# biodatageeks/datafusion-bio-functions

Hardware: AMD Instinct MI355X
Metric: overlap-pairs/sec + probe-rows/sec, IntervalJoinExec 100Mx1M (higher is better)
Workload: dtype int32; 1 GPU; join_100Mx1M_24contigs; probe_rows_per_gpu=100000000, build_rows_per_gpu=1000000, contigs=24, pairs_per_gpu=37210484, parallelism=partition-per-gpu x1, gather=False, build_overlap=True

## Files before the change

datafusion-bio-functions_amd/csrc/ivx_capi.hip:

```cpp
#include "ivx_internal.hpp"
#include <cstdlib>
#include <atomic>
#include <chrono>
#include <cstring>
#include <mutex>
#include <new>
#include <thread>
#include <condition_variable>
#include <deque>


void ivx_ctx::join_tail()
{
    if (!tail_pending) return;
    (void)hipStreamWaitEvent(stream, tail_ev, 0);
    tail_pending = false;
}

ivx_status ivx_ctx::get_scratch(int slot, size_t bytes, void **out)
{
    if (tail_pending && slot != WS_SORTHIST && slot != WS_T0 && slot != WS_T1 && slot != WS_T2) join_tail();
    ivx_buf &b = scratch[slot];
    if (sub_plan.valid && ((sub_plan.slots >> slot) & 1)) sub_plan.valid = false;
    if (join_plan.valid && ((join_plan.rows.slots >> slot) & 1)) join_plan.valid = false;
// ... 125 lines not shown
template <typename T>
ivx_status copy_out(ivx_ctx *ctx, int mem, T *dst, const T *dev, u64 n)
{
    if (mem == IVX_MEM_DEVICE || dst == nullptr || n == 0) return IVX_OK;
    IVX_HIP(ctx, hipMemcpyAsync(dst, dev, (size_t)n * sizeof(T), hipMemcpyDeviceToHost, ctx->stream));
    return IVX_OK;
}

ivx_status read_scalar(ivx_ctx *ctx, int word, u64 *out)
{
    IVX_HIP(ctx, hipMemcpyAsync(ctx->h_scalars + word, ctx->d_scalars + word, sizeof(u64), hipMemcpyDeviceToHost, ctx->stream));
    IVX_HIP(ctx, hipStreamSynchronize(ctx->stream));
    *out = ctx->h_scalars[word];
    return IVX_OK;
}

ivx_status check_probe_args(ivx_ctx *ctx, const ivx_index *ix, int kind, int mem, const void *s, const void *e, u64 n, bool defer_ready = false)
{
    if (!ctx) return IVX_ERR_INVALID;
    if (!ix) return ctx->fail(IVX_ERR_INVALID, "null index");
    if (ix->kind != kind) return ctx->fail(IVX_ERR_UNSUPPORTED, "index kind does not match this probe");
    if (ix->device != ctx->device) return ctx->fail(IVX_ERR_INVALID, "index lives on another device");
    if (mem != IVX_MEM_HOST && mem != IVX_MEM_DEVICE) return ctx->fail(IVX_ERR_INVALID, "bad mem");
    if (n && (!s || !e)) return ctx->fail(IVX_ERR_INVALID, "null coordinate column");
    if (n > 0xFFFFFFFFull) return ctx->fail(IVX_ERR_INVALID, "probe batch exceeds UInt32 index capacity");
    IVX_HIP(ctx, hipSetDevice(ctx->device));
    if (ix->ready != nullptr && !defer_ready) IVX_HIP(ctx, hipStreamWaitEvent(ctx->stream, ix->ready, 0));
    return IVX_OK;
}

struct CallMetrics {
    ivx_ctx *c; bool build; std::chrono::steady_clock::time_point t0;
    CallMetrics(ivx_ctx *ctx, bool is_build, u64 rows) : c(ctx), build(is_build), t0(std::chrono::steady_clock::now())
    {
        if (build) { c->metrics.build_input_batches++; c->metrics.build_input_rows += rows; }
        else { c->metrics.input_batches++; c->metrics.input_rows += rows; }
    }
    void out(u64 rows) { if (rows) { c->metrics.output_batches++; c->metrics.output_rows += rows; } }
    ~CallMetrics()
    {
        const double ms = std::chrono::duration<double, std::milli>(std::chrono::steady_clock::now() - t0).count();
        (build ? c->metrics.build_time : c->metrics.join_time) += ms;
    }
};

struct KernelTimer {
    ivx_ctx *c;
    explicit KernelTimer(ivx_ctx *ctx) : c(ctx) { (void)hipEventRecord(c->ev0, c->stream); c->last_ms = -1.0; }
    ~KernelTimer() { (void)hipEventRecord(c->ev1, c->stream); }
};

}


extern "C" const char *ivx_version(void) { return "ivx-hip 0.1 (gfx950)"; }

static bool create_aux_stream(hipStream_t *out)
{
    int lo = 0, hi = 0;
    if (hipDeviceGetStreamPriorityRange(&lo, &hi) == hipSuccess && hipStreamCreateWithPriority(out, hipStreamNonBlocking, hi) == hipSuccess) return true;
    return hipStreamCreateWithFlags(out, hipStreamNonBlocking) == hipSuccess;
}

extern "C" ivx_status ivx_ctx_create(int device_ordinal, ivx_ctx **out)
{
    if (!out) return IVX_ERR_INVALID;
    *out = nullptr;
    int ndev = 0;
    if (hipGetDeviceCount(&ndev) != hipSuccess || ndev <= 0) return IVX_ERR_NO_DEVICE;
    if (device_ordinal < 0 || device_ordinal >= ndev) return IVX_ERR_NO_DEVICE;
    hipDeviceProp_t prop;
    if (hipGetDeviceProperties(&prop, device_ordinal) != hipSuccess) return IVX_ERR_NO_DEVICE;
    if (std::strncmp(prop.gcnArchName, "gfx950", 6) != 0) return IVX_ERR_NO_DEVICE;
    ivx_ctx *c = new (std::nothrow) ivx_ctx();
    if (!c) return IVX_ERR_OOM;
    c->device = device_ordinal;
    bool ok = hipSetDevice(device_ordinal) == hipSuccess &&
              hipStreamCreateWithFlags(&c->own_stream, hipStreamNonBlocking) == hipSuccess &&
              create_aux_stream(&c->aux) &&
              hipEventCreateWithFlags(&c->ev_fork, hipEventDisableTiming) == hipSuccess &&
              hipEventCreateWithFlags(&c->tail_ev, hipEventDisableTiming) == hipSuccess &&
              hipEventCreate(&c->ev0) == hipSuccess && hipEventCreate(&c->ev1) == hipSuccess &&
              hipMalloc((void **)&c->d_scalars, 64 * sizeof(u64)) == hipSuccess &&
              hipHostMalloc((void **)&c->h_scalars, 64 * sizeof(u64), hipHostMallocDefault) == hipSuccess;
    if (!ok) { ivx_ctx_free(c); return IVX_ERR_HIP; }
    c->stream = c->own_stream;
    if (const char *e = getenv("IVX_BUILD_OVERLAP")) c->overlap = e[0] == '1';
    *out = c;
    return IVX_OK;
}

extern "C" void ivx_ctx_free(ivx_ctx *c)
{
    if (!c) return;
    (void)hipSetDevice(c->device);
    (void)hipStreamSynchronize(c->stream);
    if (c->aux) (void)hipStreamSynchronize(c->aux);
    for (auto &b : c->scratch) if (b.p) (void)hipFree(b.p);
    for (auto &b : c->pinned) if (b.p) (void)hipHostFree(b.p);
    if (c->d_scalars) (void)hipFree(c->d_scalars);
    if (c->h_scalars) (void)hipHostFree(c->h_scalars);
    if (c->ev0) (void)hipEventDestroy(c->ev0);
    if (c->ev1) (void)hipEventDestroy(c->ev1);
    if (c->own_stream) (void)hipStreamDestroy(c->own_stream);
    if (c->aux) (void)hipStreamDestroy(c->aux);
    if (c->ev_fork) (void)hipEventDestroy(c->ev_fork);
    if (c->tail_ev) (void)hipEventDestroy(c->tail_ev);
    delete c;
}

extern "C" const char *ivx_last_error(const ivx_ctx *c) { return c ? c->err.c_str() : "null ctx"; }

extern "C" ivx_status ivx_ctx_set_stream(ivx_ctx *c, void *hip_stream)
{
    if (!c) return IVX_ERR_INVALID;
    if (c->tail_pending) { (void)hipStreamSynchronize(c->aux); c->tail_pending = false; }
    c->stream = (hipStream_t)hip_stream;
    return IVX_OK;
}

extern "C" ivx_status ivx_ctx_use_own_stream(ivx_ctx *c)
{
    if (!c) return IVX_ERR_INVALID;
    if (c->tail_pending) { (void)hipStreamSynchronize(c->aux); c->tail_pending = false; }
    c->stream = c->own_stream;
    return IVX_OK;
}

extern "C" ivx_status ivx_ctx_set_build_overlap(ivx_ctx *c, int on)
{
    if (!c) return IVX_ERR_INVALID;
    c->overlap = on != 0;
    return IVX_OK;
}

extern "C" ivx_status ivx_ctx_synchronize(ivx_ctx *c)
{
    if (!c) return IVX_ERR_INVALID;
    if (c->tail_pending) { IVX_HIP(c, hipStreamSynchronize(c->aux)); c->tail_pending = false; }
    IVX_HIP(c, hipStreamSynchronize(c->stream));
    return IVX_OK;
}

extern "C" ivx_status ivx_ctx_metrics(const ivx_ctx *c, ivx_metrics *out)
{
    if (!c || !out) return IVX_ERR_INVALID;
    *out = c->metrics;
    return IVX_OK;
}

extern "C" void ivx_ctx_reset_metrics(ivx_ctx *c) { if (c) c->metrics = ivx_metrics{}; }

extern "C" ivx_status ivx_ctx_set_memory_limit(ivx_ctx *c, uint64_t bytes)
{
    if (!c) return IVX_ERR_INVALID;
    c->mem_limit = bytes;
    return IVX_OK;
}

extern "C" uint64_t ivx_ctx_reserved_bytes(const ivx_ctx *c) { return c ? c->reserved() : 0; }

extern "C" ivx_status ivx_ctx_trim(ivx_ctx *c, uint64_t keep_bytes)
{
    if (!c) return IVX_ERR_INVALID;
    IVX_HIP(c, hipSetDevice(c->device));
    IVX_HIP(c, hipStreamSynchronize(c->stream));
    if (c->aux) { IVX_HIP(c, hipStreamSynchronize(c->aux)); c->tail_pending = false; }
    c->sub_plan.valid = false; c->join_plan.valid = false;
// ... 76 lines not shown
    if (ix->ready) { (void)hipEventSynchronize(ix->ready); (void)hipEventDestroy(ix->ready); }
    for (size_t i = 0; i < ix->allocs.size(); i++) pool_give(ix->device, ix->allocs[i], ix->alloc_caps[i]);
    if (ix->owner_bytes) ix->owner_bytes->fetch_sub(ix->bytes, std::memory_order_relaxed);
    delete ix;
}

extern "C" uint64_t ivx_index_rows(const ivx_index *ix) { return ix ? ix->n : 0; }
extern "C" uint64_t ivx_index_device_bytes(const ivx_index *ix) { return ix ? ix->bytes : 0; }

extern "C" ivx_status ivx_index_layout(ivx_ctx *ctx, const ivx_index *ix, uint32_t *out, uint32_t n_out)
{
    if (!ctx) return IVX_ERR_INVALID;
    if (!ix) return ctx->fail(IVX_ERR_INVALID, "null index");
    if (n_out && !out) return ctx->fail(IVX_ERR_INVALID, "null out");
    if (ix->device != ctx->device) return ctx->fail(IVX_ERR_INVALID, "index lives on another device");
    u32 w[IVX_LAYOUT_WORDS] = {};
    w[IVX_LAYOUT_KIND] = (u32)ix->kind;
    if (ix->kind != IVX_KIND_NEAREST && ix->jv.hdr != nullptr) {
        IVX_HIP(ctx, hipSetDevice(ctx->device));
        if (ix->ready != nullptr) IVX_HIP(ctx, hipStreamWaitEvent(ctx->stream, ix->ready, 0));
        u32 h[HDR_WORDS];
        IVX_HIP(ctx, hipMemcpyAsync(h, ix->jv.hdr, sizeof(h), hipMemcpyDeviceToHost, ctx->stream));
        IVX_HIP(ctx, hipStreamSynchronize(ctx->stream));
        const u32 nlev = h[HDR_NLEV] < IVX_MAXL ? h[HDR_NLEV] : IVX_MAXL;
        u32 levrows = 0;
        for (u32 l = 0; l < nlev; l++) if (h[HDR_LEVCNT + l]) levrows |= 1u << l;
        w[IVX_LAYOUT_SH0] = h[HDR_SH0];
        w[IVX_LAYOUT_NLEV] = h[HDR_NLEV];
        w[IVX_LAYOUT_LEVROWS] = levrows;
        w[IVX_LAYOUT_RCELLS] = h[HDR_NREG] ? h[HDR_RCELLS] : 0u;
        w[IVX_LAYOUT_RCS] = h[HDR_NREG] ? h[HDR_CS] : 0xFFFFFFFFu;
        w[IVX_LAYOUT_NREG] = h[HDR_NREG];
        w[IVX_LAYOUT_PK24] = h[HDR_PK24];
        w[IVX_LAYOUT_SLOW] = h[HDR_SLOW];
        w[IVX_LAYOUT_FG] = h[HDR_FG];
        w[IVX_LAYOUT_FBITS] = h[HDR_FG] != 0xFFFFFFFFu ? h[HDR_FBITS] : 0u;
        w[IVX_LAYOUT_NROUTE_NREG] = ix->nroute_nreg;
        w[IVX_LAYOUT_LBUILD] = h[HDR_LBUILD];
    }
    for (u32 i = 0; i < n_out && i < (u32)IVX_LAYOUT_WORDS; i++) out[i] = w[i];
    return IVX_OK;
}


static bool rowval_routed_ok(u64 n)
{
    if (const char *f = getenv("IVX_JOIN_PATH")) return !strcmp(f, "routed");
    return n >= (1u << 21);
}

static ivx_status overlap_common(ivx_ctx *ctx, const ivx_index *ix, int mem, int mode,
                                 const u32 *key, const i32 *start, const i32 *end, u64 n,
                                 u32 *per_row, u8 *exists, u32 *bidx, u32 *pidx, u64 cap, u64 *total)
{
    IVX_TRY(check_probe_args(ctx, ix, IVX_KIND_OVERLAP, mem, start, end, n, true));
    CallMetrics cm(ctx, false, n);
    const u32 *dk = nullptr; const i32 *ds = nullptr, *de = nullptr;
    bool regions = ix->jv_nreg > 0 && (mode == JP_COUNT || mode == JP_FILL) && n >= (1u << 21);
    bool rowval = ix->jv_nreg > 0 && ix->jv_nreg <= IVX_MAXREG_WIDE && (mode == JP_PER_ROW || mode == JP_EXISTS) && n >= (1u << 21);
    if (const char *f = getenv("IVX_JOIN_PATH")) {
        if (!strcmp(f, "direct")) regions = rowval = false;
        else if (!strcmp(f, "regions")) {
            regions = ix->jv_nreg > 0 && (mode == JP_COUNT || mode == JP_FILL);
            rowval = ix->jv_nreg > 0 && ix->jv_nreg <= IVX_MAXREG_WIDE && (mode == JP_PER_ROW || mode == JP_EXISTS);
        }
    }
    const void *in[3] = {key, start, end};
    ivx_join_plan &pl = ctx->join_plan;
    const bool planned = regions && mode == JP_FILL && pl.valid && !getenv("IVX_NO_PLAN") && pl.mem == mem && memcmp(pl.in, in, sizeof(in)) == 0 && pl.n == n &&
                         pl.ix == (const void *)ix && pl.ix_serial == ix->serial && pl.stream == ctx->stream;
    if (ix->ready != nullptr && !(regions && !planned)) IVX_HIP(ctx, hipStreamWaitEvent(ctx->stream, ix->ready, 0));
    if (!planned) {
        IVX_TRY(stage_in(ctx, mem, WS_IN_KEY, key, n, &dk));
        IVX_TRY(stage_in(ctx, mem, WS_IN_START, start, n, &ds));
        IVX_TRY(stage_in(ctx, mem, WS_IN_END, end, n, &de));
    }
    u32 *d_row = nullptr, *d_b = nullptr, *d_p = nullptr; u8 *d_ex = nullptr;
    IVX_TRY(stage_out(ctx, mem, WS_OUT_A, per_row, n, &d_row));
    IVX_TRY(stage_out(ctx, mem, WS_OUT_B, exists, n, &d_ex));
    IVX_TRY(stage_out(ctx, mem, WS_OUT_C, bidx, cap, &d_b));
    IVX_TRY(stage_out(ctx, mem, WS_OUT_D, pidx, cap, &d_p));
    const bool defer_clear = regions && !planned;
    if (!defer_clear) IVX_HIP(ctx, hipMemsetAsync(ctx->d_scalars, 0, 2 * sizeof(u64), ctx->stream));
    {
        KernelTimer t(ctx);
        if (regions) {
            if (!planned) pl.valid = false;
            const ivx_status st = ivx_join_probe_regions(ctx, ix->jv, ix->jv_nreg, mode, dk, ds, de, n, d_b, d_p, cap, ctx->d_scalars, planned, ix->jv_filter, ix->jv_pk24,
                                                         ix->jv_fast_unknown ? 2 : (ix->jv_fast ? 1 : 0), planned ? nullptr : ix->ready, defer_clear);
            if (st != IVX_OK) { pl.valid = false; return st; }
            if (mode == JP_COUNT && pl.valid) { memcpy(pl.in, in, sizeof(in)); pl.mem = mem; pl.n = n; pl.ix = ix; pl.ix_serial = ix->serial; pl.stream = ctx->stream; }
        }
        else if (rowval) IVX_TRY(ivx_rowval_probe_regions(ctx, ix->jv, ix->jv_nreg, mode == JP_PER_ROW ? IVX_RV_PER_ROW : IVX_RV_EXISTS, dk, ds, de, n, 0,
                                                          mode == JP_PER_ROW ? (void *)d_row : (void *)d_ex, ctx->d_scalars, ix->jv_filter, ix->jv_pk24, ix->jv_fast && !ix->jv_fast_unknown));
        else if (n && (mode == JP_PER_ROW || mode == JP_EXISTS) && ix->nroute_nreg > 0 && rowval_routed_ok(n))
            IVX_TRY(ivx_join_rowval_routed(ctx, ix, mode, dk, ds, de, n, d_row, d_ex, ctx->d_scalars));
        else IVX_TRY(ivx_join_probe(ctx, ix->jv, mode, dk, ds, de, n, d_row, d_ex, d_b, d_p, cap, ctx->d_scalars));
    }
    u64 tot = 0;
    if (mode != JP_EXISTS) {
        IVX_HIP(ctx, hipMemcpyAsync(ctx->h_scalars, ctx->d_scalars, 2 * sizeof(u64), hipMemcpyDeviceToHost, ctx->stream));
        IVX_HIP(ctx, hipStreamSynchronize(ctx->stream));
        tot = ctx->h_scalars[0];
        if (ctx->h_scalars[1]) { ctx->join_plan.valid = false; return ctx->fail(IVX_ERR_HIP, "internal error: the probe met an unpublished page of routed rows"); }
    }
    if (mode == JP_COUNT && regions && pl.valid) pl.total = tot;
    if (total) *total = tot;
    if (mode == JP_FILL && tot > cap) return ctx->fail(IVX_ERR_CAPACITY, "pair buffers too small");
    cm.out(mode == JP_FILL ? tot : (mode == JP_COUNT ? 0 : n));
    if (planned) pl.valid = false;
    IVX_TRY(copy_out(ctx, mem, per_row, d_row, n));
    IVX_TRY(copy_out(ctx, mem, exists, d_ex, n));
    if (mode == JP_FILL) { IVX_TRY(copy_out(ctx, mem, bidx, d_b, tot)); IVX_TRY(copy_out(ctx, mem, pidx, d_p, tot)); }
    if (mem == IVX_MEM_HOST) IVX_HIP(ctx, hipStreamSynchronize(ctx->stream));
    return IVX_OK;
}

extern "C" ivx_status ivx_probe_overlap_count(ivx_ctx *ctx, const ivx_index *ix, int mem, const uint32_t *key,
                                              const int32_t *start, const int32_t *end, uint64_t n,
                                              uint32_t *per_row, uint64_t *total)
{
    return overlap_common(ctx, ix, mem, per_row ? JP_PER_ROW : JP_COUNT, key, start, end, n, per_row, nullptr, nullptr, nullptr, 0, total);
}

__global__ void k_add_base(u32 *__restrict__ p, u64 n, u32 base)
{
    for (u64 i = (u64)blockIdx.x * blockDim.x + threadIdx.x; i < n; i += (u64)gridDim.x * blockDim.x) p[i] += base;
}

struct HostCopier {
    struct Job { void *dst; const void *src; size_t bytes; hipEvent_t ev; };
    std::mutex mu; std::condition_variable cv, cv_done; std::deque<Job> jobs; bool closed = false; hipError_t herr = hipSuccess;
    u64 done = 0;
    hipStream_t cs = nullptr; std::thread th; std::vector<hipEvent_t> evs; bool started = false;
    hipError_t start(int device)
    {
        const hipError_t e = hipStreamCreateWithFlags(&cs, hipStreamNonBlocking);
        if (e != hipSuccess) return e;
        try {
        th = std::thread([this, device]() {
            (void)hipSetDevice(device);
            for (;;) {
                Job j;
                { std::unique_lock<std::mutex> lk(mu); cv.wait(lk, [&] { return closed || !jobs.empty(); }); if (jobs.empty()) return; j = jobs.front(); jobs.pop_front(); }
                hipError_t e2 = j.ev ? hipStreamWaitEvent(cs, j.ev, 0) : hipSuccess;
                if (e2 == hipSuccess && j.bytes) e2 = hipMemcpyAsync(j.dst, j.src, j.bytes, hipMemcpyDeviceToHost, cs);
                if (e2 == hipSuccess) e2 = hipStreamSynchronize(cs);
                { std::lock_guard<std::mutex> lk(mu); if (e2 != hipSuccess) herr = e2; done++; }
                cv_done.notify_all();
            }
        });
        } catch (...) { (void)hipStreamDestroy(cs); cs = nullptr; return hipErrorOutOfMemory; }
        started = true;
        return hipSuccess;
    }
    hipError_t mark(hipStream_t st, hipEvent_t *ev)
    {
        hipError_t e = hipEventCreateWithFlags(ev, hipEventDisableTiming);
        if (e != hipSuccess) return e;
        evs.push_back(*ev);
        return hipEventRecord(*ev, st);
    }
    void push(void *dst, const void *src, size_t bytes, hipEvent_t ev)
    {
        { std::lock_guard<std::mutex> lk(mu); jobs.push_back(Job{dst, src, bytes, ev}); }
        cv.notify_all();
    }
    void wait_until(u64 k) { std::unique_lock<std::mutex> lk(mu); cv_done.wait(lk, [&] { return done >= k; }); }
    hipError_t finish()
    {
        if (!started) return hipSuccess;
        { std::lock_guard<std::mutex> lk(mu); closed = true; }
        cv.notify_all();
        th.join();
        for (hipEvent_t e : evs) (void)hipEventDestroy(e);
        (void)hipStreamDestroy(cs);
        started = false;
        return herr;
    }
    ~HostCopier() { (void)finish(); }
};

static ivx_status overlap_fill_host_chunked(ivx_ctx *ctx, const ivx_index *ix, const u32 *key, const i32 *start, const i32 *end, u64 n,
                                            u32 *bidx, u32 *pidx, u64 cap, u64 *written, u32 nchunk)
// ... 46 lines not shown
        }
    }
    const hipError_t es = hipStreamSynchronize(st);
    const hipError_t herr = hc.finish();
    ctx->join_plan.valid = false;
    ctx->metrics.input_batches = m0.input_batches + 1;
    ctx->metrics.output_batches = m0.output_batches + ((rc == IVX_OK && !over && cum) ? 1 : 0);
    if (over) ctx->metrics.output_rows = m0.output_rows;
    if (rc != IVX_OK) return rc;
    if (es != hipSuccess) return ctx->fail_hip("hipStreamSynchronize", es);
    if (herr != hipSuccess) return ctx->fail_hip("hipMemcpyAsync(pairs)", herr);
    if (written) *written = over ? need : cum;
    if (over) return ctx->fail(IVX_ERR_CAPACITY, "pair buffers too small");
    return IVX_OK;
}

extern "C" ivx_status ivx_probe_overlap_fill(ivx_ctx *ctx, const ivx_index *ix, int mem, const uint32_t *key,
                                             const int32_t *start, const int32_t *end, uint64_t n,
                                             uint32_t *build_idx, uint32_t *probe_idx, uint64_t cap, uint64_t *written)
{
    if (ctx && cap && (!build_idx || !probe_idx)) return ctx->fail(IVX_ERR_INVALID, "null pair buffers");
    if (ctx && ix && mem == IVX_MEM_HOST && cap && start && end) {
        const char *ce = getenv("IVX_HOST_CHUNKS");
        const u32 nchunk = ce ? (u32)atoi(ce) : (n >= (16ull << 20) ? 4u : 1u);
        const void *in[3] = {key, start, end};
        const ivx_join_plan &pl = ctx->join_plan;
        const bool planned = pl.valid && pl.mem == mem && memcmp(pl.in, in, sizeof(in)) == 0 && pl.n == n && pl.ix == (const void *)ix && pl.ix_serial == ix->serial;
        if (nchunk > 1 && n >= (u64)nchunk * 65536 && !planned && ix->kind == IVX_KIND_OVERLAP)
            return overlap_fill_host_chunked(ctx, ix, key, start, end, n, build_idx, probe_idx, cap, written, nchunk);
    }
    return overlap_common(ctx, ix, mem, JP_FILL, key, start, end, n, nullptr, nullptr, build_idx, probe_idx, cap, written);
}

extern "C" ivx_status ivx_probe_exists(ivx_ctx *ctx, const ivx_index *ix, int mem, const uint32_t *key,
                                       const int32_t *start, const int32_t *end, uint64_t n, uint8_t *exists)
{
    if (ctx && n && !exists) return ctx->fail(IVX_ERR_INVALID, "null exists buffer");
    return overlap_common(ctx, ix, mem, JP_EXISTS, key, start, end, n, nullptr, exists, nullptr, nullptr, 0, nullptr);
}


namespace {

ivx_status marks_stage(ivx_ctx *ctx, int mem, u32 *caller, u64 nw, u32 **dev)
{
    if (mem == IVX_MEM_DEVICE) { *dev = caller; return IVX_OK; }
    IVX_TRY(ctx->get_scratch(WS_OUT_A, (size_t)nw * sizeof(u32), (void **)dev));
    if (nw) IVX_HIP(ctx, hipMemsetAsync(*dev, 0, (size_t)nw * sizeof(u32), ctx->stream));
    return IVX_OK;
}

ivx_status marks_or_back(ivx_ctx *ctx, int mem, u32 *caller, const u32 *dev, u64 nw)
{
    if (mem == IVX_MEM_DEVICE || nw == 0) return IVX_OK;
    std::vector<u32> got;
    try { got.resize((size_t)nw); } catch (const std::bad_alloc &) { return ctx->fail(IVX_ERR_OOM, "host allocation failed"); }
    IVX_HIP(ctx, hipMemcpyAsync(got.data(), dev, (size_t)nw * sizeof(u32), hipMemcpyDeviceToHost, ctx->stream));
    IVX_HIP(ctx, hipStreamSynchronize(ctx->stream));
    for (u64 w = 0; w < nw; w++) caller[w] |= got[w];
    return IVX_OK;
}

ivx_status mark_common(ivx_ctx *ctx, const ivx_index *ix, int mem, const u32 *key, const i32 *start, const i32 *end, u64 n, u32 *marks)
{
    IVX_TRY(check_probe_args(ctx, ix, IVX_KIND_OVERLAP, mem, start, end, n));
    if (n && ix->n && !marks) return ctx->fail(IVX_ERR_INVALID, "null mark bitmap");
    CallMetrics cm(ctx, false, n);
    ctx->join_plan.valid = false;
    const u64 nw = (ix->n + 31) / 32;
    if (n == 0 || nw == 0) return IVX_OK;
    bool regions = ix->jv_nreg > 0 && ix->jv_nreg <= IVX_MAXREG_WIDE && n >= (1u << 21);
    if (const char *f = getenv("IVX_JOIN_PATH")) {
        if (!strcmp(f, "direct")) regions = false;
        else if (!strcmp(f, "regions")) regions = ix->jv_nreg > 0 && ix->jv_nreg <= IVX_MAXREG_WIDE;
    }
    const u32 *dk = nullptr; const i32 *ds = nullptr, *de = nullptr; u32 *dm = nullptr;
    IVX_TRY(stage_in(ctx, mem, WS_IN_KEY, key, n, &dk));
    IVX_TRY(stage_in(ctx, mem, WS_IN_START, start, n, &ds));
    IVX_TRY(stage_in(ctx, mem, WS_IN_END, end, n, &de));
    IVX_TRY(marks_stage(ctx, mem, marks, nw, &dm));
    {
        KernelTimer t(ctx);
        bool took = false;
        if (regions) IVX_TRY(ivx_mark_probe_regions(ctx, ix->jv, ix->jv_nreg, dk, ds, de, n, dm, ix->jv_filter, ix->jv_pk24, ix->jv_fast && !ix->jv_fast_unknown, &took));
        if (!took) IVX_TRY(ivx_mark_probe(ctx, ix->jv, dk, ds, de, n, dm));
    }
    return marks_or_back(ctx, mem, marks, dm, nw);
}

}

extern "C" ivx_status ivx_probe_mark_build(ivx_ctx *ctx, const ivx_index *ix, int mem, const uint32_t *key,
                                           const int32_t *start, const int32_t *end, uint64_t n, uint32_t *marks)
{
    return mark_common(ctx, ix, mem, key, start, end, n, marks);
}

extern "C" ivx_status ivx_bits_mark(ivx_ctx *ctx, int mem, const uint32_t *idx, uint64_t n, uint32_t *bits, uint64_t n_bits)
{
    if (!ctx) return IVX_ERR_INVALID;
    if (mem != IVX_MEM_HOST && mem != IVX_MEM_DEVICE) return ctx->fail(IVX_ERR_INVALID, "bad mem");
    if (n && !idx) return ctx->fail(IVX_ERR_INVALID, "bits_mark: null idx");
    if (n_bits && !bits) return ctx->fail(IVX_ERR_INVALID, "bits_mark: null bitmap");
    if (n_bits > 0xFFFFFFFFull) return ctx->fail(IVX_ERR_INVALID, "bits_mark: bitmap exceeds UInt32 index capacity");
    if (n == 0) return IVX_OK;
    IVX_HIP(ctx, hipSetDevice(ctx->device));
    const u64 nw = (n_bits + 31) / 32;
    const u32 *didx; u32 *dbits;
    IVX_TRY(stage_in(ctx, mem, WS_IN_KEY, idx, n, &didx));
    IVX_TRY(marks_stage(ctx, mem, bits, nw, &dbits));
    {
        KernelTimer t(ctx);
        IVX_TRY(ivx_bits_mark_device(ctx, didx, n, dbits, n_bits));
    }
    return marks_or_back(ctx, mem, bits, dbits, nw);
}

extern "C" ivx_status ivx_bits_select(ivx_ctx *ctx, int mem, const uint32_t *bits, uint64_t n_bits, int want_set,
                                      uint32_t *out, uint64_t cap, uint64_t *n_out)
{
    if (!ctx) return IVX_ERR_INVALID;
    if (!n_out) return ctx->fail(IVX_ERR_INVALID, "null n_out");
    *n_out = 0;
    if (mem != IVX_MEM_HOST && mem != IVX_MEM_DEVICE) return ctx->fail(IVX_ERR_INVALID, "bad mem");
    if (n_bits && !bits) return ctx->fail(IVX_ERR_INVALID, "bits_select: null bitmap");
    if (cap && !out) return ctx->fail(IVX_ERR_INVALID, "bits_select: null out");
    if (n_bits > 0xFFFFFFFFull) return ctx->fail(IVX_ERR_INVALID, "bits_select: bitmap exceeds UInt32 index capacity");
    IVX_HIP(ctx, hipSetDevice(ctx->device));
    const u32 *dbits; u32 *dout;
    IVX_TRY(stage_in(ctx, mem, WS_IN_KEY, bits, (n_bits + 31) / 32, &dbits));
    IVX_TRY(stage_out(ctx, mem, WS_OUT_A, out, cap, &dout));
    u64 m = 0;
    {
        KernelTimer t(ctx);
        const ivx_status st = ivx_bits_select_device(ctx, dbits, n_bits, want_set, dout, cap, &m);
        *n_out = m;
        if (st != IVX_OK) return st;
    }
    if (cap) IVX_TRY(copy_out(ctx, mem, out, dout, m));
    if (mem == IVX_MEM_HOST) IVX_HIP(ctx, hipStreamSynchronize(ctx->stream));
    return IVX_OK;
}


ivx_status ivx_count_probe(ivx_ctx *ctx, const ivx_index *ix, const u32 *key, const i32 *s, const i32 *e, u64 n, int strict, i64 *out);
ivx_status ivx_coverage_probe(ivx_ctx *ctx, const ivx_index *ix, const u32 *key, const i32 *s, const i32 *e, u64 n, int strict, i64 *out);
ivx_status ivx_nearest_probe(ivx_ctx *ctx, const ivx_index *ix, const u32 *key, const i32 *s, const i32 *e, u64 n,
                             int strict, u32 k, int include_overlaps, u32 *ob, u32 *op, i64 *od, u64 cap, u64 *rows);
ivx_status ivx_merge_device(ivx_ctx *ctx, const u32 *key, const i64 *s, const i64 *e, u64 n, u32 nkeys,
                            i64 min_dist, int strict, u32 *ok, i64 *os, i64 *oe, i64 *on, u64 *m);
ivx_status ivx_subtract_device(ivx_ctx *ctx, const u32 *lkey, const i64 *ls, const i64 *le, u64 nl,
                               const u32 *rkey, const i64 *rs, const i64 *re, u64 nr, u32 nkeys, int strict,
                               u32 *ok, i64 *os, i64 *oe, u32 *orow, u64 cap, u64 *n_out);
ivx_status ivx_subtract_fill_planned(ivx_ctx *ctx, u32 *ok, i64 *os, i64 *oe, u32 *orow, u64 cap, u64 *n_out);
ivx_status ivx_cluster_device(ivx_ctx *ctx, const u32 *key, const i64 *s, const i64 *e, u64 n, u32 nkeys,
                              i64 min_dist, int strict, const i64 *key_base,
                              u32 *ok, i64 *os, i64 *oe, u32 *orow, i64 *oc, i64 *ocs, i64 *oce, u64 *key_clusters, u64 *m);
ivx_status ivx_complement_device(ivx_ctx *ctx, const u32 *key, const i64 *s, const i64 *e, u64 n,
                                 const u32 *vkey, const i64 *vs, const i64 *ve, u64 nv, u32 nkeys, int strict,
                                 u32 *ok, i64 *os, i64 *oe, u64 cap, u64 *n_out);
ivx_status ivx_take_fixed_device(ivx_ctx *ctx, const void *src, u32 width, u64 n_src, const u8 *src_valid,
                                 const u32 *idx, u64 n, void *out, u8 *out_valid);
ivx_status ivx_take_view_device(ivx_ctx *ctx, const void *views, const u8 *const *bufs, u64 n_src, const u8 *src_valid,
                                const u32 *idx, u64 n, void *out_views, u8 *out_data, u64 data_cap, u64 *data_bytes, u8 *out_valid);
ivx_status ivx_take_bits_device(ivx_ctx *ctx, const u8 *src_bits, u64 n_src, const u8 *src_valid, const u32 *idx, u64 n, u8 *out_bits, u8 *out_valid);
ivx_status ivx_take_utf8_device(ivx_ctx *ctx, int large, const void *offsets, const u8 *data, u64 n_src, const u8 *src_valid,
                                const u32 *idx, u64 n, void *out_offsets, u8 *out_data, u64 data_cap, u64 *data_bytes, u8 *out_valid);
// ... 936 lines not shown
```

datafusion-bio-functions_amd/csrc/ivx_device.hpp:

```cpp
#pragma once
#include "ivx_internal.hpp"

__device__ __forceinline__ u32 lane_id() { return __builtin_amdgcn_mbcnt_hi(~0u, __builtin_amdgcn_mbcnt_lo(~0u, 0u)); }

__device__ __forceinline__ u32 mask_rank_from(u64 mask, u32 base)
{
    return __builtin_amdgcn_mbcnt_hi((u32)(mask >> 32), __builtin_amdgcn_mbcnt_lo((u32)mask, base));
}

__device__ __forceinline__ u32 mask_rank(u64 mask)
{
    return __builtin_amdgcn_mbcnt_hi((u32)(mask >> 32), __builtin_amdgcn_mbcnt_lo((u32)mask, 0u));
}

template <int CTRL, int ROWS>
__device__ __forceinline__ u32 dpp0(u32 v) { return (u32)__builtin_amdgcn_update_dpp(0, (int)v, CTRL, ROWS, 0xf, false); }
__device__ __forceinline__ u32 wave_incl_max32(u32 v)
{
    u32 o;
    o = dpp0<0x111, 0xf>(v); v = o > v ? o : v;
    o = dpp0<0x112, 0xf>(v); v = o > v ? o : v;
    o = dpp0<0x114, 0xf>(v); v = o > v ? o : v;
    o = dpp0<0x118, 0xf>(v); v = o > v ? o : v;
    o = dpp0<0x142, 0xa>(v); v = o > v ? o : v;
    o = dpp0<0x143, 0xc>(v); v = o > v ? o : v;
    return v;
}
__device__ __forceinline__ u32 wave_incl_sum32(u32 v)
{
    v += dpp0<0x111, 0xf>(v); v += dpp0<0x112, 0xf>(v); v += dpp0<0x114, 0xf>(v); v += dpp0<0x118, 0xf>(v);
    v += dpp0<0x142, 0xa>(v); v += dpp0<0x143, 0xc>(v);
    return v;
}
__device__ __forceinline__ u32 wave_prev32(u32 v) { return dpp0<0x138, 0xf>(v); }
__device__ __forceinline__ u32 wave_next32(u32 v) { return dpp0<0x130, 0xf>(v); }

template <typename T>
__device__ __forceinline__ T wave_incl_scan(T v)
{
    const u32 l = lane_id();
#pragma unroll
    for (int d = 1; d < IVX_WAVE; d <<= 1) {
        T o = __shfl_up(v, d, IVX_WAVE);
        if (l >= (u32)d) v += o;
    }
    return v;
}

template <typename T>
__device__ __forceinline__ T wave_sum(T v)
{
#pragma unroll
    for (int d = IVX_WAVE / 2; d > 0; d >>= 1) v += __shfl_xor(v, d, IVX_WAVE);
    return v;
}

template <typename T, int NT>
__device__ __forceinline__ T block_excl_scan(T v, T *lds, T *total)
{
    constexpr int NW = NT / IVX_WAVE;
    const u32 l = lane_id();
    const u32 w = threadIdx.x / IVX_WAVE;
    T inc = wave_incl_scan(v);
    if (l == IVX_WAVE - 1) lds[w] = inc;
    __syncthreads();
    if (threadIdx.x == 0) {
        T run = 0;
#pragma unroll
        for (int i = 0; i < NW; i++) { T t = lds[i]; lds[i] = run; run += t; }
        lds[NW] = run;
    }
    __syncthreads();
    T res = inc - v + lds[w];
    *total = lds[NW];
    __syncthreads();
    return res;
}

template <typename T, int NT>
__device__ __forceinline__ T block_sum(T v, T *lds)
{
    constexpr int NW = NT / IVX_WAVE;
    T s = wave_sum(v);
    if (lane_id() == 0) lds[threadIdx.x / IVX_WAVE] = s;
    __syncthreads();
    T r = 0;
#pragma unroll
    for (int i = 0; i < NW; i++) r += lds[i];
    __syncthreads();
    return r;
}

static inline u32 ivx_stream_grid(u64 n, u32 per_block, u32 max_blocks = 2048)
{
    u64 b = (n + per_block - 1) / per_block;
    if (b < 1) b = 1;
// ... 4 lines not shown
```

datafusion-bio-functions_amd/csrc/ivx_internal.hpp:

```cpp
#pragma once
#include <hip/hip_runtime.h>
#include <stdint.h>
#include <atomic>
#include <memory>
#include <string>
#include <vector>
#include "../../include/ivx.h"

typedef uint8_t u8;
typedef uint32_t u32;
typedef int32_t i32;
typedef uint64_t u64;
typedef int64_t i64;

#define IVX_WAVE 64

struct ivx_buf { void *p = nullptr; size_t cap = 0; };

enum { IVX_NSCRATCH = 56, IVX_NPIN = 4 };

struct ivx_sub_plan {
    bool valid = false;
    u64 slots = 0;
    int mem = 0;
    const void *in[6] = {};
    u64 nl = 0, nr = 0, nh = 0, total = 0;
    u32 nkeys = 0;
    int strict = 0;
    int wf = 0;
    hipStream_t stream = nullptr;
    const u32 *lk, *lrow, *rk, *hk, *hj;
    const i64 *lsv, *lev, *rsv, *hrs, *hpm;
    const void *sm;
    const u64 *offs;
    const u32 *plan_hlo; const i64 *plan_tail;
};

struct PageTab { u32 *ptab; u32 pstride, lgpg; };
struct ivx_route_ctl {
    u32 rcur[1024];
    u32 pool_next, pad0[3];
    u32 rest_n[2], pad1[2];
    u32 rfirst[1032];
    u32 cfirst[1032];
};
struct FpRest;
enum {
    IVX_ROWS_FLAT = 0,
    IVX_ROWS_PAGED,
    IVX_ROWS_TABLE
};
struct ivx_routed {
    int form = IVX_ROWS_FLAT;
    const u64 *se = nullptr;
    const u32 *ids = nullptr;
    const unsigned short *cidx = nullptr;
    const u32 *rfirst = nullptr;
    u32 nblk = 1, chunk = 0, ndig = 0;
    const u32 *unsorted = nullptr;
    PageTab pt{nullptr, 0u, 0u};
    bool packed = false;
    u32 rowbits = 32;
    bool all_routed = false;
    ivx_route_ctl *ctl = nullptr;
    FpRest *rest = nullptr; u64 *rest_rows = nullptr;
    const uint2 *vtab = nullptr;
    const i32 *ds = nullptr, *de = nullptr;
    u32 adj = 0;
    u64 slots = 0;
};

struct ivx_join_plan {
    bool valid = false;
    int mem = 0;
    const void *in[3] = {};
    u64 n = 0;
    u64 total = 0;
    const void *ix = nullptr; u64 ix_serial = 0;
    hipStream_t stream = nullptr;
    ivx_routed rows;
};

struct ivx_ctx {
    int device = 0;
    hipStream_t own_stream = nullptr;
    hipStream_t stream = nullptr;
    hipEvent_t ev0 = nullptr, ev1 = nullptr;
    double last_ms = 0.0;
    std::string err;
    ivx_buf scratch[IVX_NSCRATCH];
    ivx_buf pinned[IVX_NPIN];
    u64 *d_scalars = nullptr;
    u64 *h_scalars = nullptr;
    ivx_sub_plan sub_plan;
    ivx_join_plan join_plan;
    ivx_metrics metrics{};
    u64 mem_limit = 0;
    u64 fill_hint = 0;
    u64 scratch_bytes = 0, building_bytes = 0;
    hipStream_t aux = nullptr;
    hipEvent_t ev_fork = nullptr, tail_ev = nullptr;
    bool overlap = false, tail_pending = false;
    void join_tail();
    std::shared_ptr<std::atomic<u64>> live_index_bytes = std::make_shared<std::atomic<u64>>(0);
    u64 reserved() const { return scratch_bytes + building_bytes + live_index_bytes->load(std::memory_order_relaxed); }

    ivx_status fail(ivx_status st, const std::string &msg) { err = msg; return st; }
    ivx_status fail_hip(const char *what, hipError_t e)
    {
        err = std::string(what) + ": " + hipGetErrorString(e);
        return e == hipErrorOutOfMemory ? IVX_ERR_OOM : IVX_ERR_HIP;
    }
    ivx_status get_scratch(int slot, size_t bytes, void **out);
    ivx_status get_pinned(int slot, size_t bytes, void **out);
};

#define IVX_HIP(ctx, call)                                              \
    do {                                                                \
        hipError_t e__ = (call);                                        \
        if (e__ != hipSuccess) return (ctx)->fail_hip(#call, e__);      \
    } while (0)

#define IVX_TRY(call)                                                   \
    do {                                                                \
        ivx_status s__ = (call);                                        \
        if (s__ != IVX_OK) return s__;                                  \
    } while (0)

enum {
    WS_IN_KEY = 0, WS_IN_START, WS_IN_END, WS_IN2_KEY, WS_IN2_START, WS_IN2_END,
    WS_OUT_A, WS_OUT_B, WS_OUT_C, WS_OUT_D, WS_OUT_E, WS_OUT_F, WS_OUT_G, WS_OUT_H,
    WS_SCAN0, WS_SCAN1, WS_SCAN2,
    WS_GRID0, WS_GRID1, WS_GRID2,
    WS_SORTHIST,
    WS_SA0, WS_SA1, WS_SA2, WS_SB0, WS_SB1, WS_SB2,
    WS_RA0, WS_RA1, WS_RA2, WS_RB0, WS_RB1, WS_RB2,
    WS_T0, WS_T1, WS_T2, WS_T3, WS_T4, WS_T5, WS_T6, WS_T7, WS_T8, WS_T9,
    WS_IN3_KEY, WS_IN3_START, WS_IN3_END, WS_IN3_WEIGHT, WS_IN_KEYLEN,
    WS_IN_TEXTOFF, WS_IN_TEXT
};
static_assert(WS_IN_TEXT < IVX_NSCRATCH, "scratch slot ids must fit the context's slot array");

#ifndef IVX_LSTEP
#define IVX_LSTEP 2
#endif
#define IVX_MAXL (32 / IVX_LSTEP)
#define IVX_SH_MIN 4

struct ivx_ent { i32 s, e; u32 row; };

enum { HDR_SH0 = 0, HDR_NLEV = 1, HDR_NBINS = 2, HDR_CS = 3 , HDR_NREG = 4,
       HDR_RCELLS = 5 , HDR_RMUL_LO = 6, HDR_RMUL_HI = 7 , HDR_LEVCNT = 8 ,
       HDR_FG = 8 + IVX_MAXL , HDR_FBITS = 9 + IVX_MAXL ,
       HDR_PK24 = 10 + IVX_MAXL ,
       HDR_SLOW = 11 + IVX_MAXL ,
       HDR_LBUILD = 12 + IVX_MAXL ,
       HDR_BADKEY = 13 + IVX_MAXL ,
       HDR_WORDS = 14 + IVX_MAXL };
#define IVX_FBITS_MAX (1u << 24)
#define IVX_MAXREG 255
#define IVX_MAXREG_WIDE 1023
#define IVX_MAXREG2 65025u
#define IVX_REG_CS_MAX 13

#ifndef IVX_RP_ECAP
#define IVX_RP_ECAP 6144
#endif
#define IVX_RP_HALO 8u
struct ivx_regdesc { u32 k; i32 origin; u32 span, lb, slo, shi, e0, ne; i32 rbase;  };

struct JoinIndexView {
    const i32 *origin;
    const u32 *span;
    const u32 *kcnt;
    const u32 *lbase;
    const u32 *binstart;
    const ivx_ent *ent;
    const u32 *hdr;
    const u32 *kreg;
    const u32 *rkey;
    const ivx_regdesc *rdesc;
    const u32 *fbits;
    const u32 *fbase;
    u32 nkeys;
};

struct RankGridView {
    const i32 *origin;
    const u32 *span;
    const u32 *kcnt;
    const u32 *koff;
    const u32 *kbase;
    const u32 *binstart;
    const i32 *val;
    const u32 *hdr;
    u32 nkeys;
};

struct CoverageView {
    RankGridView first, last;
    const i64 *pw;
    const i32 *nfirst, *nlast;
};

struct ivx_nrec { i32 a, b; u32 row; i32 pmax; };

struct NearestView {
    RankGridView by_start, by_end, pmax;
    const ivx_nrec *rs;
    const ivx_nrec *re;
    JoinIndexView ov;
};

struct DepthProfileView {
    const u32 *key, *pos;
    const i32 *cov;
    const u32 *koff;
    const u8 *seen;
    u64 steps;
};

struct ivx_index {
    u64 serial = 0;
    int kind = 0;
    int device = 0;
    u64 n = 0;
    u32 nkeys = 0;
    size_t bytes = 0;
    std::shared_ptr<std::atomic<u64>> owner_bytes;
    std::vector<void *> allocs;
    std::vector<size_t> alloc_caps;
    JoinIndexView jv{};
    u32 jv_nreg = 0;
    bool jv_filter = false;
    bool jv_pk24 = false;
    bool jv_fast = false;
    bool jv_fast_unknown = false;
    hipEvent_t ready = nullptr;
    RankGridView gs{}, ge{};
    CoverageView cv{};
    NearestView nv{};
    JoinIndexView nroute{};
    u32 nroute_nreg = 0;
    DepthProfileView dp{};
    int flags = 0;
};
enum { IVX_IXF_REGION_ROWVAL = 1 };

ivx_status ivx_scan_exclusive_u32(ivx_ctx *ctx, u32 *data, u64 n, const u32 *skip = nullptr);
ivx_status ivx_scan_exclusive_u64(ivx_ctx *ctx, u64 *data, u64 n);

ivx_status ivx_join_build(ivx_ctx *ctx, ivx_index *ix, const u32 *key, const i32 *s, const i32 *e, u64 n, bool overlap = false);
ivx_status ivx_join_probe(ivx_ctx *ctx, const JoinIndexView &jv, int mode,
                          const u32 *key, const i32 *s, const i32 *e, u64 n,
                          u32 *per_row, u8 *exists, u32 *ob, u32 *op, u64 cap, u64 *d_cursor);
enum { JP_COUNT = 0, JP_PER_ROW = 1, JP_EXISTS = 2, JP_FILL = 3 };
ivx_status ivx_join_probe_regions(ivx_ctx *ctx, const JoinIndexView &jv, u32 nreg, int mode,
                                  const u32 *key, const i32 *s, const i32 *e, u64 n,
                                  u32 *ob, u32 *op, u64 cap, u64 *d_cursor, bool planned = false, bool has_filter = false, bool pk24 = false,
                                  int fast = 0 , hipEvent_t ready = nullptr,
                                  bool clear_cursor = false );

enum { IVX_RV_COUNT = 0, IVX_RV_COVERAGE = 1, IVX_RV_PER_ROW = 2, IVX_RV_EXISTS = 3 };
ivx_status ivx_route_view_build(ivx_ctx *ctx, ivx_index *ix, const i32 *origin, const u32 *span, const u32 *kcnt);
void ivx_route_view_ready(ivx_ctx *ctx, ivx_index *ix);
ivx_status ivx_join_rowval_routed(ivx_ctx *ctx, const ivx_index *ix, int mode, const u32 *key, const i32 *s, const i32 *e, u64 n,
                                  u32 *per_row, u8 *exists, u64 *d_total);
ivx_status ivx_unroute_u32(ivx_ctx *ctx, const ivx_routed &r, u64 n, const u32 *vb, u32 *out32, u8 *out8);
ivx_status ivx_route_rows(ivx_ctx *ctx, const JoinIndexView &rv, const u32 *key, const i32 *s, const i32 *e, u64 n, u32 adj, ivx_routed *out);
ivx_status ivx_unroute_pair(ivx_ctx *ctx, const ivx_routed &r, u64 n, const u32 *vb, const i64 *vd, u32 *ob, u32 *op, i64 *od, i64 dflt);
ivx_status ivx_rowval_probe_regions(ivx_ctx *ctx, const JoinIndexView &jv, u32 nreg, int kind,
                                    const u32 *key, const i32 *s, const i32 *e, u64 n, int strict, void *out, u64 *d_total,
                                    bool has_filter = false, bool pk24 = false, bool fast = false);

ivx_status ivx_mark_probe(ivx_ctx *ctx, const JoinIndexView &jv, const u32 *key, const i32 *s, const i32 *e, u64 n, u32 *marks);
ivx_status ivx_mark_probe_regions(ivx_ctx *ctx, const JoinIndexView &jv, u32 nreg, const u32 *key, const i32 *s, const i32 *e, u64 n,
                                  u32 *marks, bool has_filter, bool pk24, bool fast, bool *took);
ivx_status ivx_bits_mark_device(ivx_ctx *ctx, const u32 *idx, u64 n, u32 *bits, u64 n_bits);
ivx_status ivx_bits_select_device(ivx_ctx *ctx, const u32 *bits, u64 n_bits, int want_set, u32 *out, u64 cap, u64 *n_out);

ivx_status ivx_depth_device(ivx_ctx *ctx, const u32 *rkey, const u32 *rpos, const u32 *rflags, const u32 *rmapq,
                            const i32 *cigar_offsets, const u32 *cigar_ops, u64 n_reads,
                            const u32 *skey, const u32 *sstart, const u32 *send, const i32 *sweight, u64 n_seg,
                            u32 nkeys, const u32 *key_len, u32 filter_flag, u32 min_mapq,
                            u32 *ok, u32 *os, u32 *oe, i32 *oc, u64 cap, u64 *n_out);

struct ivx_depth_evs { u64 n; const u64 *ev; const uint2 *cg; };
ivx_status ivx_depth_events(ivx_ctx *ctx, const u32 *rkey, const u32 *rpos, const u32 *rflags, const u32 *rmapq,
                            const i32 *cigar_offsets, const u32 *cigar_ops, u64 n_reads,
                            const u32 *skey, const u32 *sstart, const u32 *send, const i32 *sweight, u64 n_seg,
                            u32 nkeys, const u32 *key_len, u32 filter_flag, u32 min_mapq, u8 *seen, ivx_depth_evs *out);
struct ivx_cigar_plan {
    int large; const void *off; const u8 *txt; u64 n_reads, n_bytes, n_ops, nblk; i64 off0; u32 mis; void *tsum;
};
ivx_status ivx_cigar_count(ivx_ctx *ctx, int large, const void *text_offsets, const u8 *text, bool text_at_off0, u64 n_reads,
                           ivx_cigar_plan *plan);
ivx_status ivx_cigar_write(ivx_ctx *ctx, const ivx_cigar_plan &plan, i32 *out_off, u32 *out_ops);
ivx_status ivx_depth_profile_begin(ivx_ctx *ctx, ivx_index *ix, u8 **seen);
ivx_status ivx_depth_profile_finish(ivx_ctx *ctx, ivx_index *ix, const ivx_depth_evs &evs);
ivx_status ivx_depth_profile_koff(ivx_ctx *ctx, const u32 *skey, u32 steps, u32 nkeys, u32 *koff);
ivx_status ivx_depth_expand_device(ivx_ctx *ctx, const DepthProfileView &dp, u32 key, u32 first_pos, u64 n, int skip_pos0,
                                   i32 *out_pos, int16_t *out_cov);
ivx_status ivx_depth_profile_merge_device(ivx_ctx *ctx, const DepthProfileView &a, u32 nka, const DepthProfileView &b, u32 nkb, ivx_index *ix);
ivx_status ivx_depth_profile_blocks_device(ivx_ctx *ctx, const DepthProfileView &dp, u32 *ok, u32 *os, u32 *oe, i32 *oc, u64 cap, u64 *n_out);
ivx_status ivx_depth_regions_device(ivx_ctx *ctx, const DepthProfileView &dp, u32 nkeys, const u32 *qkey, const u32 *qs, const u32 *qe, u64 n,
                                    u32 pos_lo, const u32 *key_hi, int skip_pos0, const i32 *thresholds, u32 n_thr,
                                    i64 *out_len, i64 *out_sum, i64 *out_ge);
ivx_status ivx_depth_windows_device(ivx_ctx *ctx, const DepthProfileView &dp, u32 key, u32 first_pos, u32 last_pos, u32 width, u64 n,
                                    int skip_pos0, const i32 *thresholds, u32 n_thr, i64 *out_len, i64 *out_sum, i64 *out_ge);

ivx_status ivx_index_alloc(ivx_ctx *ctx, ivx_index *ix, size_t bytes, void **out);
```

datafusion-bio-functions_amd/csrc/ivx_join.hip:

```cpp
#include <cstdlib>
#include <cstring>
#include "ivx_device.hpp"
#include "ivx_grid.hpp"
#include "ivx_join.hpp"

namespace {

constexpr int BT = 256;

constexpr int LB_T = 1024;
constexpr int LB_ROWS = 4;
constexpr u32 LB_TILE = LB_T * LB_ROWS;
constexpr u32 LB_STRIDE = IVX_MAXREG_WIDE + 1;
constexpr u32 LB_CCAP = 8192;
constexpr u32 LB_MAXTILES = 1024;
constexpr int LB_KEEP = (IVX_RP_ECAP + LB_T - 1) / LB_T;
constexpr u64 LB_MIN_ROWS = 1u << 14, LB_MAX_ROWS = (u64)LB_MAXTILES * LB_TILE;
static_assert(LB_STRIDE == LB_T && LB_TILE <= 4096 && LB_CCAP == (1u << IVX_REG_CS_MAX), "k_lbuild_tiles: one table word per thread, 12-bit ranks");
static inline u32 lb_tstride(u32 ntiles) { return ntiles | 1u; }


__device__ __forceinline__ u32 cells_of(u32 cnt, u32 span, u32 sh) { return cnt ? (sh >= 32 ? 1u : (span >> sh) + 1u) : 0u; }

__global__ __launch_bounds__(1024) void k_join_layout(const i32 *kmin, const i32 *kmax, const u32 *kcnt, u32 nkeys, u64 n,
                                                      i32 *origin, u32 *span, u32 *lbase, u32 *hdr, u64 maxcells,
                                                      u32 *kreg, u32 *rkey, const u32 *lenhist, u32 regmax, u32 *fbase, int filter_mode, int lbuild_ok, const u32 *badkey)
{
    __shared__ u64 red[1024 / IVX_WAVE + 1];
    __shared__ u32 s_sh0;
    const u32 t = threadIdx.x;
    for (u32 k = t; k < nkeys; k += 1024) {
        u32 c = kcnt[k];
        origin[k] = c ? kmin[k] : 0;
        span[k] = c ? (u32)((i64)kmax[k] - (i64)kmin[k]) : 0u;
    }
    __syncthreads();
    __shared__ u64 s_tot[40];
    __shared__ u64 s_loff[IVX_MAXL + 1];
    const u32 wv = t / IVX_WAVE, ln = lane_id();
    constexpr u32 NWV = 1024 / IVX_WAVE;
    const u64 budget0 = 2 * n + nkeys;
    for (u32 sh = IVX_SH_MIN + wv; sh <= 31; sh += NWV) {
        u64 a = 0;
        for (u32 k = ln; k < nkeys; k += IVX_WAVE) a += cells_of(kcnt[k], span[k], sh);
        a = wave_sum(a);
        if (ln == 0) s_tot[sh] = a;
    }
    __syncthreads();
    __shared__ float s_occ0;
    __shared__ u64 s_cum[34];
    __shared__ float s_cost[32], s_cocc[32];
    __shared__ u32 s_shb;
    if (t <= 32) s_cum[t + 1] = lenhist[t];
    __syncthreads();
    __shared__ u32 s_fg;
    if (t == 0) {
        u32 shb = IVX_SH_MIN;
        while (shb < 31 && s_tot[shb] > budget0) shb++;
        s_shb = shb;
        u32 fg = 0xFFFFFFFFu;
        if (filter_mode != 0 && (u64)nkeys * 34 < IVX_FBITS_MAX / 2) {
            u32 g = IVX_SH_MIN;
            while (g < 31 && s_tot[g] + (u64)nkeys * 34 > IVX_FBITS_MAX) g++;
            const double bits = (double)(s_tot[g] + nkeys);
            double touched = 0.0;
            for (u32 b = 0; b <= 32; b++) touched += (double)s_cum[b + 1] * ((b > g ? (double)(3ull << (b - g)) * 0.25 : 0.0) + 1.5);
            if (n && s_tot[g] + (u64)nkeys * 34 <= IVX_FBITS_MAX && (filter_mode == 2 || touched < 0.15 * bits) && touched < 64.0 * (double)n + 1.0e6) fg = g;
        }
        s_fg = fg;
        u64 run = 0;
        s_cum[0] = 0;
        for (u32 b = 0; b <= 32; b++) { run += s_cum[b + 1]; s_cum[b + 1] = run; }
    }
    __syncthreads();
    if (t < 32) {
        const u32 sh = s_shb + t;
        float cost = 3.0e38f, occ0 = 0.f;
        if (sh <= 31) {
            cost = 0.f;
            u32 lo_bits = 0;
            for (u32 l = 0; l < IVX_MAXL; l++) {
                const u32 lsh = sh + IVX_LSTEP * l;
                const bool last = lsh >= 32 || l + 1 == IVX_MAXL;
                const u32 hi_bits = last ? 32u : lsh;
                const u64 rows = hi_bits >= lo_bits ? s_cum[hi_bits + 1] - s_cum[lo_bits] : 0;
                const float cells = lsh >= 32 ? (float)(nkeys ? nkeys : 1u) : (float)(s_tot[lsh] ? s_tot[lsh] : 1);
                const float occ = (float)rows / cells;
                if (l == 0) { occ0 = occ; cost += 1.f + 2.2f * occ; }
                else if (rows) cost += 8.f + 2.2f * occ * 4.f;
                if (last) break;
                lo_bits = lsh + 1;
            }
        }
        s_cost[t] = cost; s_cocc[t] = occ0;
    }
    __syncthreads();
    if (t == 0) {
        u32 bi = 0;
        for (u32 c = 1; c < 32; c++) if (s_cost[c] < s_cost[bi]) bi = c;
#ifdef IVX_SH_BIAS
        { const int b2 = (int)bi + (IVX_SH_BIAS); bi = b2 < 0 ? 0u : (s_shb + (u32)b2 > 31 ? 31 - s_shb : (u32)b2); }
#endif
        s_sh0 = s_shb + bi; s_occ0 = s_cocc[bi];
    }
    __syncthreads();
    const u32 sh0 = s_sh0;
    u32 nlev = 0;
    for (u32 l = 0; l < IVX_MAXL; l++) { nlev = l + 1; if (sh0 + IVX_LSTEP * l >= 32) break; }
    for (u32 l = wv; l < nlev; l += NWV) {
// ... 23 lines not shown
    }
    for (u32 mid = wv; mid <= 32; mid += NWV) {
        u64 a = 0;
        for (u32 k = ln; k < nkeys; k += IVX_WAVE) {
            const u64 c = cells_of(kcnt[k], span[k], sh0);
            a += mid >= 32 ? (c ? 1u : 0u) : ((c + (1ull << mid) - 1) >> mid);
        }
        a = wave_sum(a);
        if (ln == 0) s_tot[mid] = a;
    }
    __syncthreads();
    u32 clo = 0;
    while (clo < 32 && s_tot[clo] > IVX_MAXREG) clo++;
    if (clo > IVX_REG_CS_MAX && clo <= 32 && s_tot[IVX_REG_CS_MAX] <= IVX_MAXREG2) clo = IVX_REG_CS_MAX;
    u64 R = clo < 32 ? (1ull << clo) : 0;
    bool pow2 = true;
    if (clo < 32 && s_occ0 * (float)R > 0.9f * (float)IVX_RP_ECAP) {
        const float want = 0.85f * (float)IVX_RP_ECAP / s_occ0;
        R = want < 1.f ? 1ull : (u64)want;
        pow2 = false;
    }
    auto regions_for = [&](u64 r) -> u64 {
        u64 a = 0;
        for (u32 k = t; k < nkeys; k += 1024) { const u64 c = cells_of(kcnt[k], span[k], sh0); a += (c + r - 1) / r; }
        return block_sum<u64, 1024>(a, red);
    };
    if (R && nkeys > regmax && regions_for(1ull << 40) > regmax) R = 0;
    if (R) {
        if (!(pow2 && clo < 32 && s_tot[clo] <= regmax)) while (regions_for(R) > regmax) { R *= 2; }
        if (!pow2) {
            u64 mc = 0;
            for (u32 k = t; k < nkeys; k += 1024) { const u64 c = cells_of(kcnt[k], span[k], sh0); mc = c > mc ? c : mc; }
            __shared__ u64 s_mc;
            if (t == 0) s_mc = 0;
            __syncthreads();
            atomicMax((unsigned long long *)&s_mc, (unsigned long long)mc);
            __syncthreads();
            const u64 M = ((1ull << 40) + R - 1) / R;
            if (s_mc * R >= (1ull << 40) || s_mc > (1ull << 63) / M || (R & (R - 1)) == 0) {
                u64 p = 1; while (p * 2 <= R) p *= 2;
                R = p; pow2 = true;
                while (regions_for(R) > regmax) R *= 2;
            }
        }
    }
    u32 cs = 32;
    if (R && pow2) { cs = 0; while ((1ull << cs) < R) cs++; }
    u64 rrun = 0;
    for (u32 k0 = 0; k0 < nkeys; k0 += 1024) {
        const u32 k = k0 + t;
        u64 c = k < nkeys ? cells_of(kcnt[k], span[k], sh0) : 0u;
        c = R ? (c + R - 1) / R : 0;
        u64 tot;
        const u64 ex = block_excl_scan<u64, 1024>(c, red, &tot);
        if (k < nkeys && R) {
            kreg[k] = (u32)(rrun + ex);
            for (u64 r = 0; r < c; r++) rkey[rrun + ex + r] = k;
        }
        rrun += tot;
    }
    {
        const u32 fg = s_fg;
        u64 frun = 0;
        for (u32 k0 = 0; k0 < nkeys; k0 += 1024) {
            const u32 k = k0 + t;
            u64 c = (fg != 0xFFFFFFFFu && k < nkeys && kcnt[k]) ? (u64)(((span[k] >> fg) + 2u + 31u) & ~31u) : 0u;
            u64 tot;
            const u64 ex = block_excl_scan<u64, 1024>(c, red, &tot);
            if (k < nkeys) fbase[k] = (u32)(frun + ex);
            frun += tot;
        }
        if (t == 0) { hdr[HDR_FG] = frun <= IVX_FBITS_MAX ? fg : 0xFFFFFFFFu; hdr[HDR_FBITS] = (u32)frun; }
    }
    if (t == 0) {
        kreg[nkeys] = (u32)rrun;
        hdr[HDR_CS] = pow2 ? cs : 0xFFFFFFFFu;
        hdr[HDR_NREG] = R ? (u32)rrun : 0u;
        hdr[HDR_RCELLS] = (u32)(R > 0xFFFFFFFFull ? 0xFFFFFFFFull : R);
        const u64 M = R ? ((1ull << 40) + R - 1) / R : 0;
        hdr[HDR_RMUL_LO] = (u32)M; hdr[HDR_RMUL_HI] = (u32)(M >> 32);
        hdr[HDR_PK24] = (R && sh0 < 24 && R <= (1ull << (24 - sh0))) ? 1u : 0u;
        hdr[HDR_BADKEY] = *badkey;
        hdr[HDR_LBUILD] = (lbuild_ok && R && R <= LB_CCAP && rrun && rrun <= IVX_MAXREG_WIDE && s_cum[33] == s_cum[sh0 + 1]) ? 1u : 0u;
    }
}

__global__ __launch_bounds__(LB_T) void k_lbuild_tiles(const u32 *__restrict__ key, const i32 *__restrict__ s, const i32 *__restrict__ e, u64 n, u32 nkeys,
                                                     const i32 *origin, const u32 *kreg, u32 *hdr, ivx_ent *__restrict__ rows,
                                                     u32 *__restrict__ tab, u32 tstride, u32 *__restrict__ binstart, u64 nbinwords)
{
    if (hdr[HDR_LBUILD] == 0) {
        for (u64 i = (u64)blockIdx.x * LB_T + threadIdx.x; i < nbinwords; i += (u64)gridDim.x * LB_T) binstart[i] = 0;
        return;
    }
    __shared__ u32 s_cnt[LB_STRIDE];
    __shared__ u32 red[LB_T / IVX_WAVE + 1];
    const u32 t = threadIdx.x;
    s_cnt[t] = 0;
    const u32 sh0 = hdr[HDR_SH0], cs = hdr[HDR_CS];
    const u64 rmul = (u64)hdr[HDR_RMUL_LO] | ((u64)hdr[HDR_RMUL_HI] << 32);
    __syncthreads();
    const u64 base = (u64)blockIdx.x * LB_TILE;
    const u32 have = n - base < LB_TILE ? (u32)(n - base) : LB_TILE;
    const u32 *tk = key ? key + base : nullptr;
    const i32 *ts = s + base, *te = e + base;
    i32 rs[LB_ROWS], re[LB_ROWS];
    u32 rr[LB_ROWS];
#pragma unroll
    for (int it = 0; it < LB_ROWS; it++) {
        const u32 i = (u32)it * LB_T + t;
        rr[it] = 0xFFFFFFFFu; rs[it] = 0; re[it] = 0;
        if (i < have) {
            const u32 k = tk ? tk[i] : 0u;
            if (k < nkeys) {
                rs[it] = ts[i]; re[it] = te[i];
                const u32 c = (u32)((i64)rs[it] - (i64)origin[k]) >> sh0;
                u32 reg = kreg[k] + (cs != 0xFFFFFFFFu ? c >> cs : (u32)(((u64)c * rmul) >> 40));
                reg = reg < LB_STRIDE - 1 ? reg : LB_STRIDE - 2;
                rr[it] = reg | (atomicAdd(&s_cnt[reg], 1u) << 10);
            }
        }
    }
    __syncthreads();
    u32 tot;
    const u32 p = block_excl_scan<u32, LB_T>(s_cnt[t], red, &tot);
    s_cnt[t] = p; tab[(u64)t * tstride + blockIdx.x] = p;
    if (t == 0 && tot) hdr[HDR_LEVCNT] = 1u;
    __syncthreads();
    ivx_ent *trows = rows + base;
#pragma unroll
    for (int it = 0; it < LB_ROWS; it++) {
        if (rr[it] == 0xFFFFFFFFu) continue;
        ivx_ent x; x.s = rs[it]; x.e = re[it]; x.row = (u32)base + (u32)it * LB_T + t;
        trows[s_cnt[rr[it] & (LB_STRIDE - 1)] + (rr[it] >> 10)] = x;
    }
}

__global__ __launch_bounds__(LB_T) void k_lbuild_regions(const i32 *origin, const u32 *span, const u32 *lbase, const u32 *kreg, const u32 *rkey,
                                                       const u32 *hdr, u32 nkeys, const ivx_ent *__restrict__ rows, const u32 *__restrict__ tab,
                                                       u32 ntiles, u32 tstride, u32 *__restrict__ binstart, ivx_ent *__restrict__ ent)
{
    if (hdr[HDR_LBUILD] == 0) return;
    const u32 r = blockIdx.x, nreg = hdr[HDR_NREG], t = threadIdx.x;
    if (r >= nreg) return;
    __shared__ u32 s_cell[LB_CCAP];
    __shared__ u32 s_tpre[LB_MAXTILES + 1];
    __shared__ unsigned short s_src[LB_MAXTILES];
    __shared__ u32 red[LB_T / IVX_WAVE + 1];
    const u32 sh0 = hdr[HDR_SH0], R = hdr[HDR_RCELLS], k = rkey[r];
    const i64 o = origin[k];
    const u32 cells0 = (span[k] >> sh0) + 1u;
    const u32 rc0 = (u32)((u64)(r - kreg[k]) * R);
    const u32 nc = cells0 - rc0 < R ? cells0 - rc0 : R;
    u32 run = 0, e0 = 0, total = 0;
    for (u32 t0 = 0; t0 < ntiles; t0 += LB_T) {
        const u32 ti = t0 + t;
        u32 a = 0, b = 0;
        if (ti < ntiles) {
            a = tab[(u64)r * tstride + ti]; b = tab[(u64)(r + 1) * tstride + ti];
            total += tab[(u64)(LB_STRIDE - 1) * tstride + ti];
        }
        u32 tot;
        const u32 ex = block_excl_scan<u32, LB_T>(b - a, red, &tot);
        if (ti < ntiles) { s_tpre[ti] = run + ex; s_src[ti] = (unsigned short)a; }
        run += tot; e0 += a;
    }
    e0 = block_sum<u32, LB_T>(e0, red);
    total = block_sum<u32, LB_T>(total, red);
    const u32 N = run;
    if (t == 0) s_tpre[ntiles] = N;
    for (u32 j = t; j < nc; j += LB_T) s_cell[j] = 0;
    __syncthreads();
    auto fetch = [&](u32 i) -> ivx_ent {
        u32 lo = 0, hi = ntiles - 1;
        while (lo < hi) { const u32 m = (lo + hi + 1) >> 1; if (s_tpre[m] <= i) lo = m; else hi = m - 1; }
        return rows[(u64)lo * LB_TILE + s_src[lo] + (i - s_tpre[lo])];
    };
    auto cell_in = [&](i32 st) -> u32 { const u32 c = ((u32)((i64)st - o) >> sh0) - rc0; return c < nc ? c : nc - 1; };
    ivx_ent mine[LB_KEEP];
#pragma unroll
    for (int j = 0; j < LB_KEEP; j++) {
        const u32 i = t + (u32)j * LB_T;
        if (i < N) { mine[j] = fetch(i); atomicAdd(&s_cell[cell_in(mine[j].s)], 1u); }
    }
    for (u32 i = t + LB_KEEP * LB_T; i < N; i += LB_T) atomicAdd(&s_cell[cell_in(fetch(i).s)], 1u);
    __syncthreads();
    const u64 gb = (u64)lbase[k] + rc0;
    u32 crun = 0;
    for (u32 c0 = 0; c0 < nc; c0 += 4 * LB_T) {
        const u32 j = c0 + 4 * t;
        u32 c4[4], sum = 0, tot;
#pragma unroll
        for (int q = 0; q < 4; q++) { c4[q] = j + q < nc ? s_cell[j + q] : 0u; sum += c4[q]; }
        u32 p = crun + block_excl_scan<u32, LB_T>(sum, red, &tot);
#pragma unroll
        for (int q = 0; q < 4; q++) { if (j + q < nc) { s_cell[j + q] = p; binstart[gb + j + q] = e0 + p; } p += c4[q]; }
        crun += tot;
    }
    {
        const u32 nlev = hdr[HDR_NLEV], nbins = hdr[HDR_NBINS];
        const u32 l0 = nlev > 1 ? lbase[nkeys] : nbins;
        const u32 len = nbins + 1 - l0, per = (len + nreg - 1) / nreg;
        const u64 a = (u64)l0 + (u64)r * per, b = a + per < (u64)nbins + 1 ? a + per : (u64)nbins + 1;
        for (u64 x = a + t; x < b; x += LB_T) binstart[x] = total;
    }
    __syncthreads();
#pragma unroll
    for (int j = 0; j < LB_KEEP; j++) {
        const u32 i = t + (u32)j * LB_T;
        if (i < N) ent[e0 + atomicAdd(&s_cell[cell_in(mine[j].s)], 1u)] = mine[j];
    }
    for (u32 i = t + LB_KEEP * LB_T; i < N; i += LB_T) { const ivx_ent x = fetch(i); ent[e0 + atomicAdd(&s_cell[cell_in(x.s)], 1u)] = x; }
}

__global__ __launch_bounds__(256) void k_join_regdesc(const i32 *origin, const u32 *span, const u32 *lbase, u32 *hdr,
                                                      const u32 *kreg, const u32 *rkey, const u32 *binstart, ivx_regdesc *rdesc)
{
    const u32 r = threadIdx.x + blockIdx.x * 256;
    if (r == 0) {
        bool upper = hdr[HDR_LEVCNT] == 0;
        for (u32 l = 1; l < hdr[HDR_NLEV]; l++) upper |= hdr[HDR_LEVCNT + l] != 0;
        if (upper) hdr[HDR_SLOW] = 1u;
    }
    if (r >= hdr[HDR_NREG]) return;
    const u32 sh0 = hdr[HDR_SH0];
    const u64 R = hdr[HDR_RCELLS];
    ivx_regdesc d;
    d.k = rkey[r]; d.origin = origin[d.k]; d.span = span[d.k]; d.lb = lbase[d.k];
    const u32 cells0 = (d.span >> sh0) + 1u;
    const u64 rc0w = (u64)(r - kreg[d.k]) * R;
    const u32 rc0 = (u32)rc0w;
    const u64 rc1w = rc0w + R;
    const u32 rc1 = rc1w < cells0 ? (u32)rc1w : cells0;
    d.slo = rc0 ? rc0 - 1u : 0u;
    d.shi = rc1 + IVX_RP_HALO < cells0 ? rc1 + IVX_RP_HALO : cells0;
    d.e0 = binstart[d.lb + d.slo];
    d.ne = binstart[d.lb + d.shi] - d.e0;
    d.rbase = (i32)((i64)d.origin + (i64)(rc0w << sh0));
    if (d.ne > IVX_RP_ECAP || d.shi - d.slo + 1u > 8192u + IVX_RP_HALO + 2u) hdr[HDR_SLOW] = 1u;
    rdesc[r] = d;
}

__global__ __launch_bounds__(BT) void k_join_count(const u32 *__restrict__ key, const i32 *__restrict__ s,
                                                   const i32 *__restrict__ e, u64 n, u32 nkeys,
                                                   const i32 *origin, const u32 *lbase, u32 *hdr, u32 *bincnt,
                                                   u32 *__restrict__ cellid, u32 *__restrict__ rank)
{
    if (hdr[HDR_LBUILD]) return;
    const u32 sh0 = hdr[HDR_SH0], nlev = hdr[HDR_NLEV];
    u32 levels = 0;
    for (u64 i = (u64)blockIdx.x * BT + threadIdx.x; i < n; i += (u64)gridDim.x * BT) {
        u32 k = key ? key[i] : 0u;
        if (k >= nkeys) { cellid[i] = 0xFFFFFFFFu; continue; }
        i32 si = s[i], ei = e[i];
        u32 l = level_of(si, ei, sh0, nlev);
        const u32 c = cell_of(origin, lbase, nkeys, k, si, l, sh0);
        cellid[i] = c;
        rank[i] = atomicAdd(&bincnt[c], 1u);
        levels |= 1u << l;
    }
#pragma unroll
    for (int d = IVX_WAVE / 2; d > 0; d >>= 1) levels |= __shfl_xor(levels, d, IVX_WAVE);
    if (lane_id() == 0)
        for (u32 l = 0; l < nlev; l++)
            if ((levels >> l) & 1u) hdr[HDR_LEVCNT + l] = 1u;
}

__global__ __launch_bounds__(BT) void k_join_scatter(const i32 *__restrict__ s, const i32 *__restrict__ e, u64 n,
                                                     const u32 *__restrict__ binstart, const u32 *__restrict__ cellid,
                                                     const u32 *__restrict__ rank, ivx_ent *ent, const u32 *hdr)
{
    if (hdr[HDR_LBUILD]) return;
    for (u64 i = (u64)blockIdx.x * BT + threadIdx.x; i < n; i += (u64)gridDim.x * BT) {
        const u32 c = cellid[i];
        if (c == 0xFFFFFFFFu) continue;
        ivx_ent x; x.s = s[i]; x.e = e[i]; x.row = (u32)i;
        ent[binstart[c] + rank[i]] = x;
    }
}

__global__ __launch_bounds__(BT) void k_join_filter(const u32 *__restrict__ key, const i32 *__restrict__ s, const i32 *__restrict__ e, u64 n, u32 nkeys,
                                                    const i32 *origin, const u32 *span, const u32 *fbase, const u32 *hdr, u32 *fbits)
{
    const u32 g = hdr[HDR_FG];
    if (g == 0xFFFFFFFFu) return;
    for (u64 i = (u64)blockIdx.x * BT + threadIdx.x; i < n; i += (u64)gridDim.x * BT) {
        const u32 k = key ? key[i] : 0u;
        if (k >= nkeys) continue;
        const i32 si = s[i], ei = e[i];
        const u32 last = (span[k] >> g) + 1u;
        const i64 o = origin[k];
        const u32 b0 = (u32)(((i64)si - o) >> g);
        const i64 hi = ((i64)(ei > si ? ei : si) - o) >> g;
        const u32 b1 = hi > (i64)last ? last : (u32)hi;
        const u32 p0 = fbase[k] + b0, p1 = fbase[k] + b1;
        for (u32 w = p0 >> 5; w <= (p1 >> 5); w++) {
            u32 m = 0xFFFFFFFFu;
            if (w == (p0 >> 5)) m &= 0xFFFFFFFFu << (p0 & 31);
            if (w == (p1 >> 5)) m &= 0xFFFFFFFFu >> (31 - (p1 & 31));
            if ((fbits[w] & m) != m) atomicOr(&fbits[w], m);
        }
    }
}


constexpr int PT = 256;
constexpr int PI = 4;
constexpr int PTILE = PT * PI;

__global__ __launch_bounds__(1024) void k_nroute_layout(const i32 *origin, const u32 *span, const u32 *kcnt, u32 nkeys, u32 *kreg, u32 *rkey, u32 *hdr)
{
    __shared__ u64 red[1024 / IVX_WAVE + 1];
    const u32 t = threadIdx.x;
    const u32 sh0 = 10;
    auto regions_for = [&](u32 cs) -> u64 {
        u64 a = 0;
        for (u32 k = t; k < nkeys; k += 1024) if (kcnt[k]) a += (((u64)(span[k] >> sh0) + 1) + ((1ull << cs) - 1)) >> cs;
        return block_sum<u64, 1024>(a, red);
    };
    u32 cs = 0;
    while (cs < 32 && regions_for(cs) > IVX_MAXREG_WIDE) cs++;
    const bool ok = regions_for(cs) <= IVX_MAXREG_WIDE;
// ... 112 lines not shown


ivx_status ivx_route_view_build(ivx_ctx *ctx, ivx_index *ix, const i32 *origin, const u32 *span, const u32 *kcnt)
{
    hipStream_t st = ctx->stream;
    const u32 nkeys = ix->nkeys;
    u32 *kreg, *rkey, *rhdr;
    IVX_TRY(ivx_index_alloc(ctx, ix, ((size_t)nkeys + 1) * sizeof(u32), (void **)&kreg));
    IVX_TRY(ivx_index_alloc(ctx, ix, ((size_t)IVX_MAXREG_WIDE + 1) * sizeof(u32), (void **)&rkey));
    IVX_TRY(ivx_index_alloc(ctx, ix, HDR_WORDS * sizeof(u32), (void **)&rhdr));
    IVX_HIP(ctx, hipMemsetAsync(rhdr, 0, HDR_WORDS * sizeof(u32), st));
    hipLaunchKernelGGL(k_nroute_layout, dim3(1), dim3(1024), 0, st, origin, span, kcnt, nkeys, kreg, rkey, rhdr);
    IVX_HIP(ctx, hipMemcpyAsync(ctx->h_scalars + 48, rhdr, HDR_WORDS * sizeof(u32), hipMemcpyDeviceToHost, st));
    ix->nroute = JoinIndexView{};
    ix->nroute.origin = origin; ix->nroute.span = span; ix->nroute.kcnt = kcnt; ix->nroute.kreg = kreg; ix->nroute.rkey = rkey;
    ix->nroute.hdr = rhdr; ix->nroute.nkeys = nkeys;
    IVX_HIP(ctx, hipGetLastError());
    return IVX_OK;
}
void ivx_route_view_ready(ivx_ctx *ctx, ivx_index *ix) { ix->nroute_nreg = ((const u32 *)(ctx->h_scalars + 48))[HDR_NREG]; }

ivx_status ivx_join_rowval_routed(ivx_ctx *ctx, const ivx_index *ix, int mode, const u32 *key, const i32 *s, const i32 *e, u64 n,
                                  u32 *per_row, u8 *exists, u64 *d_total)
{
    hipStream_t st = ctx->stream;
    ivx_routed R;
    IVX_TRY(ivx_route_rows(ctx, ix->nroute, key, s, e, n, 0u, &R));
    u32 *vb;
    IVX_TRY(ctx->get_scratch(WS_T2, n * sizeof(u32), (void **)&vb));
    const u32 grid = (ivx_stream_grid(n, PT * 4, 1280u) + 7u) & ~7u;
    hipLaunchKernelGGL(k_overlap_rowval_routed, dim3(grid), dim3(PT), 0, st, ix->jv, ix->nroute.rkey, ix->nroute_nreg, R.se, R.rfirst, R.nblk,
                       mode == JP_EXISTS ? 1 : 0, vb, (unsigned long long *)d_total, R.unsorted);
    IVX_TRY(ivx_unroute_u32(ctx, R, n, vb, per_row, exists));
    const u32 g2 = ivx_stream_grid(n, PTILE, 256 * 8);
    if (mode == JP_PER_ROW) hipLaunchKernelGGL((k_probe_overlap<JP_PER_ROW, PI>), dim3(g2), dim3(PT), 0, st, ix->jv, key, s, e, n, per_row, exists, (u32 *)nullptr, (u32 *)nullptr, (u64)0, (unsigned long long *)d_total, R.unsorted);
    else hipLaunchKernelGGL((k_probe_overlap<JP_EXISTS, PI>), dim3(g2), dim3(PT), 0, st, ix->jv, key, s, e, n, per_row, exists, (u32 *)nullptr, (u32 *)nullptr, (u64)0, (unsigned long long *)d_total, R.unsorted);
    IVX_HIP(ctx, hipGetLastError());
    return IVX_OK;
}

ivx_status ivx_join_build(ivx_ctx *ctx, ivx_index *ix, const u32 *key, const i32 *s, const i32 *e, u64 n, bool overlap)
{
    const u32 nkeys = ix->nkeys;
    hipStream_t st = ctx->stream;
    const u64 maxcells = 2 * n + (IVX_LSTEP >= 4 ? n / 4 : n) + (u64)IVX_MAXL * nkeys + 64;
    if (maxcells + 1 >= 0xFFFFFFFFull) return ctx->fail(IVX_ERR_INVALID, "build side too large for 32-bit cell ids");

    i32 *origin; u32 *span, *kcnt, *lbase, *binstart, *hdr, *kreg, *rkey, *fbase, *fbits; ivx_ent *ent; ivx_regdesc *rdesc;
    IVX_TRY(ivx_index_alloc(ctx, ix, nkeys * sizeof(i32), (void **)&origin));
    IVX_TRY(ivx_index_alloc(ctx, ix, nkeys * sizeof(u32), (void **)&span));
    IVX_TRY(ivx_index_alloc(ctx, ix, nkeys * sizeof(u32), (void **)&kcnt));
    IVX_TRY(ivx_index_alloc(ctx, ix, (size_t)IVX_MAXL * nkeys * sizeof(u32), (void **)&lbase));
    IVX_TRY(ivx_index_alloc(ctx, ix, (maxcells + 1) * sizeof(u32), (void **)&binstart));
    IVX_TRY(ivx_index_alloc(ctx, ix, HDR_WORDS * sizeof(u32), (void **)&hdr));
    IVX_TRY(ivx_index_alloc(ctx, ix, ((size_t)nkeys + 1) * sizeof(u32), (void **)&kreg));
    size_t regcap = (size_t)(n / (IVX_RP_ECAP / 2)) + (size_t)(maxcells >> IVX_REG_CS_MAX) + 2 * (size_t)nkeys + 64;
    regcap = regcap <= IVX_MAXREG + 1 ? (size_t)IVX_MAXREG + 1 : (regcap > (size_t)IVX_MAXREG2 + 1 ? (size_t)IVX_MAXREG2 + 1 : regcap);
    IVX_TRY(ivx_index_alloc(ctx, ix, regcap * sizeof(u32), (void **)&rkey));
    IVX_TRY(ivx_index_alloc(ctx, ix, regcap * sizeof(ivx_regdesc), (void **)&rdesc));
    IVX_TRY(ivx_index_alloc(ctx, ix, (n ? n : 1) * sizeof(ivx_ent), (void **)&ent));
    const size_t fwords = IVX_FBITS_MAX / 32 + 4;
    IVX_TRY(ivx_index_alloc(ctx, ix, nkeys * sizeof(u32), (void **)&fbase));
    IVX_TRY(ivx_index_alloc(ctx, ix, fwords * sizeof(u32), (void **)&fbits));

    i32 *kmin, *kmax; u32 *cellid, *rank, *errflag;
    IVX_TRY(ctx->get_scratch(WS_GRID0, nkeys * sizeof(i32), (void **)&kmin));
    IVX_TRY(ctx->get_scratch(WS_GRID1, nkeys * sizeof(i32), (void **)&kmax));
    const char *benv = getenv("IVX_BUILD");
    const bool lb_try = n >= LB_MIN_ROWS && n <= LB_MAX_ROWS && !(benv && !strcmp(benv, "global"));
    const u32 lb_tiles = lb_try ? (u32)((n + LB_TILE - 1) / LB_TILE) : 0u;
    IVX_TRY(ctx->get_scratch(WS_GRID2, (n ? n : 1) * (lb_try ? sizeof(ivx_ent) : sizeof(u32)), (void **)&cellid));
    const size_t tabbytes = (size_t)lb_tstride(lb_tiles) * LB_STRIDE * sizeof(u32);
    IVX_TRY(ctx->get_scratch(WS_T9, (n ? n : 1) * sizeof(u32) > tabbytes ? (n ? n : 1) * sizeof(u32) : tabbytes, (void **)&rank));
    errflag = (u32 *)(ctx->d_scalars + 8);
    u32 *lenhist = (u32 *)(ctx->d_scalars + 32);

    ivx_zero_ranges zr{{errflag, lenhist, hdr}, {1u, 34u, (u32)HDR_WORDS}};
    const char *fenv = getenv("IVX_FILTER");
    const int filter_mode = !fenv ? 1 : !strcmp(fenv, "0") ? 0 : !strcmp(fenv, "force") ? 2 : 1;
    static_assert((IVX_FBITS_MAX / 32 + 4) % 4 == 0, "the bitmap is cleared in 16-byte words");
    if (filter_mode) { zr.big = (uint4 *)fbits; zr.nbig = (u32)(fwords / 4); }
    IVX_TRY(ivx_keystats_len(ctx, key, s, n, nkeys, kmin, kmax, kcnt, errflag, 1u, e, lenhist, &zr));
    const u32 grid = ivx_stream_grid(n, BT * 2, 16384);
    hipLaunchKernelGGL(k_join_layout, dim3(1), dim3(1024), 0, st, kmin, kmax, kcnt, nkeys, n, origin, span, lbase, hdr, maxcells, kreg, rkey, (const u32 *)lenhist, (u32)(regcap - 1), fbase, filter_mode, lb_try ? 1 : 0, (const u32 *)errflag);
    if (filter_mode) hipLaunchKernelGGL(k_join_filter, dim3(grid), dim3(BT), 0, st, key, s, e, n, nkeys, (const i32 *)origin, (const u32 *)span, (const u32 *)fbase, (const u32 *)hdr, fbits);
    const bool want_route = ix->kind == IVX_KIND_OVERLAP && n >= (4u << 20);
    overlap = overlap && ctx->overlap && ctx->aux != nullptr && !want_route && n >= (1u << 16);
    hipStream_t tail_st = st;
    struct TailGuard {
        ivx_ctx *c; bool armed = false;
        ~TailGuard() { if (armed) (void)hipStreamSynchronize(c->aux); }
    } guard{ctx};
    bool q_lds = lb_try, q_global = true;
    if (overlap) {
        ctx->join_tail();
        IVX_HIP(ctx, hipEventRecord(ctx->ev_fork, st));
        IVX_HIP(ctx, hipStreamWaitEvent(ctx->aux, ctx->ev_fork, 0));
        tail_st = ctx->aux;
        IVX_HIP(ctx, hipMemcpyAsync(ctx->h_scalars + 32, hdr, HDR_WORDS * sizeof(u32), hipMemcpyDeviceToHost, st));
        IVX_HIP(ctx, hipStreamSynchronize(st));
        if (((const u32 *)(ctx->h_scalars + 32))[HDR_BADKEY]) return ctx->fail(IVX_ERR_INVALID, "build key id >= n_keys");
        q_lds = lb_try && ((const u32 *)(ctx->h_scalars + 32))[HDR_LBUILD] != 0;
        q_global = !q_lds;
        guard.armed = true;
    }
    if (q_lds)
        hipLaunchKernelGGL(k_lbuild_tiles, dim3(lb_tiles), dim3(LB_T), 0, tail_st, key, s, e, n, nkeys, (const i32 *)origin, (const u32 *)kreg, hdr,
                           (ivx_ent *)cellid, rank, lb_tstride(lb_tiles), binstart, maxcells + 1);
    else
        IVX_HIP(ctx, hipMemsetAsync(binstart, 0, (maxcells + 1) * sizeof(u32), tail_st));
    if (q_global) {
        hipLaunchKernelGGL(k_join_count, dim3(grid), dim3(BT), 0, tail_st, key, s, e, n, nkeys, origin, lbase, hdr, binstart, cellid, rank);
        const hipStream_t keep = ctx->stream;
        ctx->stream = tail_st;
        const ivx_status sst = ivx_scan_exclusive_u32(ctx, binstart, maxcells + 1, hdr + HDR_LBUILD);
        ctx->stream = keep;
        IVX_TRY(sst);
        hipLaunchKernelGGL(k_join_scatter, dim3(grid), dim3(BT), 0, tail_st, s, e, n, (const u32 *)binstart, (const u32 *)cellid, (const u32 *)rank, ent, (const u32 *)hdr);
    }
    if (q_lds) {
        const u32 rgrid = regcap - 1 < IVX_MAXREG_WIDE ? (u32)(regcap - 1) : (u32)IVX_MAXREG_WIDE;
        hipLaunchKernelGGL(k_lbuild_regions, dim3(rgrid), dim3(LB_T), 0, tail_st, (const i32 *)origin, (const u32 *)span, (const u32 *)lbase, (const u32 *)kreg,
                           (const u32 *)rkey, (const u32 *)hdr, nkeys, (const ivx_ent *)cellid, (const u32 *)rank, lb_tiles, lb_tstride(lb_tiles), binstart, ent);
    }
    hipLaunchKernelGGL(k_join_regdesc, dim3((u32)((regcap + 255) / 256)), dim3(256), 0, tail_st, origin, span, lbase, hdr, kreg, rkey, binstart, rdesc);
    IVX_HIP(ctx, hipGetLastError());
    if (overlap) {
        if (ix->ready == nullptr) IVX_HIP(ctx, hipEventCreateWithFlags(&ix->ready, hipEventDisableTiming));
        IVX_HIP(ctx, hipEventRecord(ix->ready, ctx->aux));
        IVX_HIP(ctx, hipEventRecord(ctx->tail_ev, ctx->aux));
        ctx->tail_pending = true;
        ix->jv_fast_unknown = true;
    }
    if (want_route) IVX_TRY(ivx_route_view_build(ctx, ix, origin, span, kcnt));

    if (!overlap) {
        IVX_HIP(ctx, hipMemcpyAsync(ctx->h_scalars + 32, hdr, HDR_WORDS * sizeof(u32), hipMemcpyDeviceToHost, st));
        IVX_HIP(ctx, hipStreamSynchronize(st));
    }
    if (((const u32 *)(ctx->h_scalars + 32))[HDR_BADKEY]) return ctx->fail(IVX_ERR_INVALID, "build key id >= n_keys");
    ix->jv_nreg = ((const u32 *)(ctx->h_scalars + 32))[HDR_NREG];
    ix->jv_filter = ((const u32 *)(ctx->h_scalars + 32))[HDR_FG] != 0xFFFFFFFFu;
    ix->jv_pk24 = ((const u32 *)(ctx->h_scalars + 32))[HDR_PK24] != 0;
    ix->jv_fast = ((const u32 *)(ctx->h_scalars + 32))[HDR_SLOW] == 0 && ix->jv_nreg > 0;
    if (want_route) ivx_route_view_ready(ctx, ix);
    guard.armed = false;

    ix->jv.origin = origin; ix->jv.span = span; ix->jv.kcnt = kcnt; ix->jv.lbase = lbase;
    ix->jv.binstart = binstart; ix->jv.ent = ent; ix->jv.hdr = hdr; ix->jv.nkeys = nkeys;
    ix->jv.kreg = kreg; ix->jv.rkey = rkey; ix->jv.rdesc = rdesc;
    ix->jv.fbits = fbits; ix->jv.fbase = fbase;
    return IVX_OK;
}

ivx_status ivx_join_probe(ivx_ctx *ctx, const JoinIndexView &jv, int mode,
                          const u32 *key, const i32 *s, const i32 *e, u64 n,
                          u32 *per_row, u8 *exists, u32 *ob, u32 *op, u64 cap, u64 *d_cursor)
{
    if (n == 0) return IVX_OK;
    unsigned long long *cur = (unsigned long long *)d_cursor;
    const bool small = n <= (1u << 18);
    const u32 grid = small ? (u32)((n + PT - 1) / PT) : ivx_stream_grid(n, PTILE, 256 * 8);
#define IVX_PROBE_LAUNCH(M_) do { \
        if (small) hipLaunchKernelGGL((k_probe_overlap<M_, 1>), dim3(grid), dim3(PT), 0, ctx->stream, jv, key, s, e, n, per_row, exists, ob, op, cap, cur, (const u32 *)nullptr); \
        else hipLaunchKernelGGL((k_probe_overlap<M_, PI>), dim3(grid), dim3(PT), 0, ctx->stream, jv, key, s, e, n, per_row, exists, ob, op, cap, cur, (const u32 *)nullptr); \
    } while (0)
    switch (mode) {
    case JP_COUNT: IVX_PROBE_LAUNCH(JP_COUNT); break;
    case JP_PER_ROW: IVX_PROBE_LAUNCH(JP_PER_ROW); break;
    case JP_EXISTS: IVX_PROBE_LAUNCH(JP_EXISTS); break;
    default: IVX_PROBE_LAUNCH(JP_FILL); break;
    }
#undef IVX_PROBE_LAUNCH
    IVX_HIP(ctx, hipGetLastError());
    return IVX_OK;
}
```

datafusion-bio-functions_amd/csrc/ivx_ops32.hip:

```cpp
#include <cstdlib>
#include <cstring>
#include "ivx_grid.hpp"
#include "ivx_runs.hpp"
#include "ivx_scan.hpp"
#include "ivx_sort.hpp"

namespace {

constexpr int OT = 256;
constexpr u32 SIGN = 0x80000000u;

__device__ __forceinline__ i32 wadd(i32 a, i32 b) { return (i32)((u32)a + (u32)b); }
__device__ __forceinline__ i32 wsub(i32 a, i32 b) { return (i32)((u32)a - (u32)b); }

ivx_status check_keyflag(ivx_ctx *ctx)
{
    u32 *errflag = (u32 *)(ctx->d_scalars + 8);
    IVX_HIP(ctx, hipMemcpyAsync(ctx->h_scalars + 8, errflag, sizeof(u64), hipMemcpyDeviceToHost, ctx->stream));
    IVX_HIP(ctx, hipStreamSynchronize(ctx->stream));
    if (*(u32 *)(ctx->h_scalars + 8)) return ctx->fail(IVX_ERR_INVALID, "build key id >= n_keys");
    return IVX_OK;
}


// ... 699 lines not shown
        IVX_TRY(ctx->get_scratch(WS_T4, n * sizeof(i64), (void **)&rs));
        IVX_TRY(ctx->get_scratch(WS_T8, n * sizeof(i64), (void **)&re));
        ivx_runs_out ro{rk, rs, re, nullptr};
        IVX_TRY(ivx_merge_runs(ctx, ks, ss, es, n, 0, 0, ro, &m));
    }
    IVX_HIP(ctx, hipMemcpyAsync(ctx->h_scalars + 8, flags, sizeof(u64), hipMemcpyDeviceToHost, st));
    IVX_HIP(ctx, hipStreamSynchronize(st));
    const u32 *hf = (const u32 *)(ctx->h_scalars + 8);
    if (hf[0]) return ctx->fail(IVX_ERR_INVALID, "build key id >= n_keys");
    if (hf[1]) return ctx->fail(IVX_ERR_UNSUPPORTED, "coverage: a build interval has end < start (the reference's result for it is unspecified)");
    i32 *nfirst, *nlast; u64 *pw;
    IVX_TRY(ivx_index_alloc(ctx, ix, (m ? m : 1) * sizeof(i32), (void **)&nfirst));
    IVX_TRY(ivx_index_alloc(ctx, ix, (m ? m : 1) * sizeof(i32), (void **)&nlast));
    IVX_TRY(ivx_index_alloc(ctx, ix, (m + 1) * sizeof(u64), (void **)&pw));
    hipLaunchKernelGGL(k_nodes, dim3(grid1(m + 1)), dim3(OT), 0, st, (const i64 *)rs, (const i64 *)re, m, nfirst, nlast, pw);
    IVX_TRY(ivx_scan_exclusive_u64(ctx, pw, m + 1));
    IVX_TRY(ivx_grid_build(ctx, ix, rk, nfirst, m, nkeys, &ix->cv.first, true));
    IVX_TRY(ivx_grid_build(ctx, ix, rk, nlast, m, nkeys, &ix->cv.last, true));
    ix->cv.nfirst = nfirst; ix->cv.nlast = nlast; ix->cv.pw = (const i64 *)pw;
    IVX_HIP(ctx, hipGetLastError());
    IVX_TRY(build_route_view(ctx, ix, ix->cv.first));
    IVX_TRY(ivx_join_build(ctx, ix, rk, nfirst, nlast, m));
    route_view_ready(ctx, ix);
    ix->flags |= IVX_IXF_REGION_ROWVAL;
    return IVX_OK;
}

ivx_status ivx_nearest_build(ivx_ctx *ctx, ivx_index *ix, const u32 *key, const i32 *s, const i32 *e, u64 n)
{
    hipStream_t st = ctx->stream;
    const u32 nkeys = ix->nkeys;
    IVX_HIP(ctx, hipMemsetAsync(ctx->d_scalars + 8, 0, sizeof(u64), st));
    const u64 na = n ? n : 1;
    ivx_nrec *rs, *re; u32 *ks;
    IVX_TRY(ivx_index_alloc(ctx, ix, na * sizeof(ivx_nrec), (void **)&rs));
    IVX_TRY(ivx_index_alloc(ctx, ix, na * sizeof(ivx_nrec), (void **)&re));
    IVX_TRY(ctx->get_scratch(WS_T0, na * 4, (void **)&ks));
    IVX_TRY(nearest_sorted_records(ctx, key, s, e, n, nkeys, ks, rs, re));
    if (n) {
        SegMaxIn in{ks, rs}; SegMaxOut out{rs};
        IVX_TRY((ivxscan::inclusive_f<SegMaxOp>(ctx, in, out, n)));
    }
    IVX_TRY(ivx_grid_build(ctx, ix, ks, &rs->a, n, nkeys, &ix->nv.by_start, true, 4));
    IVX_TRY(ivx_grid_build(ctx, ix, ks, &re->a, n, nkeys, &ix->nv.by_end, true, 4));
    IVX_TRY(ivx_grid_build(ctx, ix, ks, &rs->pmax, n, nkeys, &ix->nv.pmax, true, 4));
    ix->nv.rs = rs; ix->nv.re = re;
    IVX_TRY(build_route_view(ctx, ix, ix->nv.by_start));
    IVX_HIP(ctx, hipGetLastError());
    IVX_TRY(check_keyflag(ctx));
    route_view_ready(ctx, ix);
    return IVX_OK;
}


static bool rowval_routed_wanted(const ivx_index *ix, u64 n)
{
    if (ix->nroute_nreg == 0) return false;
    const char *f = getenv("IVX_ROWVAL_PATH");
    if (f && !strcmp(f, "routed")) return true;
    if (f) return false;
    return n >= (1u << 21);
}

static ivx_status rowval_routed(ivx_ctx *ctx, const ivx_index *ix, bool coverage, const u32 *key, const i32 *s, const i32 *e, u64 n, int strict, i64 *out)
{
    hipStream_t st = ctx->stream;
    ivx_routed R;
    IVX_TRY(ivx_route_rows(ctx, ix->nroute, key, s, e, n, strict ? 1u : 0u, &R));
    i64 *vd;
    IVX_TRY(ctx->get_scratch(WS_T3, n * sizeof(i64), (void **)&vd));
    const u32 grid = (ivx_stream_grid(n, OT * 4) + 7u) & ~7u;
    if (coverage) hipLaunchKernelGGL((k_rowval_routed<true>), dim3(grid), dim3(OT), 0, st, ix->gs, ix->ge, ix->cv, ix->nroute.rkey, ix->nroute_nreg, R.se, R.rfirst, R.nblk, vd, R.unsorted);
    else hipLaunchKernelGGL((k_rowval_routed<false>), dim3(grid), dim3(OT), 0, st, ix->gs, ix->ge, ix->cv, ix->nroute.rkey, ix->nroute_nreg, R.se, R.rfirst, R.nblk, vd, R.unsorted);
    IVX_TRY(ivx_unroute_pair(ctx, R, n, nullptr, vd, nullptr, nullptr, out, 0));
    if (coverage) hipLaunchKernelGGL(k_probe_coverage, dim3(ivx_stream_grid(n, OT * 4)), dim3(OT), 0, st, ix->cv, key, s, e, n, strict, out, R.unsorted);
    else hipLaunchKernelGGL(k_probe_count, dim3(ivx_stream_grid(n, OT * 4)), dim3(OT), 0, st, ix->gs, ix->ge, key, s, e, n, strict, out, R.unsorted);
    IVX_HIP(ctx, hipGetLastError());
    return IVX_OK;
}

ivx_status ivx_count_probe(ivx_ctx *ctx, const ivx_index *ix, const u32 *key, const i32 *s, const i32 *e, u64 n, int strict, i64 *out)
{
    if (n == 0) return IVX_OK;
    if (rowval_regions_wanted(ix, n)) return ivx_rowval_probe_regions(ctx, ix->jv, ix->jv_nreg, IVX_RV_COUNT, key, s, e, n, strict, out, nullptr, ix->jv_filter, ix->jv_pk24, ix->jv_fast);
    if (rowval_routed_wanted(ix, n)) return rowval_routed(ctx, ix, false, key, s, e, n, strict, out);
    hipLaunchKernelGGL(k_probe_count, dim3(ivx_stream_grid(n, OT)), dim3(OT), 0, ctx->stream, ix->gs, ix->ge, key, s, e, n, strict, out, (const u32 *)nullptr);
    IVX_HIP(ctx, hipGetLastError());
    return IVX_OK;
}

ivx_status ivx_coverage_probe(ivx_ctx *ctx, const ivx_index *ix, const u32 *key, const i32 *s, const i32 *e, u64 n, int strict, i64 *out)
{
    if (n == 0) return IVX_OK;
    if (rowval_regions_wanted(ix, n)) return ivx_rowval_probe_regions(ctx, ix->jv, ix->jv_nreg, IVX_RV_COVERAGE, key, s, e, n, strict, out, nullptr, ix->jv_filter, ix->jv_pk24, ix->jv_fast);
    if (rowval_routed_wanted(ix, n)) return rowval_routed(ctx, ix, true, key, s, e, n, strict, out);
    hipLaunchKernelGGL(k_probe_coverage, dim3(ivx_stream_grid(n, OT)), dim3(OT), 0, ctx->stream, ix->cv, key, s, e, n, strict, out, (const u32 *)nullptr);
    IVX_HIP(ctx, hipGetLastError());
    return IVX_OK;
}

ivx_status ivx_nearest_probe(ivx_ctx *ctx, const ivx_index *ix, const u32 *key, const i32 *s, const i32 *e, u64 n,
                             int strict, u32 k, int include_overlaps, u32 *ob, u32 *op, i64 *od, u64 cap, u64 *rows)
{
    *rows = 0;
    if (n == 0) return IVX_OK;
    hipStream_t st = ctx->stream;
    if (k <= 1) {
        if (cap < n) { *rows = n; return ctx->fail(IVX_ERR_CAPACITY, "nearest: output buffers too small"); }
        bool routed = ix->nroute_nreg > 0 && n >= (1u << 21);
        if (const char *f = getenv("IVX_NEAREST_PATH")) routed = !strcmp(f, "routed") ? ix->nroute_nreg > 0 : (!strcmp(f, "direct") ? false : routed);
        if (k == 1 && routed) {
            ivx_routed R;
            IVX_TRY(ivx_route_rows(ctx, ix->nroute, key, s, e, n, strict ? 1u : 0u, &R));
            u32 *vb; i64 *vd = nullptr;
            IVX_TRY(ctx->get_scratch(WS_T2, n * sizeof(u32), (void **)&vb));
            if (od) IVX_TRY(ctx->get_scratch(WS_T3, n * sizeof(i64), (void **)&vd));
            const int pmax_first = getenv("IVX_NEAREST_PMAX_FIRST") ? atoi(getenv("IVX_NEAREST_PMAX_FIRST")) : 1;
            hipLaunchKernelGGL(k_nearest_routed, dim3((ivx_stream_grid(n, NR_T * 4, 1280u) + 7u) & ~7u), dim3(NR_T), 0, st, ix->nv, ix->nroute.rkey, ix->nroute_nreg, R.se,
                               R.rfirst, R.nblk, strict ? 1u : 0u, include_overlaps, vb, vd, R.unsorted, pmax_first);
            IVX_TRY(ivx_unroute_pair(ctx, R, n, vb, vd, ob, op, od, -1));
            hipLaunchKernelGGL(k_probe_nearest1, dim3(ivx_stream_grid(n, OT * 4)), dim3(OT), 0, st, ix->nv, key, s, e, n, strict, include_overlaps, ob, op, od, R.unsorted);
        } else if (k == 1) {
            hipLaunchKernelGGL(k_probe_nearest1, dim3(ivx_stream_grid(n, OT)), dim3(OT), 0, st, ix->nv, key, s, e, n, strict, include_overlaps, ob, op, od, (const u32 *)nullptr);
        } else {
            u32 *cnt; u64 *offs;
            IVX_TRY(ctx->get_scratch(WS_T3, n * sizeof(u32), (void **)&cnt));
            IVX_TRY(ctx->get_scratch(WS_T4, (n + 1) * sizeof(u64), (void **)&offs));
            IVX_HIP(ctx, hipMemsetAsync(cnt, 0, n * sizeof(u32), st));
            hipLaunchKernelGGL(k_rows_of, dim3(grid1(n + 1)), dim3(OT), 0, st, (const u32 *)cnt, n, offs);
            IVX_TRY(ivx_scan_exclusive_u64(ctx, offs, n + 1));
            hipLaunchKernelGGL(k_nearest_emit, dim3(ivx_stream_grid(n, OT)), dim3(OT), 0, st, n, 1u, (const u32 *)cnt, (const i64 *)nullptr, (const u32 *)cnt, (const u64 *)offs, cap, ob, op, od);
        }
        IVX_HIP(ctx, hipGetLastError());
        *rows = n;
        return IVX_OK;
    }
    u32 *tmp, *cnt; u64 *offs; i64 *tmpd = nullptr;
    IVX_TRY(ctx->get_scratch(WS_T2, n * (u64)k * sizeof(u32), (void **)&tmp));
    if (od) IVX_TRY(ctx->get_scratch(WS_T5, n * (u64)k * sizeof(i64), (void **)&tmpd));
    IVX_TRY(ctx->get_scratch(WS_T3, n * sizeof(u32), (void **)&cnt));
    IVX_TRY(ctx->get_scratch(WS_T4, (n + 1) * sizeof(u64), (void **)&offs));
    hipLaunchKernelGGL(k_probe_nearestk, dim3(ivx_stream_grid(n, OT * 2)), dim3(OT), 0, st, ix->nv, key, s, e, n, strict, include_overlaps, k, tmp, tmpd, cnt);
    hipLaunchKernelGGL(k_rows_of, dim3(grid1(n + 1)), dim3(OT), 0, st, (const u32 *)cnt, n, offs);
    IVX_TRY(ivx_scan_exclusive_u64(ctx, offs, n + 1));
    IVX_HIP(ctx, hipMemcpyAsync(ctx->h_scalars + 3, offs + n, sizeof(u64), hipMemcpyDeviceToHost, st));
    IVX_HIP(ctx, hipStreamSynchronize(st));
    const u64 total = ctx->h_scalars[3];
    *rows = total;
    if (total > cap) return ctx->fail(IVX_ERR_CAPACITY, "nearest: output buffers too small");
    hipLaunchKernelGGL(k_nearest_emit, dim3(ivx_stream_grid(n, OT * 2)), dim3(OT), 0, st, n, k, (const u32 *)tmp, (const i64 *)tmpd, (const u32 *)cnt, (const u64 *)offs, cap, ob, op, od);
    IVX_HIP(ctx, hipGetLastError());
    return IVX_OK;
}
```

datafusion-bio-functions_amd/csrc/ivx_regions.hpp:

```cpp
#pragma once
#include <type_traits>
#include <cstdlib>
#include <cstring>
#include "ivx_join.hpp"

__host__ __device__ __forceinline__ u32 pk_maxlen(u32 rowbits) { const u32 spare = rowbits >= 32 ? 0u : 32u - rowbits; return (1u << (8u + (spare > 8u ? 8u : spare))) - 1u; }
struct PkRow { u32 rel, len, hi; };
__device__ __forceinline__ PkRow pk_unpack(u64 w, u32 rowbits)
{
    const u32 lo32 = (u32)w, hi32 = (u32)(w >> 32);
    return PkRow{lo32 & 0xFFFFFFu, (lo32 >> 24) | ((rowbits < 32 ? (hi32 >> rowbits) & 0xFFu : 0u) << 8), hi32};
}

template <class W, class Miss>
__device__ __forceinline__ W *routed_word(const PageTab &pt, W *pool, u32 r, u32 v, Miss &&miss)
{
    u32 pg = pt.ptab[(u64)r * pt.pstride + (v >> pt.lgpg)];
    if (pg == 0u) { pg = 1u; miss(); }
    return pool + (((u64)(pg - 1u) << pt.lgpg) + (v & ((1u << pt.lgpg) - 1u)));
}

constexpr int RP_T = 1024;
constexpr int RP_W = RP_T / IVX_WAVE;
constexpr u32 FP_CHUNK = (u32)RP_W * IVX_WAVE * 8u;

struct FpRest { u32 r, first, cnt, pad; };
__host__ __device__ __forceinline__ u64 fp_max_batches(u64 n, u32 nreg) { return ((n >> 13) + nreg + 1) * (u64)(RP_W * 8); }

template <class F> inline void with_bools(F &&f) { f(); }
template <class F, class... B> inline void with_bools(F &&f, bool b, B... rest)
{
    if (b) with_bools([&](auto... t) { f(std::true_type{}, t...); }, rest...);
    else with_bools([&](auto... t) { f(std::false_type{}, t...); }, rest...);
}
#define IVX_B(tag) (decltype(tag)::value)

ivx_status ivx_route_flat(ivx_ctx *ctx, const JoinIndexView &jv, const u32 *key, const i32 *s, const i32 *e, u64 n, u32 adj,
                          u32 ndig, bool ids16, u32 max_tiles, ivx_routed *R);
struct ivx_paged_opts { bool filter, packed, rowval, lean; u32 adj; u64 *zero2 = nullptr; };
ivx_status ivx_route_paged(ivx_ctx *ctx, const JoinIndexView &jv, u32 nreg, const u32 *key, const i32 *s, const i32 *e, u64 n,
                           const ivx_paged_opts &o, ivx_routed *R);
ivx_status ivx_route_two_level(ivx_ctx *ctx, const JoinIndexView &jv, u32 nreg, const u32 *key, const i32 *s, const i32 *e, u64 n, ivx_routed *R);
ivx_status ivx_unroute_values(ivx_ctx *ctx, const ivx_routed &R, u32 nreg, int kind, const u32 *val, u64 n, void *out, u64 *d_total, int sorted_done = 0);
```

datafusion-bio-functions_amd/csrc/ivx_regions_probe.hip:

```cpp
#include "ivx_regions.hpp"

namespace {


#ifndef IVX_RP_B
#define IVX_RP_B 8
#endif
#ifndef IVX_RP_RING
#define IVX_RP_RING 512
#endif
#ifndef IVX_RP_ECAP
#define IVX_RP_ECAP 6144
#endif
constexpr int RP_B = IVX_RP_B;
constexpr u32 RP_HALO = IVX_RP_HALO;
constexpr u32 RP_CCAP = 8192 + RP_HALO + 2;
constexpr u32 RP_ECAP = IVX_RP_ECAP;
constexpr u32 RP_RING = IVX_RP_RING;
constexpr u32 RP_NSLOT = 4;
constexpr u32 RP_NPG = 64;
constexpr u32 RP_STASH = 48;
constexpr u32 FD_SLOT_SHIFT = 13;
#ifndef IVX_FD_HEAD
#define IVX_FD_HEAD 3
// ... 414 lines not shown
                            prel[PK ? q : 0] = w.rel; plen[PK ? q : 0] = w.len;
                            qs[q] = (i32)((u32)S.rbase + w.rel); qe[q] = (i32)((u32)qs[q] + w.len); rowv[q] = w.hi & rowmask;
                            nxr[q] = w.len;
                        } else { qs[q] = (i32)(u32)nx[q]; qe[q] = (i32)(u32)(nx[q] >> 32); rowv[q] = nxr[q]; }
                        if (!nfull && b0 + (u64)q * (RP_W * IVX_WAVE) + ln < c_hi) okmask |= 1u << q;
                    }
                    if (nfull) okmask = (1u << B) - 1u;
                    const bool cfull = nfull;
                    cat0 = nat0;
                    if (PK) {
                        u32 esc = 0;
#pragma unroll
                        for (int q = 0; q < B; q++) if (((okmask >> q) & 1u) && nxr[q] == maxlen) esc |= 1u << q;
                        relmask = okmask & ~esc;
                        if (__any(esc != 0)) {
                            i32 ts[B], te[B];
#pragma unroll
                            for (int q = 0; q < B; q++) { const u32 rr = ((esc >> q) & 1u) ? rowv[q] : 0u; ts[q] = ps_in[rr]; te[q] = pe_in[rr]; }
#pragma unroll
                            for (int q = 0; q < B; q++) if ((esc >> q) & 1u) { qs[q] = (i32)((u32)ts[q] + adj); qe[q] = (i32)((u32)te[q] - adj); }
                        }
                    }
                    nfull = prefetch(r0 + (u64)RP_W * WB, b0 + (u64)RP_W * WB);
                    if (MODE >= RV_COUNT) {
                        u32 val[B];
                        if constexpr (PK) batch_rowval<MODE, B, true>(S, qs, qe, okmask, val, (const u32 (&)[B])prel, (const u32 (&)[B])plen, relmask);
                        else batch_rowval<MODE, B, false>(S, qs, qe, okmask, val, (const u32 (&)[B])qs, (const u32 (&)[B])qs, 0u);
#pragma unroll
                        for (int q = 0; q < B; q++) {
                            if (!((okmask >> q) & 1u)) continue;
                            const u64 i = b0 + (u64)q * (RP_W * IVX_WAVE) + ln;
                            if (PAGED) {
                                const u64 at = cfull ? cat0 + (u64)q * (RP_W * IVX_WAVE) : row_at(i, r, rf);
                                ((u64 *)ob)[at] = (u64)val[q] | ((u64)rowv[q] << 32);
                            } else ob[i] = val[q];
                        }
                        continue;
                    }
                    u32 start = 0;
                    bool direct = false;
                    u32 got;
                    if constexpr (PK) got = batch_walk<FILL, B, true>(S, L, qs, qe, rowv, okmask, wv, pend_start, start, direct, (const u32 (&)[B])prel, (const u32 (&)[B])plen, relmask);
                    else got = batch_walk<FILL, B, false>(S, L, qs, qe, rowv, okmask, wv, pend_start, start, direct, (const u32 (&)[B])qs, (const u32 (&)[B])qs, 0u);
                    if (MODE == 0) { wcur += got; continue; }
                    round_publish(L, got, round, wv, cursor);
                    if (direct) {
                        bool fits;
                        const u64 g = round_wait(L, round, wv, cap, fits);
                        batch_write_direct<B>(S, L, qs, qe, rowv, okmask, wv, g, fits, ob, op);
                        start += got; got = 0;
                    }
                    if (round) round_copy_out(L, pend_mine, pend_start, round - 1, wv, ob, op, cap);
                    pend_mine = got; pend_start = start; round++;
                }
                lo = c_hi;
                if (PAGED && lo < hi && lo < rend) r--;
            }
        }
        if (MODE == 0) {
            const u64 tot = wave_sum(wcur);
            if (ln == 0 && tot) atomicAdd(cursor, (unsigned long long)tot);
        }
    }
    if (FILL && round) round_copy_out(L, pend_mine, pend_start, round - 1, wv, ob, op, cap);
}


template <int B, class W>
struct LeanRows {
    static constexpr u32 WB = IVX_WAVE * B;
    static constexpr u32 SUB = 8u / B;
    const u32 *s_cfirst, *rcur; PageTab pt; W *pool;
    u32 rowbits, maxlen, wv, ln, nreg, c_lo, nbatch;
    u32 r, first, cnt; W *src; u64 nx[B];
    struct Batch { u32 first, cnt; W *src; };

    __device__ __forceinline__ bool init(const JoinIndexView &ix, u32 *s_cf, const u32 *cfirst, const u32 *rcur_, const PageTab &pt_, W *pool_, u32 rowbits_)
    {
        s_cfirst = s_cf; rcur = rcur_; pt = pt_; pool = pool_; rowbits = rowbits_; maxlen = pk_maxlen(rowbits_);
        wv = __builtin_amdgcn_readfirstlane(threadIdx.x / IVX_WAVE); ln = lane_id();
        nreg = ix.hdr[HDR_NREG];
        for (u32 t = threadIdx.x; t <= nreg; t += RP_T) s_cf[t] = cfirst[t];
        __syncthreads();
        const u32 nchunk = s_cf[nreg];
        c_lo = (u32)((u64)nchunk * blockIdx.x / gridDim.x);
        const u32 c_hi = (u32)((u64)nchunk * (blockIdx.x + 1) / gridDim.x);
        nbatch = (c_hi - c_lo) * SUB;
        return c_lo < c_hi;
    }
    template <class Miss>
    __device__ __forceinline__ void start(Miss &&miss)
    {
        {
            u32 a = 0, b = nreg;
            while (a < b) { const u32 m = (a + b + 1) >> 1; if (s_cfirst[m] <= c_lo) a = m; else b = m - 1; }
            r = a;
        }
        src = pool;
        prefetch(0, miss);
    }
    template <class Miss>
    __device__ __forceinline__ void prefetch(u32 i, Miss &&miss)
    {
        const u32 c = c_lo + i / SUB, sb = i % SUB;
        while (c >= s_cfirst[r + 1]) r++;
        first = (c - s_cfirst[r]) * FP_CHUNK + wv * (8u * IVX_WAVE) + sb * WB;
        const u32 rows = rcur[r];
        cnt = rows > first ? (rows - first < WB ? rows - first : WB) : 0u;
        if (cnt) {
            src = routed_word(pt, pool, r, first, miss);
#pragma unroll
            for (int q = 0; q < B; q++) nx[q] = src[q * IVX_WAVE + ln];
        }
    }
    template <class Miss>
    __device__ __forceinline__ Batch take(u32 i, u32 (&rel)[B], u32 (&len)[B], u32 (&hi)[B], Miss &&miss)
    {
        const Batch b{first, cnt, src};
#pragma unroll
        for (int q = 0; q < B; q++) { const PkRow w = pk_unpack(nx[q], rowbits); rel[q] = w.rel; len[q] = w.len; hi[q] = w.hi; }
        if (i + 1 < nbatch) prefetch(i + 1, miss);
        return b;
    }
};

template <int B, bool FULL>
__device__ __forceinline__ void lean_cells_of(const Slice &S, const u32 (&rel)[B], const u32 (&len)[B], u32 maxlen, u32 cnt, u32 ln,
                                              u32 (&ca)[B], u32 (&cb)[B], u32 &slow, u32 &okm)
{
    const u32 sh0 = S.sh0, off = S.off, cmax = S.cmax, ncm1 = S.ncm1;
#pragma unroll
    for (int q = 0; q < B; q++) {
        const u32 t = ((rel[q] + 1u) >> sh0) + off;
        const u32 bl0 = (t > 1u ? t : 1u) - 1u;
        const u32 bh0 = ((rel[q] + len[q]) >> sh0) + off;
        const u32 bh = bh0 < cmax ? bh0 : cmax;
        bool bad = len[q] == maxlen || bh >= ncm1;
        const bool ok = FULL || (u32)q * IVX_WAVE + ln < cnt;
        if (ok && bad) slow |= 1u << q;
        if (ok && !bad) okm |= 1u << q;
        bad |= !ok;
        const u32 e1 = bad ? 0u : bh + 1u;
        const u32 bl = bl0 < e1 ? bl0 : e1;
        ca[q] = S.s_off[bl];
        cb[q] = S.s_off[e1];
    }
}
template <int B>
__device__ __forceinline__ void lean_cells(const Slice &S, const u32 (&rel)[B], const u32 (&len)[B], u32 maxlen, u32 cnt, u32 ln,
                                           u32 (&ca)[B], u32 (&cb)[B], u32 &slow, u32 &okm)
{
    slow = 0; okm = 0;
    if (cnt == IVX_WAVE * B) lean_cells_of<B, true>(S, rel, len, maxlen, cnt, ln, ca, cb, slow, okm);
    else lean_cells_of<B, false>(S, rel, len, maxlen, cnt, ln, ca, cb, slow, okm);
}

template <int B>
__device__ __forceinline__ void lean_list_slow(u32 slow, u32 r, u32 first, u32 ln, u64 *__restrict__ rest_rows, u32 *rest_n)
{
#pragma unroll
    for (int q = 0; q < B; q++)
        if ((slow >> q) & 1u) rest_rows[atomicAdd(rest_n + 1, 1u)] = (u64)(first + (u32)q * IVX_WAVE + ln) | ((u64)r << 32);
}

template <class W> struct RestRow { W *slot; u32 row, hi; i32 qs, qe; };
template <class W, class Miss>
__device__ __forceinline__ RestRow<W> rest_row(const JoinIndexView &ix, const PageTab &pt, W *pool, u32 r, u32 v, u32 rowbits,
                                               const i32 *ps_in, const i32 *pe_in, u32 adj, Miss &&miss)
{
    W *slot = routed_word(pt, pool, r, v, miss);
    const PkRow w = pk_unpack(*slot, rowbits);
    const u32 row = w.hi & (rowbits >= 32 ? 0xFFFFFFFFu : (1u << rowbits) - 1u);
    i32 qs, qe;
    if (w.len == pk_maxlen(rowbits)) { qs = (i32)((u32)ps_in[row] + adj); qe = (i32)((u32)pe_in[row] - adj); }
    else { qs = (i32)((u32)ix.rdesc[r].rbase + w.rel); qe = (i32)((u32)qs + w.len); }
    return RestRow<W>{slot, row, w.hi, qs, qe};
}

template <int B, bool DRAIN>
__global__ __launch_bounds__(RP_T) void k_fill_fast(JoinIndexView ix, const u64 *__restrict__ pool, const u32 *__restrict__ rcur,
                                                    const u32 *__restrict__ cfirst, PageTab pt, u32 *__restrict__ ob, u32 *__restrict__ op, u64 cap,
                                                    unsigned long long *cursor, const u32 *bsel, u32 rowbits, FpRest *__restrict__ rest, u64 *__restrict__ rest_rows, u32 *rest_n,
                                                    u32 drain)
{
    if (bsel != nullptr && *bsel != (u32)B) return;
    if (ix.hdr[HDR_SLOW] != 0u) return;
    IVX_PROBE_LDS(true)
    __shared__ u32 s_cfirst[IVX_MAXREG_WIDE + 2];
    __shared__ u32 s_wat[RP_NSLOT][RP_W];
    __shared__ u32 s_stash[DRAIN ? RP_W : 1][RP_STASH];
    const u32 wv = __builtin_amdgcn_readfirstlane(threadIdx.x / IVX_WAVE), ln = lane_id();
    auto miss = [&]() { if (ln == 0) atomicOr((unsigned int *)(cursor + 1), 1u); };
    LeanRows<B, const u64> rows;
    if (!rows.init(ix, s_cfirst, cfirst, rcur, pt, pool, rowbits)) return;
    Slice S;
    slice_init(ix, S, L);
    rows.start(miss);
    const u32 rowmask = rowbits >= 32 ? 0xFFFFFFFFu : (1u << rowbits) - 1u;
    u32 loaded_r = 0xFFFFFFFFu;
    u32 round = 0;
    u32 pend_mine = 0;
    constexpr u32 HALF = RP_RING / 2;
    auto copy_out = [&](u32 pr) {
        const u32 sl = pr % RP_NSLOT;
        while (__hip_atomic_load(&L.s_ready[sl], __ATOMIC_ACQUIRE, __HIP_MEMORY_SCOPE_WORKGROUP) != pr + 1u) __builtin_amdgcn_s_sleep(1);
        if (!pend_mine) return;
        const u64 base = L.s_base[sl];
        const u32 tot = s_wat[sl][RP_W - 1] + L.s_wcnt[sl][RP_W - 1];
        if (base + tot > cap) return;
        const u64 g = base + s_wat[sl][wv];
        u32 *ob_w = ob + g, *op_w = op + g;
        const uint2 *half = (const uint2 *)L.s_q[wv] + (pr & 1u) * HALF;
        for (u32 t = ln; t < pend_mine; t += IVX_WAVE) {
            const uint2 x = half[t];
            ob_w[t] = L.s_row[x.x]; op_w[t] = x.y & rowmask;
        }
    };
    for (u32 i = 0; i < rows.nbatch; i++) {
        const u32 r = rows.r;
        if (r != loaded_r) {
            if (round) { copy_out(round - 1u); pend_mine = 0; }
            slice_load(ix, S, L, r, true);
            loaded_r = r;
        }
        u32 rel[B], len[B], roww[B];
        const auto bt = rows.take(i, rel, len, roww, miss);
        const u32 first = bt.first, cnt = bt.cnt;
        const i32 rbase = S.rbase;
        u32 ca[B], cb[B], slow, okm;
        lean_cells<B>(S, rel, len, rows.maxlen, cnt, ln, ca, cb, slow, okm);
        u32 wpos = 0;
        uint2 *half = (uint2 *)L.s_q[wv] + (round & 1u) * HALF;
        auto step = [&](u32 &j, u32 jend, i32 qs, i32 qe, u32 rw, u64 &actm) {
            const u64 x = L.s_ent[j];
            const u64 mm = actm & __builtin_amdgcn_sicmp((i32)(u32)x, qe, 41 ) & __builtin_amdgcn_sicmp((i32)(u32)(x >> 32), qs, 39 );
            if (__builtin_amdgcn_inverse_ballot_w64(mm)) half[mask_rank_from(mm, wpos) & (HALF - 1)] = make_uint2(j, rw);
            wpos += (u32)__popcll(mm);
            j++;
            actm = __builtin_amdgcn_uicmp(j, jend, 36 );
        };
        u32 sfill = 0;
#pragma unroll
        for (int q = 0; q < B; q++) {
            const i32 qs = (i32)((u32)rbase + rel[q]), qe = (i32)((u32)qs + len[q]);
            u32 j = ca[q];
            const u32 jend = cb[q];
            u64 actm = __builtin_amdgcn_uicmp(j, jend, 36);
            if constexpr (!DRAIN) {
                if (actm != 0) {
                    do step(j, jend, qs, qe, roww[q], actm); while (actm != 0);
                }
            } else {
                const u32 lim = drain < RP_STASH - sfill ? drain : RP_STASH - sfill;
                if ((u32)__popcll(actm) > lim) {
#pragma unroll
                    for (int h = 0; h < FD_HEAD; h++) step(j, jend, qs, qe, roww[q], actm);
                    while ((u32)__popcll(actm) > lim) step(j, jend, qs, qe, roww[q], actm);
                }
                if (actm != 0) {
                    if (__builtin_amdgcn_inverse_ballot_w64(actm)) s_stash[wv][mask_rank_from(actm, sfill)] = j | (((u32)q * IVX_WAVE + ln) << FD_SLOT_SHIFT);
                    sfill += (u32)__popcll(actm);
                }
            }
        }
        if (DRAIN && sfill != 0) {
            __builtin_amdgcn_fence(__ATOMIC_RELEASE, "wavefront");
            __builtin_amdgcn_wave_barrier();
            __builtin_amdgcn_fence(__ATOMIC_ACQUIRE, "wavefront");
            const bool has = ln < sfill;
            const u32 e = has ? s_stash[wv][ln] : 0u;
            const PkRow w = pk_unpack(bt.src[e >> FD_SLOT_SHIFT], rowbits);
            const i32 qs = (i32)((u32)rbase + w.rel), qe = (i32)((u32)qs + w.len);
            const u32 bh0 = ((w.rel + w.len) >> S.sh0) + S.off;
            u32 j = e & ((1u << FD_SLOT_SHIFT) - 1u);
            const u32 jend = has ? (u32)S.s_off[(bh0 < S.cmax ? bh0 : S.cmax) + 1u] : 0u;
            u64 actm = __builtin_amdgcn_uicmp(j, jend, 36);
            while (actm != 0) step(j, jend, qs, qe, w.hi, actm);
        }
        u32 got = wpos;
        const bool skip = got > HALF;
        if (__builtin_expect(skip, 0)) {
            if (ln < B && ln * IVX_WAVE < cnt) rest[atomicAdd(rest_n, 1u)] = FpRest{r, first + ln * IVX_WAVE, cnt - ln * IVX_WAVE < IVX_WAVE ? cnt - ln * IVX_WAVE : (u32)IVX_WAVE, 0u};
            got = 0;
        } else if (__builtin_expect(slow != 0, 0)) lean_list_slow<B>(slow, r, first, ln, rest_rows, rest_n);
        if (ln == 0) {
            const u32 sl = round % RP_NSLOT;
            L.s_wcnt[sl][wv] = got;
            const u32 before = __hip_atomic_fetch_add(&L.s_arrive[sl], 1u, __ATOMIC_ACQ_REL, __HIP_MEMORY_SCOPE_WORKGROUP);
            if (before == RP_W - 1) {
                u32 tot = 0;
#pragma unroll
                for (int w = 0; w < RP_W; w++) { s_wat[sl][w] = tot; tot += L.s_wcnt[sl][w]; }
                L.s_base[sl] = tot ? atomicAdd(cursor, (unsigned long long)tot) : 0ull;
                __hip_atomic_store(&L.s_arrive[sl], 0u, __ATOMIC_RELAXED, __HIP_MEMORY_SCOPE_WORKGROUP);
                __hip_atomic_store(&L.s_ready[sl], round + 1u, __ATOMIC_RELEASE, __HIP_MEMORY_SCOPE_WORKGROUP);
            }
        }
        if (round) copy_out(round - 1u);
        pend_mine = got; round++;
    }
    if (round) copy_out(round - 1u);
}

__global__ __launch_bounds__(256) void k_fill_rest(JoinIndexView ix, const u64 *__restrict__ pool, PageTab pt, const FpRest *__restrict__ rest,
                                                   const u64 *__restrict__ rest_rows, const u32 *__restrict__ rest_n, u32 *__restrict__ ob,
                                                   u32 *__restrict__ op, u64 cap, unsigned long long *cursor, const i32 *__restrict__ ps_in,
                                                   const i32 *__restrict__ pe_in, u32 rowbits)
{
    const u32 nbat = rest_n[0], nrow = rest_n[1];
    if (nbat == 0 && nrow == 0) return;
    const u32 wpb = blockDim.x / IVX_WAVE, ln = lane_id();
    const u32 sh0 = ix.hdr[HDR_SH0], nlev = ix.hdr[HDR_NLEV];
    auto rows64 = [&](bool ok, u32 r, u32 v) {
        i32 qs = 0, qe = -1; u32 row = 0, k = 0;
        if (ok) {
            const auto e = rest_row(ix, pt, pool, r, v, rowbits, ps_in, pe_in, 0u, [&]() { atomicOr((unsigned int *)(cursor + 1), 1u); });
            qs = e.qs; qe = e.qe; row = e.row;
            k = ix.rkey[r];
        }
        u32 m = 0;
        if (ok) walk(ix, sh0, 0, nlev, k, qs, qe, [&](u32) { m++; });
        const u32 inc = wave_incl_scan(m);
        const u32 tot = __shfl(inc, IVX_WAVE - 1, IVX_WAVE);
        if (tot == 0) return;
        unsigned long long g = 0;
        if (ln == 0) g = atomicAdd(cursor, (unsigned long long)tot);
        g = __shfl(g, 0, IVX_WAVE);
        if (g + tot > cap) return;
        u64 at = g + inc - m;
        if (m) walk(ix, sh0, 0, nlev, k, qs, qe, [&](u32 brow) { ob[at] = brow; op[at] = row; at++; });
    };
    const u32 wave = blockIdx.x * wpb + threadIdx.x / IVX_WAVE, nwave = gridDim.x * wpb;
    for (u32 i0 = wave * IVX_WAVE; i0 < nrow; i0 += nwave * IVX_WAVE) {
        const bool ok = i0 + ln < nrow;
        const u64 e = ok ? rest_rows[i0 + ln] : 0ull;
        rows64(ok, (u32)(e >> 32), (u32)e);
    }
    for (u32 b = wave; b < nbat; b += nwave) {
        const FpRest w = rest[b];
        for (u32 t0 = 0; t0 < w.cnt; t0 += IVX_WAVE) rows64(t0 + ln < w.cnt, w.r, w.first + t0 + ln);
    }
}

#ifndef IVX_RV_WPS
#define IVX_RV_WPS 4
#endif
#ifndef IVX_RV_B
#define IVX_RV_B 8
#endif
template <int KIND, int B>
__global__ __launch_bounds__(RP_T, IVX_RV_WPS) void k_rv_fast(JoinIndexView ix, u64 *__restrict__ pool, const u32 *__restrict__ rcur, const u32 *__restrict__ cfirst,
                                                  PageTab pt, u32 rowbits, u64 *__restrict__ rest_rows, u32 *rest_n)
{
    __shared__ unsigned short s_off[RP_CCAP];
    __shared__ u64 s_ent[RP_ECAP];
    __shared__ u32 s_cfirst[IVX_MAXREG_WIDE + 2];
    ProbeLds L{s_off, s_ent, nullptr, nullptr, nullptr, nullptr, nullptr, nullptr, nullptr};
    const u32 ln = lane_id();
    auto miss = []() {};
    LeanRows<B, u64> rows;
    if (!rows.init(ix, s_cfirst, cfirst, rcur, pt, pool, rowbits)) return;
    Slice S;
    slice_init(ix, S, L);
    rows.start(miss);
    u32 loaded_r = 0xFFFFFFFFu;
    for (u32 i = 0; i < rows.nbatch; i++) {
        const u32 r = rows.r;
        if (r != loaded_r) { slice_load(ix, S, L, r, true); loaded_r = r; }
        u32 rel[B], len[B], roww[B];
        const auto bt = rows.take(i, rel, len, roww, miss);
        u64 *dst = bt.src;
        const i32 rbase = S.rbase;
        u32 ca[B], cb[B], slow, okm;
        lean_cells<B>(S, rel, len, rows.maxlen, bt.cnt, ln, ca, cb, slow, okm);
#pragma unroll
        for (int q = 0; q < B; q++) {
            const i32 qs = (i32)((u32)rbase + rel[q]), qe = (i32)((u32)qs + len[q]);
            const i32 ca1 = rv_wadd(qe, 1), cb1 = rv_wsub(qs, 1);
            u32 v = 0;
            for (u32 j = ca[q]; j < cb[q]; j++) {
                const u64 x = s_ent[j];
                const i32 xs = (i32)(u32)x, xe = (i32)(u32)(x >> 32);
                if (xs <= qe && xe >= qs) {
                    if (KIND == RV_COVERAGE) { const i32 d = rv_wsub(ca1 < xe ? ca1 : xe, cb1 > xs ? cb1 : xs); v = (u32)rv_wadd((i32)v, d > 1 ? d : 1); }
                    else v++;
                }
            }
            if ((okm >> q) & 1u) dst[q * IVX_WAVE + ln] = (u64)v | ((u64)roww[q] << 32);
        }
        if (__builtin_expect(slow != 0, 0)) lean_list_slow<B>(slow, r, bt.first, ln, rest_rows, rest_n);
    }
}

template <int KIND>
__global__ __launch_bounds__(256) void k_rv_rest(JoinIndexView ix, u64 *__restrict__ pool, PageTab pt, const u64 *__restrict__ rest_rows,
                                                 const u32 *__restrict__ rest_n, const i32 *__restrict__ ps_in, const i32 *__restrict__ pe_in,
                                                 u32 rowbits, u32 adj)
{
    const u32 nrow = rest_n[1];
    const u32 sh0 = ix.hdr[HDR_SH0], nlev = ix.hdr[HDR_NLEV];
    for (u32 i = blockIdx.x * blockDim.x + threadIdx.x; i < nrow; i += gridDim.x * blockDim.x) {
        const u64 ent = rest_rows[i];
        const u32 r = (u32)(ent >> 32);
        const auto e = rest_row(ix, pt, pool, r, (u32)ent, rowbits, ps_in, pe_in, adj, []() {});
        const i32 qs = e.qs, qe = e.qe;
        u32 v = 0;
        if (KIND == RV_COVERAGE) {
            const i32 a = rv_wadd(qe, 1), b = rv_wsub(qs, 1);
            walk_ent(ix, sh0, 0, nlev, ix.rkey[r], qs, qe, [&](const ivx_ent &n) {
                const i32 d = rv_wsub(a < n.e ? a : n.e, b > n.s ? b : n.s);
                v = (u32)rv_wadd((i32)v, d > 1 ? d : 1);
            });
        } else if (KIND != RV_COUNT || !(qe < qs)) {
            walk_ent(ix, sh0, 0, nlev, ix.rkey[r], qs, qe, [&](const ivx_ent &) { v++; });
        }
        *e.slot = (u64)v | ((u64)e.hi << 32);
    }
}

template <int B>
__global__ __launch_bounds__(RP_T, IVX_RV_WPS) void k_mark_fast(JoinIndexView ix, const u64 *__restrict__ pool, const u32 *__restrict__ rcur, const u32 *__restrict__ cfirst,
                                                    PageTab pt, u32 rowbits, u64 *__restrict__ rest_rows, u32 *rest_n, u32 *marks)
{
// ... 192 lines not shown
                    const u32 ncell = S.ncell0;
                    const i64 lo64 = (i64)qs - ((i64)1 << S.sh0) + 1 - (i64)S.origin;
                    const i64 bl = lo64 <= 0 ? 0 : (lo64 >> S.sh0);
                    if (bl < (i64)ncell) {
                        const u32 blo = (u32)bl;
                        const i64 bh = hi64 >> S.sh0;
                        const u32 bhi = bh >= (i64)ncell ? ncell - 1u : (u32)bh;
                        if (blo <= bhi) {
                            lds = S.inlds && blo >= S.slo && bhi < S.shi;
                            if (lds) { ja = S.s_off[blo - S.slo]; jb = S.s_off[bhi + 1 - S.slo]; }
                            else { ja = ix.binstart[S.lb + blo]; jb = ix.binstart[S.lb + bhi + 1]; }
                        }
                    }
                }
                const u32 la = lds ? ja : 0u, lb = lds ? jb : 0u, ga = lds ? 0u : ja, gb = lds ? 0u : jb;
                walk(la, lb, true);
                if (__any(ga < gb)) walk(ga, gb, false);
            }
            if (S.upper) {
                for (u32 l = 1; l < S.nlev; l++) {
                    if (ix.hdr[HDR_LEVCNT + l] == 0) continue;
                    const u32 sh = S.sh0 + IVX_LSTEP * l;
                    u32 ja = 0, jb = 0;
                    if (live) {
                        u32 blo = 0, bhi = 0; bool any = true;
                        if (sh < 32) {
                            const u32 ncell = (S.span >> sh) + 1u;
                            const i64 lo64 = (i64)qs - ((i64)1 << sh) + 1 - (i64)S.origin;
                            const i64 bl = lo64 <= 0 ? 0 : (lo64 >> sh);
                            const i64 bh = hi64 >> sh;
                            if (bl >= (i64)ncell) any = false;
                            else { blo = (u32)bl; bhi = bh >= (i64)ncell ? ncell - 1u : (u32)bh; if (blo > bhi) any = false; }
                        }
                        if (any) { const u32 lbase = ix.lbase[(u64)l * ix.nkeys + S.k]; ja = ix.binstart[lbase + blo]; jb = ix.binstart[lbase + bhi + 1]; }
                    }
                    if (__any(ja < jb)) walk(ja, jb, false);
                }
            }
        }
        lo = c_hi;
        if (PAGED && lo < hi && lo < rend) r--;
    }
}

struct RegionKnobs {
    bool two_pass;
    bool pack_off;
    bool lean_off;
    bool filter_off;
    const char *dense;
    const char *rp_rows;
    const char *fill_drain;
};
RegionKnobs region_knobs()
{
    auto is = [](const char *name, const char *v) { const char *x = getenv(name); return x && !strcmp(x, v); };
    return RegionKnobs{is("IVX_PART", "two"), is("IVX_PACK", "0"), is("IVX_FILL", "old"), is("IVX_FILTER", "0"), getenv("IVX_DENSE"), getenv("IVX_RP_ROWS"), getenv("IVX_FILL_DRAIN")};
}

int fill_rows_per_lane(const RegionKnobs &K, u64 cap, u64 n)
{
    if (K.rp_rows) return atoi(K.rp_rows);
    const double per_row = (double)cap / (double)n;
    return per_row <= 0.40 ? 8 : per_row <= 0.8 ? 4 : per_row <= 1.6 ? 2 : 1;
}

u32 fill_drain_of(const RegionKnobs &K, int b)
{
    if (K.fill_drain) { const int t = atoi(K.fill_drain); return t <= 0 ? 0u : (u32)t < RP_STASH ? (u32)t : RP_STASH; }
    return b == 8 ? 12u : b == 4 ? 16u : 0u;
}

bool dense_fill_wanted(const RegionKnobs &K, u64 cap, u64 n)
{
    if (K.dense) return atoi(K.dense) != 0;
    return (double)cap / (double)n > 3.5;
}

bool lean_rows_ok(const ivx_routed &R)
{
    return R.form == IVX_ROWS_PAGED && R.packed && R.pt.lgpg >= 13 && R.rest_rows != nullptr;
}

template <int V> using int_tag = std::integral_constant<int, V>;
template <class F> void with_rows_per_lane(int b, F &&f)
{
    switch (b) { case 1: f(int_tag<1>{}); break; case 2: f(int_tag<2>{}); break; case 4: f(int_tag<4>{}); break; default: f(int_tag<8>{}); }
}

template <int MODE, int B>
void launch_probe_regions(hipStream_t st, const JoinIndexView &jv, const ivx_routed &R, u32 grid, u32 *ob, u32 *op, u64 cap,
                          unsigned long long *cur, const u32 *bsel = nullptr, const u32 *only_if_set = nullptr)
{
    const u32 vpb = RP_VGRID / grid;
    if (R.form == IVX_ROWS_PAGED) {
        auto go = [&](auto pk) {
            hipLaunchKernelGGL((k_probe_regions<MODE, B, false, true, IVX_B(pk)>), dim3(grid), dim3(RP_T), 0, st, jv, (const void *)R.se, (const void *)R.ids, R.rfirst, 1u, vpb,
                               ob, op, cap, cur, 1u, R.adj, (const u32 *)nullptr, R.pt, bsel, R.ds, R.de, R.rowbits, only_if_set);
        };
        if constexpr (MODE >= RV_COUNT) go(std::true_type{}); else with_bools(go, R.packed);
        return;
    }
    hipLaunchKernelGGL((k_probe_regions<MODE, B, false>), dim3(grid), dim3(RP_T), 0, st, jv, (const void *)R.se, (const void *)R.ids, R.rfirst, R.nblk, vpb, ob, op, cap, cur, 1u, R.adj, R.unsorted);
    hipLaunchKernelGGL((k_probe_regions<MODE, B, true>), dim3(grid), dim3(RP_T), 0, st, jv, (const void *)R.ds, (const void *)R.de, R.rfirst, R.nblk, vpb, ob, op, cap, cur, 1u, R.adj, R.unsorted);
}

ivx_status dense_fill(ivx_ctx *ctx, const JoinIndexView &jv, u32 nreg, const ivx_routed &R, u64 n, u32 *ob, u32 *op, u64 cap, u64 *d_cursor)
{
    hipStream_t st = ctx->stream;
    const u64 slots = (n >> 6) + nreg + 3;
    u64 *pcount;
    IVX_TRY(ctx->get_scratch(WS_T3, slots * sizeof(u64), (void **)&pcount));
    IVX_HIP(ctx, hipMemsetAsync(pcount, 0, slots * sizeof(u64), st));
    auto pass = [&](auto pass_tag) {
        constexpr int P = decltype(pass_tag)::value;
        if (R.form == IVX_ROWS_PAGED) {
            with_bools([&](auto pk) {
                hipLaunchKernelGGL((k_probe_dense<P, false, true, IVX_B(pk)>), dim3(RP_VGRID), dim3(RP_T), 0, st, jv, (const void *)R.se, (const void *)R.ids, R.rfirst, 1u, 1u,
                                   (const u32 *)nullptr, pcount, ob, op, cap, R.pt, R.ds, R.de, R.rowbits);
            }, R.packed);
            return;
        }
        hipLaunchKernelGGL((k_probe_dense<P, false>), dim3(RP_VGRID), dim3(RP_T), 0, st, jv, (const void *)R.se, (const void *)R.ids, R.rfirst, R.nblk, 1u, R.unsorted, pcount, ob, op, cap);
        hipLaunchKernelGGL((k_probe_dense<P, true>), dim3(RP_VGRID), dim3(RP_T), 0, st, jv, (const void *)R.ds, (const void *)R.de, R.rfirst, R.nblk, 1u, R.unsorted, pcount, ob, op, cap);
    };
    pass(int_tag<0>{});
    IVX_TRY(ivx_scan_exclusive_u64(ctx, pcount, slots));
    IVX_HIP(ctx, hipMemcpyAsync(d_cursor, pcount + (slots - 1), sizeof(u64), hipMemcpyDeviceToDevice, st));
    pass(int_tag<1>{});
    IVX_HIP(ctx, hipGetLastError());
    return IVX_OK;
}

ivx_status probe_pairs(ivx_ctx *ctx, const JoinIndexView &jv, u32 nreg, int mode, const ivx_routed &R, u64 n, u32 *ob, u32 *op, u64 cap,
                       u64 *d_cursor, u64 hint, int fast, bool reused, const RegionKnobs &K)
{
    hipStream_t st = ctx->stream;
    unsigned long long *cur = (unsigned long long *)d_cursor;
    if (mode != JP_FILL) {
        launch_probe_regions<0, RP_B>(st, jv, R, RP_VGRID, ob, op, cap, cur);
        IVX_HIP(ctx, hipGetLastError());
        return IVX_OK;
    }
    if (dense_fill_wanted(K, hint, n)) return dense_fill(ctx, jv, nreg, R, n, ob, op, cap, d_cursor);
    const bool paged = R.form == IVX_ROWS_PAGED;
    u32 *bsel = paged && !R.all_routed ? (u32 *)(ctx->d_scalars + 11) : nullptr;
    if (bsel) hipLaunchKernelGGL(k_pick_rows, dim3(1), dim3(1), 0, st, R.rfirst, nreg, hint, K.rp_rows ? (u32)atoi(K.rp_rows) : 0u, bsel);
    auto every_b = [&](auto &&f) {
        if (bsel) { f(int_tag<8>{}); f(int_tag<4>{}); f(int_tag<2>{}); f(int_tag<1>{}); }
        else with_rows_per_lane(fill_rows_per_lane(K, hint, n), f);
    };
    const u32 *slow_gate = nullptr;
    if (lean_rows_ok(R) && fast != 0 && !K.lean_off && R.rest != nullptr) {
        u32 *rest_n = R.ctl->rest_n;
        if (reused) IVX_HIP(ctx, hipMemsetAsync(rest_n, 0, 2 * sizeof(u32), st));
        every_b([&](auto b) {
            const u32 drain = fill_drain_of(K, decltype(b)::value);
            with_bools([&](auto dr) {
                hipLaunchKernelGGL((k_fill_fast<decltype(b)::value, IVX_B(dr)>), dim3(RP_GRID), dim3(RP_T), 0, st, jv, R.se, (const u32 *)R.ctl->rcur, (const u32 *)R.ctl->cfirst, R.pt, ob, op, cap, cur,
                                   (const u32 *)bsel, R.rowbits, R.rest, R.rest_rows, rest_n, drain);
            }, drain != 0);
        });
        hipLaunchKernelGGL(k_fill_rest, dim3(512), dim3(256), 0, st, jv, R.se, R.pt, (const FpRest *)R.rest, (const u64 *)R.rest_rows, (const u32 *)rest_n, ob, op, cap, cur, R.ds, R.de, R.rowbits);
        IVX_HIP(ctx, hipGetLastError());
        if (fast == 1) return IVX_OK;
        slow_gate = jv.hdr + HDR_SLOW;
    }
    every_b([&](auto b) { launch_probe_regions<1, decltype(b)::value>(st, jv, R, RP_GRID, ob, op, cap, cur, bsel, slow_gate); });
    IVX_HIP(ctx, hipGetLastError());
    return IVX_OK;
}

}

ivx_status ivx_join_probe_regions(ivx_ctx *ctx, const JoinIndexView &jv, u32 nreg, int mode,
                                  const u32 *key, const i32 *s, const i32 *e, u64 n,
                                  u32 *ob, u32 *op, u64 cap, u64 *d_cursor, bool planned, bool has_filter, bool pk24, int fast, hipEvent_t ready, bool clear_cursor)
{
    auto wait_ready = [&]() -> ivx_status { if (ready) { IVX_HIP(ctx, hipStreamWaitEvent(ctx->stream, ready, 0)); ready = nullptr; } return IVX_OK; };
    const RegionKnobs K = region_knobs();
    const bool paged_route = !planned && n != 0 && nreg <= IVX_MAXREG_WIDE && !K.two_pass;
    if (clear_cursor && !paged_route) IVX_HIP(ctx, hipMemsetAsync(d_cursor, 0, 2 * sizeof(u64), ctx->stream));
    if (n == 0) return wait_ready();
    ivx_join_plan &pl = ctx->join_plan;
    ivx_routed R;
    if (planned) R = pl.rows;
    else {
        if (nreg > IVX_MAXREG_WIDE) {
            IVX_TRY(wait_ready());
            IVX_TRY(ivx_route_two_level(ctx, jv, nreg, key, s, e, n, &R));
        } else if (K.two_pass) {
            IVX_TRY(wait_ready());
            IVX_TRY(ivx_route_flat(ctx, jv, key, s, e, n, 0u, nreg > IVX_MAXREG ? 1024u : 256u, false, 4, &R));
        } else {
            IVX_TRY(ivx_route_paged(ctx, jv, nreg, key, s, e, n, ivx_paged_opts{has_filter && !K.filter_off, pk24 && !K.pack_off, false, fast != 0, 0u, clear_cursor ? d_cursor : nullptr}, &R));
        }
        if (mode == JP_COUNT) { pl.rows = R; pl.valid = true; }
    }
    IVX_TRY(wait_ready());
    const u64 hint = ctx->fill_hint ? ctx->fill_hint : (planned && pl.total < cap ? pl.total : cap);
    return probe_pairs(ctx, jv, nreg, mode, R, n, ob, op, cap, d_cursor, hint, fast, planned, K);
}

ivx_status ivx_rowval_probe_regions(ivx_ctx *ctx, const JoinIndexView &jv, u32 nreg, int kind,
                                    const u32 *key, const i32 *s, const i32 *e, u64 n, int strict, void *out, u64 *d_total,
                                    bool has_filter, bool pk24, bool fast)
{
    if (n == 0) return IVX_OK;
    if (nreg == 0 || nreg > IVX_MAXREG_WIDE) return ctx->fail(IVX_ERR_INVALID, "per-row region probe: one partition pass only");
    hipStream_t st = ctx->stream;
    const RegionKnobs K = region_knobs();
    const u32 adj = strict ? 1u : 0u;
    const bool paged = pk24 && nreg <= IVX_MAXREG && !K.two_pass && !K.pack_off;
    ivx_routed R;
    u32 *val = nullptr;
    if (paged) IVX_TRY(ivx_route_paged(ctx, jv, nreg, key, s, e, n, ivx_paged_opts{has_filter && !K.filter_off, true, true, fast && !K.lean_off, adj}, &R));
    else {
        IVX_TRY(ivx_route_flat(ctx, jv, key, s, e, n, adj, nreg > IVX_MAXREG ? 1024u : 256u, true, 2, &R));
        IVX_TRY(ctx->get_scratch(WS_T2, n * sizeof(u32), (void **)&val));
    }
    u64 *pool = const_cast<u64 *>(R.se);
    auto probe = [&](auto kind_tag) {
        constexpr int M = decltype(kind_tag)::value;
        if (lean_rows_ok(R)) {
            hipLaunchKernelGGL((k_rv_fast<M, IVX_RV_B>), dim3(RP_GRID * (IVX_RV_WPS / 4)), dim3(RP_T), 0, st, jv, pool, (const u32 *)R.ctl->rcur, (const u32 *)R.ctl->cfirst, R.pt, R.rowbits, R.rest_rows, R.ctl->rest_n);
            hipLaunchKernelGGL((k_rv_rest<M>), dim3(256), dim3(256), 0, st, jv, pool, R.pt, (const u64 *)R.rest_rows, (const u32 *)R.ctl->rest_n, s, e, R.rowbits, adj);
        } else launch_probe_regions<M, RP_B>(st, jv, R, RP_VGRID, paged ? (u32 *)pool : val, nullptr, 0, nullptr);
    };
    if (kind == IVX_RV_COVERAGE) probe(int_tag<RV_COVERAGE>{}); else if (kind == IVX_RV_COUNT) probe(int_tag<RV_COUNT>{}); else probe(int_tag<RV_MATCHES>{});
    IVX_HIP(ctx, hipGetLastError());
    return ivx_unroute_values(ctx, R, nreg, kind, val, n, out, d_total);
}

ivx_status ivx_mark_probe_regions(ivx_ctx *ctx, const JoinIndexView &jv, u32 nreg, const u32 *key, const i32 *s, const i32 *e, u64 n,
                                  u32 *marks, bool has_filter, bool pk24, bool fast, bool *took)
{
    *took = false;
    const RegionKnobs K = region_knobs();
    if (n == 0 || nreg == 0 || nreg > IVX_MAXREG || !pk24 || !fast || K.two_pass || K.pack_off || K.lean_off) return IVX_OK;
    hipStream_t st = ctx->stream;
    ivx_routed R;
    IVX_TRY(ivx_route_paged(ctx, jv, nreg, key, s, e, n, ivx_paged_opts{has_filter && !K.filter_off, true, true, true, 0u}, &R));
    if (!lean_rows_ok(R)) return IVX_OK;
    hipLaunchKernelGGL((k_mark_fast<IVX_RV_B>), dim3(RP_GRID * (IVX_RV_WPS / 4)), dim3(RP_T), 0, st, jv, R.se, (const u32 *)R.ctl->rcur, (const u32 *)R.ctl->cfirst, R.pt, R.rowbits,
                       R.rest_rows, R.ctl->rest_n, marks);
    hipLaunchKernelGGL(k_mark_rest, dim3(256), dim3(256), 0, st, jv, R.se, R.pt, (const u64 *)R.rest_rows, (const u32 *)R.ctl->rest_n, s, e, R.rowbits, marks);
    IVX_HIP(ctx, hipGetLastError());
    *took = true;
    return IVX_OK;
}
```

datafusion-bio-functions_amd/csrc/ivx_regions_route.hip:

```cpp
#include "ivx_regions.hpp"

namespace {


constexpr int PA_T = 1024;
#ifndef IVX_PA_I
#define IVX_PA_I 12
#endif
constexpr int PA_I = IVX_PA_I;
constexpr int PA_TILE = PA_T * PA_I;
constexpr u32 NO_REGION = 0xFFFFFFFFu;
constexpr u32 KT_MAX = 256;

struct KeyTab {
    bool lds;
    u32 nkeys, sh0, cs;
    u64 rmul;
};

__device__ __forceinline__ void keytab_load(const JoinIndexView &ix, i32 *s_origin, u32 *s_last, u32 *s_kreg, KeyTab &kt)
{
    kt.nkeys = ix.nkeys; kt.sh0 = ix.hdr[HDR_SH0]; kt.cs = ix.hdr[HDR_CS];
    kt.rmul = (u64)ix.hdr[HDR_RMUL_LO] | ((u64)ix.hdr[HDR_RMUL_HI] << 32);
    kt.lds = ix.nkeys <= KT_MAX;
// ... 762 lines not shown
static inline bool cols_aligned16(const u32 *key, const i32 *s, const i32 *e) { return (((uintptr_t)key | (uintptr_t)s | (uintptr_t)e) & 15) == 0; }
static constexpr u64 IN_COLS = (1ull << WS_IN_START) | (1ull << WS_IN_END);

ivx_status ivx_route_flat(ivx_ctx *ctx, const JoinIndexView &jv, const u32 *key, const i32 *s, const i32 *e, u64 n, u32 adj,
                          u32 ndig, bool ids16, u32 max_tiles, ivx_routed *R)
{
    hipStream_t st = ctx->stream;
    const u32 chunk = part_chunk(n, max_tiles);
    const u32 nblk = (u32)((n + chunk - 1) / chunk);
    const u64 nh = (u64)ndig * nblk + 1;
    u32 *hist; u64 *pse; void *ids;
    IVX_TRY(ctx->get_scratch(WS_SORTHIST, nh * sizeof(u32), (void **)&hist));
    IVX_TRY(ctx->get_scratch(WS_T0, n * sizeof(u64), (void **)&pse));
    IVX_TRY(ctx->get_scratch(WS_T1, n * (ids16 ? sizeof(unsigned short) : sizeof(u32)), &ids));
    u32 *unsorted = (u32 *)(ctx->d_scalars + 10);
    IVX_HIP(ctx, hipMemsetAsync(hist + (nh - 1), 0, sizeof(u32), st));
    IVX_HIP(ctx, hipMemsetAsync(unsorted, 0, sizeof(u32), st));
    ivx_status scan = IVX_OK;
    with_bools([&](auto vec, auto wide, auto i16) {
        constexpr int ND = IVX_B(wide) ? 1024 : 256;
        using RowT = typename std::conditional<IVX_B(i16), unsigned short, u32>::type;
        hipLaunchKernelGGL((k_part_hist<IVX_B(vec), ND>), dim3(nblk), dim3(PA_T), 0, st, jv, key, s, n, nblk, chunk, hist, adj, unsorted);
        if ((scan = ivx_scan_exclusive_u32(ctx, hist, nh)) != IVX_OK) return;
        hipLaunchKernelGGL((k_part_scatter<IVX_B(vec), RowT, ND>), dim3(nblk), dim3(PA_T), 0, st, jv, key, s, e, n, nblk, (const u32 *)hist, pse, (RowT *)ids, chunk, adj, (const u32 *)unsorted);
    }, cols_aligned16(key, s, e), ndig > 256, ids16);
    IVX_TRY(scan);
    IVX_HIP(ctx, hipGetLastError());
    *R = ivx_routed{};
    R->form = IVX_ROWS_FLAT; R->se = pse; R->rfirst = hist; R->nblk = nblk; R->chunk = chunk; R->ndig = ndig; R->unsorted = unsorted;
    if (ids16) R->cidx = (const unsigned short *)ids; else R->ids = (const u32 *)ids;
    R->ds = s; R->de = e; R->adj = adj;
    R->slots = (1ull << WS_SORTHIST) | (1ull << WS_T0) | (1ull << WS_T1) | IN_COLS;
    return IVX_OK;
}

ivx_status ivx_route_paged(ivx_ctx *ctx, const JoinIndexView &jv, u32 nreg, const u32 *key, const i32 *s, const i32 *e, u64 n,
                           const ivx_paged_opts &o, ivx_routed *R)
{
    hipStream_t st = ctx->stream;
    const bool wide = nreg > IVX_MAXREG;
    const bool half = o.packed && !wide;
    const u32 tile = wide ? PA_T * 8u : half ? 512u * 16u : PA_T * 12u;
    u32 rowbits = 1;
    while (rowbits < 32 && (n - 1) >> rowbits) rowbits++;
    if (o.filter) rowbits = 32;
    u32 lgpg = 14;
    while (lgpg < 31 && (n >> lgpg) > 4096) lgpg++;
    const u64 pstride = (n >> lgpg) + 2;
    const u64 npages = (n >> lgpg) + nreg + 1;
    const u64 ntiles = (n + tile - 1) / tile;
    ivx_route_ctl *ctl; u32 *ptab; u64 *pool; u32 *prow = nullptr; uint2 *vtab = nullptr; void *rest = nullptr;
    *R = ivx_routed{};
    R->slots = (1ull << WS_SORTHIST) | (1ull << WS_T0) | (1ull << WS_T1) | (1ull << WS_T2) | IN_COLS;
    IVX_TRY(ctx->get_scratch(WS_SORTHIST, sizeof(ivx_route_ctl), (void **)&ctl));
    IVX_TRY(ctx->get_scratch(WS_T2, (size_t)nreg * pstride * sizeof(u32), (void **)&ptab));
    IVX_TRY(ctx->get_scratch(WS_T0, (size_t)(npages << lgpg) * sizeof(u64), (void **)&pool));
    if (o.rowval) IVX_TRY(ctx->get_scratch(WS_T1, (size_t)ntiles * 256 * sizeof(uint2), (void **)&vtab));
    else if (!o.packed) IVX_TRY(ctx->get_scratch(WS_T1, (size_t)(npages << lgpg) * sizeof(u32), (void **)&prow));
    else if (o.lean) IVX_TRY(ctx->get_scratch(WS_T1, (size_t)fp_max_batches(n, nreg) * sizeof(FpRest) + (size_t)(n + 64) * sizeof(u64), &rest));
    if (rest) { R->rest = (FpRest *)rest; R->rest_rows = (u64 *)(R->rest + fp_max_batches(n, nreg)); }
    if (o.rowval && o.lean) { IVX_TRY(ctx->get_scratch(WS_T3, (size_t)(n + 64) * sizeof(u64), (void **)&R->rest_rows)); R->slots |= 1ull << WS_T3; }
    {
        const u32 nctl = (u32)(offsetof(ivx_route_ctl, rfirst) / sizeof(u32));
        const u64 nptab = (u64)nreg * pstride;
        u64 cg = (nptab / 4 + 256 * 8 - 1) / (256 * 8);
        cg = cg < (nctl + 255) / 256 ? (nctl + 255) / 256 : (cg > 1024 ? 1024 : cg);
        hipLaunchKernelGGL(k_route_clear, dim3((u32)cg), dim3(256), 0, st, (u32 *)ctl, nctl, ptab, nptab, o.zero2);
    }
    const PageTab pt{ptab, (u32)pstride, lgpg};
    u32 tiles = n >= (16u << 20) ? 4u : n >= (4u << 20) ? 2u : 1u;
    if (const char *tenv = getenv("IVX_PART_TILES"))
        if ((tenv[0] == '1' || tenv[0] == '2' || tenv[0] == '4' || tenv[0] == '8') && tenv[1] == 0) tiles = (u32)(tenv[0] - '0');
    const u32 chunk1 = tile * tiles;
    const u32 nblk1 = (u32)((n + chunk1 - 1) / chunk1);
    with_bools([&](auto vec, auto klds, auto filt, auto pk) {
        auto part = [&](auto kern, u32 threads) {
            hipLaunchKernelGGL(kern, dim3(nblk1), dim3(threads), 0, st, jv, key, s, e, n, chunk1, ctl->rcur, pt, &ctl->pool_next, pool, prow, rowbits, o.adj, vtab);
        };
        if (half) part(k_part_onepass<IVX_B(vec), 256, 16, IVX_B(klds), IVX_B(filt), true, 512>, 512u);
        else if (wide) part(k_part_onepass<IVX_B(vec), 1024, 8, IVX_B(klds), IVX_B(filt), IVX_B(pk)>, (u32)PA_T);
        else part(k_part_onepass<IVX_B(vec), 256, 12, IVX_B(klds), IVX_B(filt), IVX_B(pk)>, (u32)PA_T);
    }, cols_aligned16(key, s, e), jv.nkeys <= KT_MAX, o.filter, o.packed);
    if (o.rowval && !o.lean) hipLaunchKernelGGL(k_page_bounds, dim3(1), dim3(1024), 0, st, (const u32 *)ctl->rcur, nreg, ctl->rfirst);
    else hipLaunchKernelGGL(k_chunk_bounds, dim3(1), dim3(1024), 0, st, (const u32 *)ctl->rcur, nreg, ctl->rfirst, ctl->cfirst);
    IVX_HIP(ctx, hipGetLastError());
    R->form = IVX_ROWS_PAGED; R->se = pool; R->ids = prow; R->rfirst = ctl->rfirst; R->pt = pt; R->packed = o.packed; R->rowbits = rowbits;
    R->all_routed = !o.filter; R->ctl = ctl; R->vtab = vtab; R->ds = s; R->de = e; R->adj = o.adj;
    return IVX_OK;
}

ivx_status ivx_route_two_level(ivx_ctx *ctx, const JoinIndexView &jv, u32 nreg, const u32 *key, const i32 *s, const i32 *e, u64 n, ivx_routed *R)
{
    hipStream_t st = ctx->stream;
    u32 *unsorted = (u32 *)(ctx->d_scalars + 10);
    const u32 G = (nreg + IVX_MAXREG_WIDE - 1) / IVX_MAXREG_WIDE;
    if (G > P2_SUBMAX) return ctx->fail(IVX_ERR_INVALID, "overlap index with too many probe regions");
    const u32 nsuper = (nreg + G - 1) / G;
    const uint2 split = make_uint2(G, (u32)(((1ull << 32) + G - 1) / G));
    const u32 chunk = part_chunk(n);
    const u32 nblk1 = (u32)((n + chunk - 1) / chunk);
    const u64 nh1 = (u64)1024 * nblk1 + 1;
    const u32 grid2 = (u32)(n / PA_TILE) + nsuper + 1;
    const u64 nh2 = (u64)G * grid2 + 1;
    u32 *hist1, *hist2, *tprefix, *prow1, *rfirst, *prow2; u64 *pse1, *pse2; unsigned char *sub1;
    IVX_TRY(ctx->get_scratch(WS_SORTHIST, nh1 * sizeof(u32), (void **)&hist1));
    IVX_TRY(ctx->get_scratch(WS_T0, n * sizeof(u64), (void **)&pse1));
    IVX_TRY(ctx->get_scratch(WS_T1, n * sizeof(u32), (void **)&prow1));
    IVX_TRY(ctx->get_scratch(WS_T2, n, (void **)&sub1));
    IVX_TRY(ctx->get_scratch(WS_SA0, n * sizeof(u64), (void **)&pse2));
    IVX_TRY(ctx->get_scratch(WS_SA1, n * sizeof(u32), (void **)&prow2));
    IVX_TRY(ctx->get_scratch(WS_T4, ((size_t)nsuper + 1) * sizeof(u32), (void **)&tprefix));
    IVX_TRY(ctx->get_scratch(WS_T5, nh2 * sizeof(u32), (void **)&hist2));
    IVX_TRY(ctx->get_scratch(WS_T6, ((size_t)nreg + 1) * sizeof(u32), (void **)&rfirst));
    IVX_HIP(ctx, hipMemsetAsync(hist1 + (nh1 - 1), 0, sizeof(u32), st));
    IVX_HIP(ctx, hipMemsetAsync(hist2, 0, nh2 * sizeof(u32), st));
    IVX_HIP(ctx, hipMemsetAsync(unsorted, 0, sizeof(u32), st));
    ivx_status scan = IVX_OK;
    with_bools([&](auto vec) {
        hipLaunchKernelGGL((k_part_hist<IVX_B(vec), 1024, true>), dim3(nblk1), dim3(PA_T), 0, st, jv, key, s, n, nblk1, chunk, hist1, 0u, unsorted, split);
        if ((scan = ivx_scan_exclusive_u32(ctx, hist1, nh1)) != IVX_OK) return;
        hipLaunchKernelGGL((k_part_scatter<IVX_B(vec), u32, 1024, true>), dim3(nblk1), dim3(PA_T), 0, st, jv, key, s, e, n, nblk1, (const u32 *)hist1, pse1, prow1, chunk, 0u, (const u32 *)unsorted, split, sub1);
    }, cols_aligned16(key, s, e));
    IVX_TRY(scan);
    hipLaunchKernelGGL(k_p2_layout, dim3(1), dim3(1024), 0, st, (const u32 *)hist1, nblk1, nsuper, tprefix, (const u32 *)unsorted);
    hipLaunchKernelGGL(k_p2_hist, dim3(grid2), dim3(PA_T), 0, st, (const unsigned char *)sub1, (const u32 *)hist1, nblk1, nsuper, (const u32 *)tprefix, G, hist2, (const u32 *)unsorted);
    IVX_TRY(ivx_scan_exclusive_u32(ctx, hist2, nh2));
    hipLaunchKernelGGL(k_p2_scatter, dim3(grid2), dim3(PA_T), 0, st, (const unsigned char *)sub1, (const u64 *)pse1, (const u32 *)prow1, (const u32 *)hist1, nblk1, nsuper,
                       (const u32 *)tprefix, G, (const u32 *)hist2, pse2, prow2, (const u32 *)unsorted);
    const u32 bgrid = (nreg + 1 + WR_T - 1) / WR_T;
    hipLaunchKernelGGL(k_p2_bounds, dim3(bgrid), dim3(WR_T), 0, st, nreg, G, nsuper, (const u32 *)hist1, nblk1, nh1, (const u32 *)tprefix, (const u32 *)hist2, rfirst, (const u32 *)unsorted);
    hipLaunchKernelGGL(k_sorted_bounds, dim3(bgrid), dim3(WR_T), 0, st, jv, key, s, n, nreg, rfirst, (const u32 *)unsorted);
    IVX_HIP(ctx, hipGetLastError());
    *R = ivx_routed{};
    R->form = IVX_ROWS_TABLE; R->se = pse2; R->ids = prow2; R->rfirst = rfirst; R->unsorted = unsorted; R->ds = s; R->de = e;
    R->slots = IN_COLS;
    for (int slot : {WS_SORTHIST, WS_T0, WS_T1, WS_T2, WS_SA0, WS_SA1, WS_T4, WS_T5, WS_T6}) R->slots |= 1ull << slot;
    return IVX_OK;
}

ivx_status ivx_unroute_values(ivx_ctx *ctx, const ivx_routed &R, u32 nreg, int kind, const u32 *val, u64 n, void *out, u64 *d_total, int sorted_done)
{
    hipStream_t st = ctx->stream;
    auto go = [&](auto out_tag) {
        constexpr int O = decltype(out_tag)::value;
        if (R.form == IVX_ROWS_PAGED) {
            constexpr u32 TILE = 512u * 16u;
            hipLaunchKernelGGL((k_unpermute_paged<O, (int)TILE>), dim3((u32)((n + TILE - 1) / TILE)), dim3(512), 0, st, R.se, R.vtab, R.pt, nreg, R.rowbits, n, out, (unsigned long long *)d_total);
        } else with_bools([&](auto wide) {
            constexpr int ND = IVX_B(wide) ? 1024 : 256;
            hipLaunchKernelGGL((k_unpermute<O, ND>), dim3(R.nblk), dim3(PA_T), 0, st, val, R.cidx, R.rfirst, R.nblk, R.chunk, (u32)ND, n, out, R.unsorted, (unsigned long long *)d_total, sorted_done);
        }, R.ndig > 256);
    };
    switch (kind) {
    case IVX_RV_COVERAGE: go(std::integral_constant<int, UP_I64S>{}); break;
    case IVX_RV_COUNT: go(std::integral_constant<int, UP_I64>{}); break;
    case IVX_RV_PER_ROW: go(std::integral_constant<int, UP_U32>{}); break;
    default: go(std::integral_constant<int, UP_U8>{}); break;
    }
    IVX_HIP(ctx, hipGetLastError());
    return IVX_OK;
}

ivx_status ivx_route_rows(ivx_ctx *ctx, const JoinIndexView &rv, const u32 *key, const i32 *s, const i32 *e, u64 n, u32 adj, ivx_routed *out)
{
    return ivx_route_flat(ctx, rv, key, s, e, n, adj, 1024, true, 1, out);
}

ivx_status ivx_unroute_u32(ivx_ctx *ctx, const ivx_routed &r, u64 n, const u32 *vb, u32 *out32, u8 *out8)
{
    if (out32) IVX_TRY(ivx_unroute_values(ctx, r, 1024u, IVX_RV_PER_ROW, vb, n, out32, nullptr, 1));
// ... 11 lines not shown
```

Measured before the change: 35.46 billion overlap-pairs/s.

## Mirror build header and fill totals into mapped host memory to cut sync copies

Makes the host scalar buffer mapped and coherent, so kernels write the join header and the fill totals straight into host memory with system-scope stores. This drops the device-to-host memcpy calls. The overlapped-build path now waits on the ready event and reads the slow flag from the mirror, which resolves the fast/slow choice before the fill, and the fill-rest kernel has its last block publish the totals. The chunk-bounds kernel is deferred and launched only on fill paths that need it, and the filter launch is moved after the header check. In exchange the code adds an extra host sync on the ready event and relies on coherent host-visible stores from the device.

```diff
diff --git a/datafusion-bio-functions_amd/csrc/ivx_capi.hip b/datafusion-bio-functions_amd/csrc/ivx_capi.hip
--- a/datafusion-bio-functions_amd/csrc/ivx_capi.hip
+++ b/datafusion-bio-functions_amd/csrc/ivx_capi.hip
@@ -231,8 +231,10 @@
               hipEventCreateWithFlags(&c->tail_ev, hipEventDisableTiming) == hipSuccess &&
               hipEventCreate(&c->ev0) == hipSuccess && hipEventCreate(&c->ev1) == hipSuccess &&
               hipMalloc((void **)&c->d_scalars, 64 * sizeof(u64)) == hipSuccess &&
-              hipHostMalloc((void **)&c->h_scalars, 64 * sizeof(u64), hipHostMallocDefault) == hipSuccess;
+              hipHostMalloc((void **)&c->h_scalars, IVX_HS_WORDS * sizeof(u64), hipHostMallocMapped | hipHostMallocCoherent) == hipSuccess &&
+              hipHostGetDevicePointer((void **)&c->hd_scalars, c->h_scalars, 0) == hipSuccess;
     if (!ok) { ivx_ctx_free(c); return IVX_ERR_HIP; }
+    memset(c->h_scalars, 0, IVX_HS_WORDS * sizeof(u64));
     c->stream = c->own_stream;
     if (const char *e = getenv("IVX_BUILD_OVERLAP")) c->overlap = e[0] == '1';
     *out = c;
@@ -475,24 +477,27 @@
     IVX_TRY(stage_out(ctx, mem, WS_OUT_D, pidx, cap, &d_p));
     const bool defer_clear = regions && !planned;
     if (!defer_clear) IVX_HIP(ctx, hipMemsetAsync(ctx->d_scalars, 0, 2 * sizeof(u64), ctx->stream));
+    ivx_probe_note note;
+    note.ix_serial = ix->serial;
     {
         KernelTimer t(ctx);
         if (regions) {
             if (!planned) pl.valid = false;
             const ivx_status st = ivx_join_probe_regions(ctx, ix->jv, ix->jv_nreg, mode, dk, ds, de, n, d_b, d_p, cap, ctx->d_scalars, planned, ix->jv_filter, ix->jv_pk24,
-                                                         ix->jv_fast_unknown ? 2 : (ix->jv_fast ? 1 : 0), planned ? nullptr : ix->ready, defer_clear);
+                                                         ix->jv_lean.load(std::memory_order_relaxed), planned ? nullptr : ix->ready, defer_clear, &note);
+            if (note.fast >= 0) ix->jv_lean.store(note.fast, std::memory_order_relaxed);
             if (st != IVX_OK) { pl.valid = false; return st; }
             if (mode == JP_COUNT && pl.valid) { memcpy(pl.in, in, sizeof(in)); pl.mem = mem; pl.n = n; pl.ix = ix; pl.ix_serial = ix->serial; pl.stream = ctx->stream; }
         }
         else if (rowval) IVX_TRY(ivx_rowval_probe_regions(ctx, ix->jv, ix->jv_nreg, mode == JP_PER_ROW ? IVX_RV_PER_ROW : IVX_RV_EXISTS, dk, ds, de, n, 0,
-                                                          mode == JP_PER_ROW ? (void *)d_row : (void *)d_ex, ctx->d_scalars, ix->jv_filter, ix->jv_pk24, ix->jv_fast && !ix->jv_fast_unknown));
+                                                          mode == JP_PER_ROW ? (void *)d_row : (void *)d_ex, ctx->d_scalars, ix->jv_filter, ix->jv_pk24, ix->jv_lean.load(std::memory_order_relaxed) == 1));
         else if (n && (mode == JP_PER_ROW || mode == JP_EXISTS) && ix->nroute_nreg > 0 && rowval_routed_ok(n))
             IVX_TRY(ivx_join_rowval_routed(ctx, ix, mode, dk, ds, de, n, d_row, d_ex, ctx->d_scalars));
         else IVX_TRY(ivx_join_probe(ctx, ix->jv, mode, dk, ds, de, n, d_row, d_ex, d_b, d_p, cap, ctx->d_scalars));
     }
     u64 tot = 0;
     if (mode != JP_EXISTS) {
-        IVX_HIP(ctx, hipMemcpyAsync(ctx->h_scalars, ctx->d_scalars, 2 * sizeof(u64), hipMemcpyDeviceToHost, ctx->stream));
+        if (!note.totals_on_host) IVX_HIP(ctx, hipMemcpyAsync(ctx->h_scalars, ctx->d_scalars, 2 * sizeof(u64), hipMemcpyDeviceToHost, ctx->stream));
         IVX_HIP(ctx, hipStreamSynchronize(ctx->stream));
         tot = ctx->h_scalars[0];
         if (ctx->h_scalars[1]) { ctx->join_plan.valid = false; return ctx->fail(IVX_ERR_HIP, "internal error: the probe met an unpublished page of routed rows"); }
@@ -705,7 +710,7 @@
     {
         KernelTimer t(ctx);
         bool took = false;
-        if (regions) IVX_TRY(ivx_mark_probe_regions(ctx, ix->jv, ix->jv_nreg, dk, ds, de, n, dm, ix->jv_filter, ix->jv_pk24, ix->jv_fast && !ix->jv_fast_unknown, &took));
+        if (regions) IVX_TRY(ivx_mark_probe_regions(ctx, ix->jv, ix->jv_nreg, dk, ds, de, n, dm, ix->jv_filter, ix->jv_pk24, ix->jv_lean.load(std::memory_order_relaxed) == 1, &took));
         if (!took) IVX_TRY(ivx_mark_probe(ctx, ix->jv, dk, ds, de, n, dm));
     }
     return marks_or_back(ctx, mem, marks, dm, nw);
diff --git a/datafusion-bio-functions_amd/csrc/ivx_device.hpp b/datafusion-bio-functions_amd/csrc/ivx_device.hpp
--- a/datafusion-bio-functions_amd/csrc/ivx_device.hpp
+++ b/datafusion-bio-functions_amd/csrc/ivx_device.hpp
@@ -12,6 +12,9 @@
 {
     return __builtin_amdgcn_mbcnt_hi((u32)(mask >> 32), __builtin_amdgcn_mbcnt_lo((u32)mask, 0u));
 }
+
+template <typename T>
+__device__ __forceinline__ void host_store(T *p, T v) { __hip_atomic_store(p, v, __ATOMIC_RELAXED, __HIP_MEMORY_SCOPE_SYSTEM); }
 
 template <int CTRL, int ROWS>
 __device__ __forceinline__ u32 dpp0(u32 v) { return (u32)__builtin_amdgcn_update_dpp(0, (int)v, CTRL, ROWS, 0xf, false); }
diff --git a/datafusion-bio-functions_amd/csrc/ivx_internal.hpp b/datafusion-bio-functions_amd/csrc/ivx_internal.hpp
--- a/datafusion-bio-functions_amd/csrc/ivx_internal.hpp
+++ b/datafusion-bio-functions_amd/csrc/ivx_internal.hpp
@@ -18,6 +18,7 @@
 struct ivx_buf { void *p = nullptr; size_t cap = 0; };
 
 enum { IVX_NSCRATCH = 56, IVX_NPIN = 4 };
+enum { IVX_HS_HDR = 64, IVX_HS_WORDS = 80 };
 
 struct ivx_sub_plan {
     bool valid = false;
@@ -40,7 +41,8 @@
 struct ivx_route_ctl {
     u32 rcur[1024];
     u32 pool_next, pad0[3];
-    u32 rest_n[2], pad1[2];
+    u32 rest_n[2];
+    u32 fill_done, pad1;
     u32 rfirst[1032];
     u32 cfirst[1032];
 };
@@ -61,6 +63,7 @@
     PageTab pt{nullptr, 0u, 0u};
     bool packed = false;
     u32 rowbits = 32;
+    bool tables_due = false;
     bool all_routed = false;
     ivx_route_ctl *ctl = nullptr;
     FpRest *rest = nullptr; u64 *rest_rows = nullptr;
@@ -92,6 +95,8 @@
     ivx_buf pinned[IVX_NPIN];
     u64 *d_scalars = nullptr;
     u64 *h_scalars = nullptr;
+    u64 *hd_scalars = nullptr;
+    u64 hdr_mirror_serial = 0;
     ivx_sub_plan sub_plan;
     ivx_join_plan join_plan;
     ivx_metrics metrics{};
@@ -157,6 +162,7 @@
        HDR_LBUILD = 12 + IVX_MAXL ,
        HDR_BADKEY = 13 + IVX_MAXL ,
        HDR_WORDS = 14 + IVX_MAXL };
+static_assert(IVX_HS_HDR * sizeof(u64) + HDR_WORDS * sizeof(u32) <= IVX_HS_WORDS * sizeof(u64), "the header mirror fits the host words");
 #define IVX_FBITS_MAX (1u << 24)
 #define IVX_MAXREG 255
 #define IVX_MAXREG_WIDE 1023
@@ -234,8 +240,7 @@
     u32 jv_nreg = 0;
     bool jv_filter = false;
     bool jv_pk24 = false;
-    bool jv_fast = false;
-    bool jv_fast_unknown = false;
+    mutable std::atomic<int> jv_lean{0};
     hipEvent_t ready = nullptr;
     RankGridView gs{}, ge{};
     CoverageView cv{};
@@ -255,11 +260,17 @@
                           const u32 *key, const i32 *s, const i32 *e, u64 n,
                           u32 *per_row, u8 *exists, u32 *ob, u32 *op, u64 cap, u64 *d_cursor);
 enum { JP_COUNT = 0, JP_PER_ROW = 1, JP_EXISTS = 2, JP_FILL = 3 };
+struct ivx_probe_note {
+    u64 ix_serial = 0;
+    int fast = -1;
+    bool totals_on_host = false;
+};
 ivx_status ivx_join_probe_regions(ivx_ctx *ctx, const JoinIndexView &jv, u32 nreg, int mode,
                                   const u32 *key, const i32 *s, const i32 *e, u64 n,
                                   u32 *ob, u32 *op, u64 cap, u64 *d_cursor, bool planned = false, bool has_filter = false, bool pk24 = false,
                                   int fast = 0 , hipEvent_t ready = nullptr,
-                                  bool clear_cursor = false );
+                                  bool clear_cursor = false ,
+                                  ivx_probe_note *note = nullptr);
 
 enum { IVX_RV_COUNT = 0, IVX_RV_COVERAGE = 1, IVX_RV_PER_ROW = 2, IVX_RV_EXISTS = 3 };
 ivx_status ivx_route_view_build(ivx_ctx *ctx, ivx_index *ix, const i32 *origin, const u32 *span, const u32 *kcnt);
diff --git a/datafusion-bio-functions_amd/csrc/ivx_join.hip b/datafusion-bio-functions_amd/csrc/ivx_join.hip
--- a/datafusion-bio-functions_amd/csrc/ivx_join.hip
+++ b/datafusion-bio-functions_amd/csrc/ivx_join.hip
@@ -24,7 +24,8 @@
 
 __global__ __launch_bounds__(1024) void k_join_layout(const i32 *kmin, const i32 *kmax, const u32 *kcnt, u32 nkeys, u64 n,
                                                       i32 *origin, u32 *span, u32 *lbase, u32 *hdr, u64 maxcells,
-                                                      u32 *kreg, u32 *rkey, const u32 *lenhist, u32 regmax, u32 *fbase, int filter_mode, int lbuild_ok, const u32 *badkey)
+                                                      u32 *kreg, u32 *rkey, const u32 *lenhist, u32 regmax, u32 *fbase, int filter_mode, int lbuild_ok, const u32 *badkey,
+                                                      u32 *hmirror)
 {
     __shared__ u64 red[1024 / IVX_WAVE + 1];
     __shared__ u32 s_sh0;
@@ -214,6 +215,12 @@
         hdr[HDR_PK24] = (R && sh0 < 24 && R <= (1ull << (24 - sh0))) ? 1u : 0u;
         hdr[HDR_BADKEY] = *badkey;
         hdr[HDR_LBUILD] = (lbuild_ok && R && R <= LB_CCAP && rrun && rrun <= IVX_MAXREG_WIDE && s_cum[33] == s_cum[sh0 + 1]) ? 1u : 0u;
+        static_assert(HDR_WORDS % 2 == 0, "the mirror is written in 8-byte words");
+        u32 hv[HDR_WORDS];
+#pragma unroll
+        for (u32 w = 0; w < HDR_WORDS; w++) hv[w] = hdr[w];
+#pragma unroll
+        for (u32 w = 0; w < HDR_WORDS; w += 2) host_store((u64 *)hmirror + w / 2, (u64)hv[w] | ((u64)hv[w + 1] << 32));
     }
 }
 
@@ -346,13 +353,13 @@
 }
 
 __global__ __launch_bounds__(256) void k_join_regdesc(const i32 *origin, const u32 *span, const u32 *lbase, u32 *hdr,
-                                                      const u32 *kreg, const u32 *rkey, const u32 *binstart, ivx_regdesc *rdesc)
+                                                      const u32 *kreg, const u32 *rkey, const u32 *binstart, ivx_regdesc *rdesc, u32 *hslow)
 {
     const u32 r = threadIdx.x + blockIdx.x * 256;
     if (r == 0) {
         bool upper = hdr[HDR_LEVCNT] == 0;
         for (u32 l = 1; l < hdr[HDR_NLEV]; l++) upper |= hdr[HDR_LEVCNT + l] != 0;
-        if (upper) hdr[HDR_SLOW] = 1u;
+        if (upper) { hdr[HDR_SLOW] = 1u; host_store(hslow, 1u); }
     }
     if (r >= hdr[HDR_NREG]) return;
     const u32 sh0 = hdr[HDR_SH0];
@@ -369,7 +376,7 @@
     d.e0 = binstart[d.lb + d.slo];
     d.ne = binstart[d.lb + d.shi] - d.e0;
     d.rbase = (i32)((i64)d.origin + (i64)(rc0w << sh0));
-    if (d.ne > IVX_RP_ECAP || d.shi - d.slo + 1u > 8192u + IVX_RP_HALO + 2u) hdr[HDR_SLOW] = 1u;
+    if (d.ne > IVX_RP_ECAP || d.shi - d.slo + 1u > 8192u + IVX_RP_HALO + 2u) { hdr[HDR_SLOW] = 1u; host_store(hslow, 1u); }
     rdesc[r] = d;
 }
 
@@ -648,10 +655,15 @@
     if (filter_mode) { zr.big = (uint4 *)fbits; zr.nbig = (u32)(fwords / 4); }
     IVX_TRY(ivx_keystats_len(ctx, key, s, n, nkeys, kmin, kmax, kcnt, errflag, 1u, e, lenhist, &zr));
     const u32 grid = ivx_stream_grid(n, BT * 2, 16384);
-    hipLaunchKernelGGL(k_join_layout, dim3(1), dim3(1024), 0, st, kmin, kmax, kcnt, nkeys, n, origin, span, lbase, hdr, maxcells, kreg, rkey, (const u32 *)lenhist, (u32)(regcap - 1), fbase, filter_mode, lb_try ? 1 : 0, (const u32 *)errflag);
-    if (filter_mode) hipLaunchKernelGGL(k_join_filter, dim3(grid), dim3(BT), 0, st, key, s, e, n, nkeys, (const i32 *)origin, (const u32 *)span, (const u32 *)fbase, (const u32 *)hdr, fbits);
+    u32 *hmirror = (u32 *)(ctx->h_scalars + IVX_HS_HDR), *hmirror_d = (u32 *)(ctx->hd_scalars + IVX_HS_HDR);
+    ctx->hdr_mirror_serial = ix->serial;
+    hipLaunchKernelGGL(k_join_layout, dim3(1), dim3(1024), 0, st, kmin, kmax, kcnt, nkeys, n, origin, span, lbase, hdr, maxcells, kreg, rkey, (const u32 *)lenhist, (u32)(regcap - 1), fbase, filter_mode, lb_try ? 1 : 0, (const u32 *)errflag, hmirror_d);
+    auto launch_filter = [&]() {
+        hipLaunchKernelGGL(k_join_filter, dim3(grid), dim3(BT), 0, st, key, s, e, n, nkeys, (const i32 *)origin, (const u32 *)span, (const u32 *)fbase, (const u32 *)hdr, fbits);
+    };
     const bool want_route = ix->kind == IVX_KIND_OVERLAP && n >= (4u << 20);
     overlap = overlap && ctx->overlap && ctx->aux != nullptr && !want_route && n >= (1u << 16);
+    if (filter_mode && !overlap) launch_filter();
     hipStream_t tail_st = st;
     struct TailGuard {
         ivx_ctx *c; bool armed = false;
@@ -663,13 +675,14 @@
         IVX_HIP(ctx, hipEventRecord(ctx->ev_fork, st));
         IVX_HIP(ctx, hipStreamWaitEvent(ctx->aux, ctx->ev_fork, 0));
         tail_st = ctx->aux;
-        IVX_HIP(ctx, hipMemcpyAsync(ctx->h_scalars + 32, hdr, HDR_WORDS * sizeof(u32), hipMemcpyDeviceToHost, st));
         IVX_HIP(ctx, hipStreamSynchronize(st));
-        if (((const u32 *)(ctx->h_scalars + 32))[HDR_BADKEY]) return ctx->fail(IVX_ERR_INVALID, "build key id >= n_keys");
-        q_lds = lb_try && ((const u32 *)(ctx->h_scalars + 32))[HDR_LBUILD] != 0;
+        if (hmirror[HDR_BADKEY]) return ctx->fail(IVX_ERR_INVALID, "build key id >= n_keys");
+        q_lds = lb_try && hmirror[HDR_LBUILD] != 0;
         q_global = !q_lds;
+        if (filter_mode && hmirror[HDR_FG] != 0xFFFFFFFFu) launch_filter();
         guard.armed = true;
     }
+    hmirror[HDR_SLOW] = 0;
     if (q_lds)
         hipLaunchKernelGGL(k_lbuild_tiles, dim3(lb_tiles), dim3(LB_T), 0, tail_st, key, s, e, n, nkeys, (const i32 *)origin, (const u32 *)kreg, hdr,
                            (ivx_ent *)cellid, rank, lb_tstride(lb_tiles), binstart, maxcells + 1);
@@ -689,26 +702,22 @@
         hipLaunchKernelGGL(k_lbuild_regions, dim3(rgrid), dim3(LB_T), 0, tail_st, (const i32 *)origin, (const u32 *)span, (const u32 *)lbase, (const u32 *)kreg,
                            (const u32 *)rkey, (const u32 *)hdr, nkeys, (const ivx_ent *)cellid, (const u32 *)rank, lb_tiles, lb_tstride(lb_tiles), binstart, ent);
     }
-    hipLaunchKernelGGL(k_join_regdesc, dim3((u32)((regcap + 255) / 256)), dim3(256), 0, tail_st, origin, span, lbase, hdr, kreg, rkey, binstart, rdesc);
+    hipLaunchKernelGGL(k_join_regdesc, dim3((u32)((regcap + 255) / 256)), dim3(256), 0, tail_st, origin, span, lbase, hdr, kreg, rkey, binstart, rdesc, hmirror_d + HDR_SLOW);
     IVX_HIP(ctx, hipGetLastError());
     if (overlap) {
         if (ix->ready == nullptr) IVX_HIP(ctx, hipEventCreateWithFlags(&ix->ready, hipEventDisableTiming));
         IVX_HIP(ctx, hipEventRecord(ix->ready, ctx->aux));
         IVX_HIP(ctx, hipEventRecord(ctx->tail_ev, ctx->aux));
         ctx->tail_pending = true;
-        ix->jv_fast_unknown = true;
     }
     if (want_route) IVX_TRY(ivx_route_view_build(ctx, ix, origin, span, kcnt));
 
-    if (!overlap) {
-        IVX_HIP(ctx, hipMemcpyAsync(ctx->h_scalars + 32, hdr, HDR_WORDS * sizeof(u32), hipMemcpyDeviceToHost, st));
-        IVX_HIP(ctx, hipStreamSynchronize(st));
-    }
-    if (((const u32 *)(ctx->h_scalars + 32))[HDR_BADKEY]) return ctx->fail(IVX_ERR_INVALID, "build key id >= n_keys");
-    ix->jv_nreg = ((const u32 *)(ctx->h_scalars + 32))[HDR_NREG];
-    ix->jv_filter = ((const u32 *)(ctx->h_scalars + 32))[HDR_FG] != 0xFFFFFFFFu;
-    ix->jv_pk24 = ((const u32 *)(ctx->h_scalars + 32))[HDR_PK24] != 0;
-    ix->jv_fast = ((const u32 *)(ctx->h_scalars + 32))[HDR_SLOW] == 0 && ix->jv_nreg > 0;
+    if (!overlap) IVX_HIP(ctx, hipStreamSynchronize(st));
+    if (hmirror[HDR_BADKEY]) return ctx->fail(IVX_ERR_INVALID, "build key id >= n_keys");
+    ix->jv_nreg = hmirror[HDR_NREG];
+    ix->jv_filter = hmirror[HDR_FG] != 0xFFFFFFFFu;
+    ix->jv_pk24 = hmirror[HDR_PK24] != 0;
+    ix->jv_lean.store(overlap ? 2 : (hmirror[HDR_SLOW] == 0 && ix->jv_nreg > 0 ? 1 : 0), std::memory_order_relaxed);
     if (want_route) ivx_route_view_ready(ctx, ix);
     guard.armed = false;
 
diff --git a/datafusion-bio-functions_amd/csrc/ivx_ops32.hip b/datafusion-bio-functions_amd/csrc/ivx_ops32.hip
--- a/datafusion-bio-functions_amd/csrc/ivx_ops32.hip
+++ b/datafusion-bio-functions_amd/csrc/ivx_ops32.hip
@@ -805,7 +805,7 @@
 ivx_status ivx_count_probe(ivx_ctx *ctx, const ivx_index *ix, const u32 *key, const i32 *s, const i32 *e, u64 n, int strict, i64 *out)
 {
     if (n == 0) return IVX_OK;
-    if (rowval_regions_wanted(ix, n)) return ivx_rowval_probe_regions(ctx, ix->jv, ix->jv_nreg, IVX_RV_COUNT, key, s, e, n, strict, out, nullptr, ix->jv_filter, ix->jv_pk24, ix->jv_fast);
+    if (rowval_regions_wanted(ix, n)) return ivx_rowval_probe_regions(ctx, ix->jv, ix->jv_nreg, IVX_RV_COUNT, key, s, e, n, strict, out, nullptr, ix->jv_filter, ix->jv_pk24, ix->jv_lean.load(std::memory_order_relaxed) == 1);
     if (rowval_routed_wanted(ix, n)) return rowval_routed(ctx, ix, false, key, s, e, n, strict, out);
     hipLaunchKernelGGL(k_probe_count, dim3(ivx_stream_grid(n, OT)), dim3(OT), 0, ctx->stream, ix->gs, ix->ge, key, s, e, n, strict, out, (const u32 *)nullptr);
     IVX_HIP(ctx, hipGetLastError());
@@ -815,7 +815,7 @@
 ivx_status ivx_coverage_probe(ivx_ctx *ctx, const ivx_index *ix, const u32 *key, const i32 *s, const i32 *e, u64 n, int strict, i64 *out)
 {
     if (n == 0) return IVX_OK;
-    if (rowval_regions_wanted(ix, n)) return ivx_rowval_probe_regions(ctx, ix->jv, ix->jv_nreg, IVX_RV_COVERAGE, key, s, e, n, strict, out, nullptr, ix->jv_filter, ix->jv_pk24, ix->jv_fast);
+    if (rowval_regions_wanted(ix, n)) return ivx_rowval_probe_regions(ctx, ix->jv, ix->jv_nreg, IVX_RV_COVERAGE, key, s, e, n, strict, out, nullptr, ix->jv_filter, ix->jv_pk24, ix->jv_lean.load(std::memory_order_relaxed) == 1);
     if (rowval_routed_wanted(ix, n)) return rowval_routed(ctx, ix, true, key, s, e, n, strict, out);
     hipLaunchKernelGGL(k_probe_coverage, dim3(ivx_stream_grid(n, OT)), dim3(OT), 0, ctx->stream, ix->cv, key, s, e, n, strict, out, (const u32 *)nullptr);
     IVX_HIP(ctx, hipGetLastError());
diff --git a/datafusion-bio-functions_amd/csrc/ivx_regions.hpp b/datafusion-bio-functions_amd/csrc/ivx_regions.hpp
--- a/datafusion-bio-functions_amd/csrc/ivx_regions.hpp
+++ b/datafusion-bio-functions_amd/csrc/ivx_regions.hpp
@@ -37,8 +37,9 @@
 
 ivx_status ivx_route_flat(ivx_ctx *ctx, const JoinIndexView &jv, const u32 *key, const i32 *s, const i32 *e, u64 n, u32 adj,
                           u32 ndig, bool ids16, u32 max_tiles, ivx_routed *R);
-struct ivx_paged_opts { bool filter, packed, rowval, lean; u32 adj; u64 *zero2 = nullptr; };
+struct ivx_paged_opts { bool filter, packed, rowval, lean; u32 adj; u64 *zero2 = nullptr; bool defer_bounds = false; };
 ivx_status ivx_route_paged(ivx_ctx *ctx, const JoinIndexView &jv, u32 nreg, const u32 *key, const i32 *s, const i32 *e, u64 n,
                            const ivx_paged_opts &o, ivx_routed *R);
+ivx_status ivx_route_paged_bounds(ivx_ctx *ctx, const ivx_routed &R, u32 nreg);
 ivx_status ivx_route_two_level(ivx_ctx *ctx, const JoinIndexView &jv, u32 nreg, const u32 *key, const i32 *s, const i32 *e, u64 n, ivx_routed *R);
 ivx_status ivx_unroute_values(ivx_ctx *ctx, const ivx_routed &R, u32 nreg, int kind, const u32 *val, u64 n, void *out, u64 *d_total, int sorted_done = 0);
diff --git a/datafusion-bio-functions_amd/csrc/ivx_regions_probe.hip b/datafusion-bio-functions_amd/csrc/ivx_regions_probe.hip
--- a/datafusion-bio-functions_amd/csrc/ivx_regions_probe.hip
+++ b/datafusion-bio-functions_amd/csrc/ivx_regions_probe.hip
@@ -520,7 +520,24 @@
         nreg = ix.hdr[HDR_NREG];
         for (u32 t = threadIdx.x; t <= nreg; t += RP_T) s_cf[t] = cfirst[t];
         __syncthreads();
-        const u32 nchunk = s_cf[nreg];
+        return share();
+    }
+    __device__ __forceinline__ bool init_scan(const JoinIndexView &ix, u32 *s_cf, u32 *red, const u32 *rcur_, const PageTab &pt_, W *pool_, u32 rowbits_)
+    {
+        static_assert(IVX_MAXREG_WIDE < RP_T, "init_scan: one region per thread, and thread nreg for the total");
+        s_cfirst = s_cf; rcur = rcur_; pt = pt_; pool = pool_; rowbits = rowbits_; maxlen = pk_maxlen(rowbits_);
+        wv = __builtin_amdgcn_readfirstlane(threadIdx.x / IVX_WAVE); ln = lane_id();
+        nreg = ix.hdr[HDR_NREG];
+        const u32 t = threadIdx.x;
+        u32 tot;
+        const u32 ex = block_excl_scan<u32, RP_T>(t < nreg ? (rcur_[t] + FP_CHUNK - 1) / FP_CHUNK : 0u, red, &tot);
+        if (t <= nreg) s_cf[t] = ex;
+        __syncthreads();
+        return share();
+    }
+    __device__ __forceinline__ bool share()
+    {
+        const u32 nchunk = s_cfirst[nreg];
         c_lo = (u32)((u64)nchunk * blockIdx.x / gridDim.x);
         const u32 c_hi = (u32)((u64)nchunk * (blockIdx.x + 1) / gridDim.x);
         nbatch = (c_hi - c_lo) * SUB;
@@ -617,7 +634,7 @@
 
 template <int B, bool DRAIN>
 __global__ __launch_bounds__(RP_T) void k_fill_fast(JoinIndexView ix, const u64 *__restrict__ pool, const u32 *__restrict__ rcur,
-                                                    const u32 *__restrict__ cfirst, PageTab pt, u32 *__restrict__ ob, u32 *__restrict__ op, u64 cap,
+                                                    PageTab pt, u32 *__restrict__ ob, u32 *__restrict__ op, u64 cap,
                                                     unsigned long long *cursor, const u32 *bsel, u32 rowbits, FpRest *__restrict__ rest, u64 *__restrict__ rest_rows, u32 *rest_n,
                                                     u32 drain)
 {
@@ -630,7 +647,7 @@
     const u32 wv = __builtin_amdgcn_readfirstlane(threadIdx.x / IVX_WAVE), ln = lane_id();
     auto miss = [&]() { if (ln == 0) atomicOr((unsigned int *)(cursor + 1), 1u); };
     LeanRows<B, const u64> rows;
-    if (!rows.init(ix, s_cfirst, cfirst, rcur, pt, pool, rowbits)) return;
+    if (!rows.init_scan(ix, s_cfirst, &s_wat[0][0], rcur, pt, pool, rowbits)) return;
     Slice S;
     slice_init(ix, S, L);
     rows.start(miss);
@@ -743,16 +760,18 @@
 __global__ __launch_bounds__(256) void k_fill_rest(JoinIndexView ix, const u64 *__restrict__ pool, PageTab pt, const FpRest *__restrict__ rest,
                                                    const u64 *__restrict__ rest_rows, const u32 *__restrict__ rest_n, u32 *__restrict__ ob,
                                                    u32 *__restrict__ op, u64 cap, unsigned long long *cursor, const i32 *__restrict__ ps_in,
-                                                   const i32 *__restrict__ pe_in, u32 rowbits)
+                                                   const i32 *__restrict__ pe_in, u32 rowbits, u32 *done, u64 *host_totals)
 {
     const u32 nbat = rest_n[0], nrow = rest_n[1];
-    if (nbat == 0 && nrow == 0) return;
     const u32 wpb = blockDim.x / IVX_WAVE, ln = lane_id();
     const u32 sh0 = ix.hdr[HDR_SH0], nlev = ix.hdr[HDR_NLEV];
     auto rows64 = [&](bool ok, u32 r, u32 v) {
         i32 qs = 0, qe = -1; u32 row = 0, k = 0;
         if (ok) {
-            const auto e = rest_row(ix, pt, pool, r, v, rowbits, ps_in, pe_in, 0u, [&]() { atomicOr((unsigned int *)(cursor + 1), 1u); });
+            const auto e = rest_row(ix, pt, pool, r, v, rowbits, ps_in, pe_in, 0u, [&]() {
+                const u32 was = atomicOr((unsigned int *)(cursor + 1), 1u);
+                asm volatile("" ::"v"(was));
+            });
             qs = e.qs; qe = e.qe; row = e.row;
             k = ix.rkey[r];
         }
@@ -777,6 +796,12 @@
     for (u32 b = wave; b < nbat; b += nwave) {
         const FpRest w = rest[b];
         for (u32 t0 = 0; t0 < w.cnt; t0 += IVX_WAVE) rows64(t0 + ln < w.cnt, w.r, w.first + t0 + ln);
+    }
+    if (host_totals == nullptr) return;
+    __syncthreads();
+    if (threadIdx.x == 0 && __hip_atomic_fetch_add(done, 1u, __ATOMIC_RELAXED, __HIP_MEMORY_SCOPE_AGENT) == gridDim.x - 1u) {
+        host_store(host_totals, (u64)__hip_atomic_load(cursor, __ATOMIC_RELAXED, __HIP_MEMORY_SCOPE_AGENT));
+        host_store(host_totals + 1, (u64)__hip_atomic_load(cursor + 1, __ATOMIC_RELAXED, __HIP_MEMORY_SCOPE_AGENT));
     }
 }
 
@@ -1135,6 +1160,8 @@
     return R.form == IVX_ROWS_PAGED && R.packed && R.pt.lgpg >= 13 && R.rest_rows != nullptr;
 }
 
+bool lean_fill_ok(const ivx_routed &R, const RegionKnobs &K) { return lean_rows_ok(R) && !K.lean_off && R.rest != nullptr; }
+
 template <int V> using int_tag = std::integral_constant<int, V>;
 template <class F> void with_rows_per_lane(int b, F &&f)
 {
@@ -1186,39 +1213,48 @@
 }
 
 ivx_status probe_pairs(ivx_ctx *ctx, const JoinIndexView &jv, u32 nreg, int mode, const ivx_routed &R, u64 n, u32 *ob, u32 *op, u64 cap,
-                       u64 *d_cursor, u64 hint, int fast, bool reused, const RegionKnobs &K)
+                       u64 *d_cursor, u64 hint, int fast, bool reused, const RegionKnobs &K, ivx_probe_note *note)
 {
     hipStream_t st = ctx->stream;
     unsigned long long *cur = (unsigned long long *)d_cursor;
+    bool due = R.tables_due;
+    auto tables = [&]() -> ivx_status { if (due) { due = false; return ivx_route_paged_bounds(ctx, R, nreg); } return IVX_OK; };
     if (mode != JP_FILL) {
+        IVX_TRY(tables());
         launch_probe_regions<0, RP_B>(st, jv, R, RP_VGRID, ob, op, cap, cur);
         IVX_HIP(ctx, hipGetLastError());
         return IVX_OK;
     }
-    if (dense_fill_wanted(K, hint, n)) return dense_fill(ctx, jv, nreg, R, n, ob, op, cap, d_cursor);
+    if (dense_fill_wanted(K, hint, n)) { IVX_TRY(tables()); return dense_fill(ctx, jv, nreg, R, n, ob, op, cap, d_cursor); }
     const bool paged = R.form == IVX_ROWS_PAGED;
     u32 *bsel = paged && !R.all_routed ? (u32 *)(ctx->d_scalars + 11) : nullptr;
+    if (bsel) IVX_TRY(tables());
     if (bsel) hipLaunchKernelGGL(k_pick_rows, dim3(1), dim3(1), 0, st, R.rfirst, nreg, hint, K.rp_rows ? (u32)atoi(K.rp_rows) : 0u, bsel);
     auto every_b = [&](auto &&f) {
         if (bsel) { f(int_tag<8>{}); f(int_tag<4>{}); f(int_tag<2>{}); f(int_tag<1>{}); }
         else with_rows_per_lane(fill_rows_per_lane(K, hint, n), f);
     };
     const u32 *slow_gate = nullptr;
-    if (lean_rows_ok(R) && fast != 0 && !K.lean_off && R.rest != nullptr) {
+    if (fast != 0 && lean_fill_ok(R, K)) {
         u32 *rest_n = R.ctl->rest_n;
-        if (reused) IVX_HIP(ctx, hipMemsetAsync(rest_n, 0, 2 * sizeof(u32), st));
+        static_assert(offsetof(ivx_route_ctl, fill_done) == offsetof(ivx_route_ctl, rest_n) + 2 * sizeof(u32), "one memset clears the rest counts and the done-counter");
+        if (reused) IVX_HIP(ctx, hipMemsetAsync(rest_n, 0, 3 * sizeof(u32), st));
+        const bool publish = fast == 1 && note != nullptr && ctx->hd_scalars != nullptr;
         every_b([&](auto b) {
             const u32 drain = fill_drain_of(K, decltype(b)::value);
             with_bools([&](auto dr) {
-                hipLaunchKernelGGL((k_fill_fast<decltype(b)::value, IVX_B(dr)>), dim3(RP_GRID), dim3(RP_T), 0, st, jv, R.se, (const u32 *)R.ctl->rcur, (const u32 *)R.ctl->cfirst, R.pt, ob, op, cap, cur,
+                hipLaunchKernelGGL((k_fill_fast<decltype(b)::value, IVX_B(dr)>), dim3(RP_GRID), dim3(RP_T), 0, st, jv, R.se, (const u32 *)R.ctl->rcur, R.pt, ob, op, cap, cur,
                                    (const u32 *)bsel, R.rowbits, R.rest, R.rest_rows, rest_n, drain);
             }, drain != 0);
         });
-        hipLaunchKernelGGL(k_fill_rest, dim3(512), dim3(256), 0, st, jv, R.se, R.pt, (const FpRest *)R.rest, (const u64 *)R.rest_rows, (const u32 *)rest_n, ob, op, cap, cur, R.ds, R.de, R.rowbits);
+        hipLaunchKernelGGL(k_fill_rest, dim3(512), dim3(256), 0, st, jv, R.se, R.pt, (const FpRest *)R.rest, (const u64 *)R.rest_rows, (const u32 *)rest_n, ob, op, cap, cur, R.ds, R.de, R.rowbits,
+                           &R.ctl->fill_done, publish ? ctx->hd_scalars : (u64 *)nullptr);
         IVX_HIP(ctx, hipGetLastError());
+        if (publish) note->totals_on_host = true;
         if (fast == 1) return IVX_OK;
         slow_gate = jv.hdr + HDR_SLOW;
     }
+    IVX_TRY(tables());
     every_b([&](auto b) { launch_probe_regions<1, decltype(b)::value>(st, jv, R, RP_GRID, ob, op, cap, cur, bsel, slow_gate); });
     IVX_HIP(ctx, hipGetLastError());
     return IVX_OK;
@@ -1228,7 +1264,8 @@
 
 ivx_status ivx_join_probe_regions(ivx_ctx *ctx, const JoinIndexView &jv, u32 nreg, int mode,
                                   const u32 *key, const i32 *s, const i32 *e, u64 n,
-                                  u32 *ob, u32 *op, u64 cap, u64 *d_cursor, bool planned, bool has_filter, bool pk24, int fast, hipEvent_t ready, bool clear_cursor)
+                                  u32 *ob, u32 *op, u64 cap, u64 *d_cursor, bool planned, bool has_filter, bool pk24, int fast, hipEvent_t ready, bool clear_cursor,
+                                  ivx_probe_note *note)
 {
     auto wait_ready = [&]() -> ivx_status { if (ready) { IVX_HIP(ctx, hipStreamWaitEvent(ctx->stream, ready, 0)); ready = nullptr; } return IVX_OK; };
     const RegionKnobs K = region_knobs();
@@ -1246,13 +1283,19 @@
             IVX_TRY(wait_ready());
             IVX_TRY(ivx_route_flat(ctx, jv, key, s, e, n, 0u, nreg > IVX_MAXREG ? 1024u : 256u, false, 4, &R));
         } else {
-            IVX_TRY(ivx_route_paged(ctx, jv, nreg, key, s, e, n, ivx_paged_opts{has_filter && !K.filter_off, pk24 && !K.pack_off, false, fast != 0, 0u, clear_cursor ? d_cursor : nullptr}, &R));
+            const bool bounds_due = mode == JP_FILL && !(has_filter && !K.filter_off);
+            IVX_TRY(ivx_route_paged(ctx, jv, nreg, key, s, e, n, ivx_paged_opts{has_filter && !K.filter_off, pk24 && !K.pack_off, false, fast != 0, 0u, clear_cursor ? d_cursor : nullptr, bounds_due}, &R));
+            if (fast == 2 && ready != nullptr && note != nullptr && note->ix_serial != 0 && ctx->hdr_mirror_serial == note->ix_serial) {
+                IVX_HIP(ctx, hipEventSynchronize(ready));
+                fast = ((const u32 *)(ctx->h_scalars + IVX_HS_HDR))[HDR_SLOW] == 0 ? 1 : 0;
+                note->fast = fast;
+            }
         }
         if (mode == JP_COUNT) { pl.rows = R; pl.valid = true; }
     }
     IVX_TRY(wait_ready());
     const u64 hint = ctx->fill_hint ? ctx->fill_hint : (planned && pl.total < cap ? pl.total : cap);
-    return probe_pairs(ctx, jv, nreg, mode, R, n, ob, op, cap, d_cursor, hint, fast, planned, K);
+    return probe_pairs(ctx, jv, nreg, mode, R, n, ob, op, cap, d_cursor, hint, fast, planned, K, note);
 }
 
 ivx_status ivx_rowval_probe_regions(ivx_ctx *ctx, const JoinIndexView &jv, u32 nreg, int kind,
diff --git a/datafusion-bio-functions_amd/csrc/ivx_regions_route.hip b/datafusion-bio-functions_amd/csrc/ivx_regions_route.hip
--- a/datafusion-bio-functions_amd/csrc/ivx_regions_route.hip
+++ b/datafusion-bio-functions_amd/csrc/ivx_regions_route.hip
@@ -868,10 +868,18 @@
         else part(k_part_onepass<IVX_B(vec), 256, 12, IVX_B(klds), IVX_B(filt), IVX_B(pk)>, (u32)PA_T);
     }, cols_aligned16(key, s, e), jv.nkeys <= KT_MAX, o.filter, o.packed);
     if (o.rowval && !o.lean) hipLaunchKernelGGL(k_page_bounds, dim3(1), dim3(1024), 0, st, (const u32 *)ctl->rcur, nreg, ctl->rfirst);
-    else hipLaunchKernelGGL(k_chunk_bounds, dim3(1), dim3(1024), 0, st, (const u32 *)ctl->rcur, nreg, ctl->rfirst, ctl->cfirst);
+    else if (!o.defer_bounds) hipLaunchKernelGGL(k_chunk_bounds, dim3(1), dim3(1024), 0, st, (const u32 *)ctl->rcur, nreg, ctl->rfirst, ctl->cfirst);
     IVX_HIP(ctx, hipGetLastError());
     R->form = IVX_ROWS_PAGED; R->se = pool; R->ids = prow; R->rfirst = ctl->rfirst; R->pt = pt; R->packed = o.packed; R->rowbits = rowbits;
+    R->tables_due = o.defer_bounds && !(o.rowval && !o.lean);
     R->all_routed = !o.filter; R->ctl = ctl; R->vtab = vtab; R->ds = s; R->de = e; R->adj = o.adj;
+    return IVX_OK;
+}
+
+ivx_status ivx_route_paged_bounds(ivx_ctx *ctx, const ivx_routed &R, u32 nreg)
+{
+    hipLaunchKernelGGL(k_chunk_bounds, dim3(1), dim3(1024), 0, ctx->stream, (const u32 *)R.ctl->rcur, nreg, R.ctl->rfirst, R.ctl->cfirst);
+    IVX_HIP(ctx, hipGetLastError());
     return IVX_OK;
 }
 
```

New measurement: 36.32 billion overlap-pairs/s, median of 6. 1.02x the previous value.
